# FermiQ/octree-mg

Hardware: AMD Instinct MI355X
Metric: V-cycle cell-updates/s + smoother HBM GB/s vs roofline, 3D Poisson 512^3 (higher is better)
Workload: dtype f64; 1 GPU; C3: 3D Poisson, 512^3 per GPU, box 16, periodic, GSRB FAS V-cycle (n_cycle_down=up=2); mode=weak, box_size=16, parallelism=domain-decomposition x1 (RCCL halos)

## Files before the change

octree-mg_amd/csrc/omg_api.cpp:

```cpp
#include <algorithm>

#include "omg_host.h"

using namespace omg;
using namespace omg::host;

thread_local bool omg::host::g_host_only = false;

namespace {

thread_local std::string g_last_error;

template <typename F>
int guarded(F&& f) {
  try {
    f();
    return 0;
  } catch (const std::exception& e) {
    g_last_error = e.what();
    return 1;
  }
}

void resolve_stats(omg_ctx* c) {
  if (c->pending.empty()) return;
  for (auto& p : c->pending) {
    float ms = 0;
    HIPCHK(hipEventSynchronize(p.e1));
    HIPCHK(hipEventElapsedTime(&ms, p.e0, p.e1));
    for (int pass = 0; pass < (p.lvl == NO_LVL ? 1 : 2); pass++) {
      auto& s = c->stats[pass ? std::string(p.name) + "@" + std::to_string(p.lvl) : std::string(p.name)];
      s.launches++;
      s.ms += ms;
      s.cells += p.cells;
    }
    (void)hipEventDestroy(p.e0);
    (void)hipEventDestroy(p.e1);
  }
  c->pending.clear();
}

double* stage(omg_ctx* c, size_t n) {
  if (n > c->stage_n) {
    dfree(c->d_stage);
    HIPCHK(hipMalloc(&c->d_stage, sizeof(double) * n));
    c->stage_n = n;
  }
  return c->d_stage;
}

constexpr long long kDenseMax = 1LL << 40;

DensePlan& dense_plan(omg_ctx* c, Level& L, const long long* lo, const long long* n, const long long* stride,
                      bool aligned, bool generic, bool own_only) {
  for (auto& P : L.dense)
    if (std::equal(lo, lo + 3, P.lo) && std::equal(n, n + 3, P.n) && std::equal(stride, stride + 3, P.stride) &&
        P.aligned == aligned && P.generic == generic && P.own_only == own_only) {
      P.age = ++c->dense_age;
      return P;
    }
  if ((int)L.dense.size() < kDensePlans) L.dense.emplace_back();
  DensePlan& P = *std::min_element(L.dense.begin(), L.dense.end(),
                                   [](const DensePlan& a, const DensePlan& b) { return a.age < b.age; });
  if (P.d_clips) host_sync(c, c->stream);
  std::copy(lo, lo + 3, P.lo);
  std::copy(n, n + 3, P.n);
  std::copy(stride, stride + 3, P.stride);
  P.aligned = aligned;
  P.generic = generic;
  P.own_only = own_only;
  P.age = ++c->dense_age;
  P.n_row = P.n_gen = 0;
  P.n_cells = 0;
  std::vector<DenseClip> row, gen;
  const long long nc = L.nc;
  const bool row_ok = !generic && aligned && dense_row_nc(L.nc) && stride[1] % 2 == 0 && stride[2] % 2 == 0;
  auto clip = [&](int b) {
    DenseClip r{};
    r.box = b;
    int* lohi[3][2] = {{&r.i0, &r.i1}, {&r.j0, &r.j1}, {&r.k0, &r.k1}};
    long long cells = 1;
    for (int d = 0; d < 3; d++) {
      const long long g0 = ((long long)c->ix[(size_t)(L.ids[b] - 1) * 3 + d] - 1) * nc;
      const long long a = std::max(g0, lo[d]), e = std::min(g0 + nc, lo[d] + n[d]);
      if (a >= e) return;
      *lohi[d][0] = (int)(a - g0) + 1;
      *lohi[d][1] = (int)(e - g0);
      r.off += (a - lo[d]) * stride[d];
      cells *= e - a;
    }
    P.n_cells += cells;
    (row_ok && r.i0 == 1 && r.i1 == L.nc && r.off % 2 == 0 ? row : gen).push_back(r);
  };
  if (own_only)
    for (int b : L.host_local) clip(b);
  else
    for (int b = 0; b < L.n; b++) clip(b);
  P.n_row = (int)row.size();
  P.n_gen = (int)gen.size();
  row.insert(row.end(), gen.begin(), gen.end());
  if (!c->host_only && !row.empty()) {
    if (row.size() > P.cap) {
      dfree(P.d_clips);
      if (P.h_clips) HIPCHK(hipHostFree(P.h_clips));
      P.h_clips = nullptr;
      P.cap = 0;
      HIPCHK(hipHostMalloc((void**)&P.h_clips, sizeof(DenseClip) * row.size()));
      HIPCHK(hipMalloc(&P.d_clips, sizeof(DenseClip) * row.size()));
      P.cap = row.size();
    }
    std::copy(row.begin(), row.end(), P.h_clips);
    HIPCHK(hipMemcpyAsync(P.d_clips, P.h_clips, sizeof(DenseClip) * row.size(), hipMemcpyHostToDevice, c->stream));
  }
  return P;
}

void dense_io(omg_ctx* c, int lvl, int iv, double* dev, const long long* lo, const long long* n,
              const long long* stride, void* stream, long long* n_cells, bool put) {
  const char* who = put ? "omg_put_dense" : "omg_get_dense";
  auto fail = [&](const std::string& what) { throw OmgError(std::string(who) + ": " + what); };
  Level* L = level_ptr(c, lvl);
  if (!L) fail("no such level");
  if (iv < 1 || iv > c->n_vars) fail("bad variable index");
  if (!lo || !n || !stride) fail("lo, n and stride are required");
  for (int d = 0; d < 3; d++) {
    if (n[d] < 0) fail("negative extent");
    if (n[d] > kDenseMax || lo[d] > kDenseMax || lo[d] < -kDenseMax || stride[d] > kDenseMax)
      fail("window out of range");
  }
  if (stride[0] != 1) fail("stride[0] must be 1");
  const bool empty = n[0] == 0 || n[1] == 0 || n[2] == 0;
  if (!empty) {
    if (stride[1] < n[0]) fail("stride[1] < n[0]");
    if (stride[2] / n[1] < stride[1]) fail("stride[2] < stride[1]*n[1]");
    if (stride[2] > LLONG_MAX / 8 / n[2]) fail("window out of range");
    if (!dev) fail("NULL pointer with a non-empty window");
  }
  if (put && L->replicated)
    fail("level " + std::to_string(lvl) + " is replicated on every rank: use omg_upload_level");
  const bool generic = env_flag("OMG_DENSE_GENERIC");
  const bool aligned = ((uintptr_t)dev & 15) == 0;
  if (c->host_only) {
    if (n_cells) *n_cells = empty ? 0 : dense_plan(c, *L, lo, n, stride, aligned, generic, L->replicated).n_cells;
    return;
  }
  if (!empty) {
    hipPointerAttribute_t at{};
    if (hipPointerGetAttributes(&at, dev) != hipSuccess) {
      (void)hipGetLastError();
      fail("the pointer is not device memory");
    }
    if (at.type != hipMemoryTypeDevice) fail("the pointer is not device memory");
    if (at.device != c->device) fail("the pointer belongs to another GPU than the context's");
    hipDeviceptr_t base = nullptr;
    size_t bytes = 0;
    if (hipMemGetAddressRange(&base, &bytes, (hipDeviceptr_t)dev) == hipSuccess) {
      const long long extent = (n[2] - 1) * stride[2] + (n[1] - 1) * stride[1] + n[0];
      if ((const char*)dev + (size_t)extent * sizeof(double) > (const char*)base + bytes)
        fail("the window reaches past the end of the pointer's allocation");
    } else {
      (void)hipGetLastError();
    }
  }
  if (put) {
    enter(c);
    if (iv == 1) phi_dirty(c, lvl);
  } else {
    enter(c, false);
  }
  if (n_cells) *n_cells = 0;
  if (empty || !L->n) return;
  DensePlan& P = dense_plan(c, *L, lo, n, stride, aligned, generic, L->replicated);
  if (n_cells) *n_cells = P.n_cells;
  if (!P.n_cells) return;
  if ((long long)P.n_gen * 16 > INT_MAX) fail("too many boxes for one launch");
  hipStream_t user = (hipStream_t)stream;
  const bool foreign = user != c->stream;
  if (foreign) {
    HIPCHK(hipEventRecord(c->ev_dense_in, user));
    HIPCHK(hipStreamWaitEvent(c->stream, c->ev_dense_in, 0));
  }
  {
    Prof p(c, put ? "dense_put" : "dense_get", (double)P.n_cells, lvl);
    const LevelView V = L->view();
    if (P.n_row) {
      Prof pr(c, put ? "dense_put_row" : "dense_get_row", (double)P.n_row * L->nc * L->nc * L->nc, lvl);
      launch_dense_row(V, iv, P.d_clips, P.n_row, dev, stride[1], stride[2], put, c->stream);
    }
    launch_dense_cell(V, iv, P.d_clips + P.n_row, P.n_gen, dev, stride[1], stride[2], put, c->stream);
    HIPCHK(hipGetLastError());
  }
  if (foreign) {
    HIPCHK(hipEventRecord(c->ev_dense_out, c->stream));
    HIPCHK(hipStreamWaitEvent(user, c->ev_dense_out, 0));
  }
}

}

extern "C" {

const char* omg_last_error(void) { return g_last_error.c_str(); }

int omg_get_unique_id(void* out) {
  return guarded([&] {
    ncclUniqueId id;
    NCCLCHK(ncclGetUniqueId(&id));
    std::memcpy(out, &id, sizeof(id));
  });
}

int omg_loopback_unique_id(long long tag, void* out) {
  return guarded([&] {
    loopback_unique_id(tag, out);
  });
}

int omg_host_unique_id(void* out) {
  return guarded([&] {
    host_unique_id(out);
  });
}

int omg_set_host_transport(omg_ctx* c, omg_host_exchange_fn exchange, omg_host_allgather_fn allgather, void* user) {
  return guarded([&] {
    if (!c->host_xport) throw OmgError("omg_set_host_transport: the context was not created with omg_host_unique_id");
    c->hx_exchange = exchange;
    c->hx_allgather = allgather;
    c->hx_user = user;
  });
}

int omg_device_count(int* n) {
  return guarded([&] { HIPCHK(hipGetDeviceCount(n)); });
}

int omg_ctx_create(omg_ctx** out, int device, int rank, int n_ranks, const void* unique_id) {
  return guarded([&] {
    if (n_ranks < 1 || rank < 0 || rank >= n_ranks) throw OmgError("bad rank / n_ranks");
    if (n_ranks > 1 && !unique_id && device != OMG_DEVICE_NONE)
      throw OmgError("unique_id required for n_ranks > 1");
    auto plan_switches = [](omg_ctx* c) {
      c->no_block3 = env_flag("OMG_NO_BLOCK3");
      c->no_block3_phys = env_flag("OMG_NO_BLOCK3_PHYS");
      c->no_deep = env_flag("OMG_NO_DEEP");
      if (const char* v = getenv("OMG_BLOCK3_MIN_BOXES")) c->b3_min_boxes = std::max(1, atoi(v));
      if (const char* v = getenv("OMG_BLOCK3_COLUMN")) c->b3_col = std::min(std::max(2, atoi(v) & ~1), kB3MaxZ);
      if (const char* v = getenv("OMG_BLOCK3_SMALL_COL")) c->b3_col_small = std::min(std::max(2, atoi(v) & ~1), kB3MaxZ);
    };
    if (device == OMG_DEVICE_NONE) {
      omg_ctx* c = new omg_ctx();
      c->device = device;
      c->rank = rank;
      c->n_ranks = n_ranks;
      c->host_only = true;
      plan_switches(c);
      *out = c;
      return;
    }
    if (device < 0) {
      int n_dev = 0;
      HIPCHK(hipGetDeviceCount(&n_dev));
      if (n_dev < 1) throw OmgError("no HIP device visible");
      device = rank % n_dev;
    }
    omg_ctx* c = new omg_ctx();
    c->device = device;
    c->rank = rank;
    c->n_ranks = n_ranks;
    c->no_tail = env_flag("OMG_NO_TAIL");
    c->no_fuse_up = env_flag("OMG_NO_FUSE_UP");
    c->no_skip1 = env_flag("OMG_NO_SKIP1");
    c->tail_timing = env_flag("OMG_TAIL_TIMING");
    c->no_fill_tile = env_flag("OMG_NO_FILL_TILE");
    c->no_fill_crhs = env_flag("OMG_NO_FILL_CRHS");
    c->no_tail_crhs = env_flag("OMG_NO_TAIL_CRHS");
    c->no_rbgv = env_flag("OMG_NO_RBGV");
    c->no_graph = !env_flag("OMG_GRAPH");
    c->no_fuse_down = env_flag("OMG_NO_FUSE_DOWN");
    c->no_rb_fill_fuse = env_flag("OMG_NO_RB_FUSE");
    c->no_gs_plane = env_flag("OMG_NO_GS_PLANE");
    c->no_fill_xl = env_flag("OMG_NO_FILL_XL");
    c->no_gs_dbl = env_flag("OMG_NO_GS_DBL");
    plan_switches(c);
    c->no_block3p = env_flag("OMG_NO_BLOCK3P");
    c->no_block3r = env_flag("OMG_NO_BLOCK3R");
    c->block4 = !env_flag("OMG_NO_BLOCK4");
    c->no_block4p = env_flag("OMG_NO_BLOCK4P");
    c->block4_phys = env_flag("OMG_BLOCK4_PHYS");
    c->no_defer_gc = env_flag("OMG_NO_DEFER_GC");
    c->no_rhs_pend = env_flag("OMG_NO_RHS_PEND");
    c->no_fuse_down_bc = env_flag("OMG_NO_FUSE_DOWN_BC");
    c->roctx = env_flag("OMG_ROCTX");
    c->debug = env_flag("OMG_DEBUG");
    c->check_collective = env_flag("OMG_CHECK_COLLECTIVE") || c->debug;
    if (const char* v = getenv("OMG_GRAPH_FAIL")) c->graph_fail_at = std::atoi(v);
    HIPCHK(hipSetDevice(device));
    HIPCHK(hipStreamCreateWithFlags(&c->stream, hipStreamNonBlocking));
    HIPCHK(hipMalloc(&c->d_scalar, sizeof(double) * (64 + 2 * (size_t)n_ranks)));
    HIPCHK(hipMalloc(&c->d_red, sizeof(double) * (8 + 2 * (size_t)n_ranks)));
    HIPCHK(hipMemset(c->d_red, 0, sizeof(double) * (8 + 2 * (size_t)n_ranks)));
    HIPCHK(hipMalloc(&c->d_rhs_pend, sizeof(double) * (omg::kRhsPendMax + 1)));
    HIPCHK(hipMemset(c->d_rhs_pend, 0, sizeof(double) * (omg::kRhsPendMax + 1)));
    HIPCHK(hipMalloc(&c->d_maxslots, sizeof(unsigned long long) * omg::kMaxSlots * omg::kMaxSlotStride));
    HIPCHK(hipMalloc(&c->d_tail, sizeof(TailArgs)));
    c->h_tail = new TailArgs;
    std::memset(c->h_tail, 0xff, sizeof(TailArgs));
    HIPCHK(hipMemset(c->d_maxslots, 0, sizeof(unsigned long long) * omg::kMaxSlots * omg::kMaxSlotStride));
    HIPCHK(hipStreamCreateWithFlags(&c->stream2, hipStreamNonBlocking));
    {
      int least = 0, greatest = 0;
      HIPCHK(hipDeviceGetStreamPriorityRange(&least, &greatest));
      HIPCHK(hipStreamCreateWithPriority(&c->stream_comm, hipStreamNonBlocking, greatest));
      c->comm_priority = greatest;
    }
    HIPCHK(hipEventCreateWithFlags(&c->ev_bnd, hipEventDisableTiming));
    HIPCHK(hipEventCreateWithFlags(&c->ev_comm, hipEventDisableTiming));
    HIPCHK(hipEventCreateWithFlags(&c->ev_main, hipEventDisableTiming));
    HIPCHK(hipEventCreateWithFlags(&c->ev_side, hipEventDisableTiming));
    HIPCHK(hipEventCreateWithFlags(&c->ev_phi, hipEventDisableTiming));
    HIPCHK(hipEventCreateWithFlags(&c->ev_dense_in, hipEventDisableTiming));
    HIPCHK(hipEventCreateWithFlags(&c->ev_dense_out, hipEventDisableTiming));
    HIPCHK(hipHostMalloc(&c->h_scalar, sizeof(double) * (16 + (size_t)n_ranks)));
    for (int iv = 0; iv < kMaxVars; iv++)
      for (int nb = 0; nb < 6; nb++) {
        c->bc[iv].type[nb] = OMG_BC_DIRICHLET;
        c->bc[iv].value[nb] = 0.0;
      }
    transport_attach(c, unique_id);
    *out = c;
  });
}

int omg_ctx_destroy(omg_ctx* c) {
  return guarded([&] {
    if (!c) return;
    if (c->host_only) {
      g_host_only = true;
      free_levels(c);
      g_host_only = false;
      delete c;
      return;
    }
    (void)hipSetDevice(c->device);
    (void)hipStreamSynchronize(c->stream);
    (void)hipStreamSynchronize(c->stream2);
    (void)hipStreamSynchronize(c->stream_comm);
    free_levels(c);
    dfree(c->d_scalar);
    if (c->d_tail) (void)hipFree(c->d_tail);
    if (c->d_tail_stamps) (void)hipFree(c->d_tail_stamps);
    delete c->h_tail;
    dfree(c->d_red);
    dfree(c->d_rhs_pend);
    dfree(c->d_maxslots);
    for (auto& kv : c->graphs)
      if (kv.second) (void)hipGraphExecDestroy(kv.second);
    c->graphs.clear();
    dfree(c->d_stage);
    if (c->ev_main) (void)hipEventDestroy(c->ev_main);
    if (c->ev_side) (void)hipEventDestroy(c->ev_side);
    if (c->ev_phi) (void)hipEventDestroy(c->ev_phi);
    if (c->ev_dense_in) (void)hipEventDestroy(c->ev_dense_in);
    if (c->ev_dense_out) (void)hipEventDestroy(c->ev_dense_out);
    if (c->stream2) (void)hipStreamDestroy(c->stream2);
    if (c->stream_comm) (void)hipStreamDestroy(c->stream_comm);
    if (c->ev_bnd) (void)hipEventDestroy(c->ev_bnd);
    if (c->ev_comm) (void)hipEventDestroy(c->ev_comm);
    if (c->h_scalar) (void)hipHostFree(c->h_scalar);
    if (c->h_xsend) (void)hipHostFree(c->h_xsend);
    if (c->h_xrecv) (void)hipHostFree(c->h_xrecv);
    transport_detach(c);
    (void)hipStreamDestroy(c->stream);
    delete c;
  });
}

int omg_tree_setup(omg_ctx* c, int n_boxes, const int* lvl, const int* parent, const int* children,
                   const int* neighbors, const int* ix, const int* rank, int lowest_lvl,
                   int highest_lvl, int first_normal_lvl, int box_size, const int* box_size_lvl,
                   const double* dr, const int* list_off, const int* lists, int n_vars) {
  return guarded([&] {
    if (n_vars < 4 || n_vars > kMaxVars) throw OmgError("n_vars out of range");
    struct HostOnly {
      explicit HostOnly(bool on) { g_host_only = on; }
      ~HostOnly() { g_host_only = false; }
    } host_only_scope(c->host_only);
    if (!c->host_only) (void)hipSetDevice(c->device);
    free_levels(c);
    c->n_boxes = n_boxes;
    c->lvl.assign(lvl, lvl + n_boxes);
    c->parent.assign(parent, parent + n_boxes);
    c->children.assign(children, children + 8 * (size_t)n_boxes);
    c->neighbors.assign(neighbors, neighbors + 6 * (size_t)n_boxes);
    c->ix.assign(ix, ix + 3 * (size_t)n_boxes);
    c->rank_of.assign(rank, rank + n_boxes);
    c->lowest = lowest_lvl;
    c->highest = highest_lvl;
    c->first_normal = first_normal_lvl;
    c->box_size = box_size;
    c->n_vars = n_vars;
    c->bsl.clear();
    c->drl.clear();
    c->ids.clear(); c->leaves.clear(); c->parents.clear(); c->ref_bnds.clear();
    for (int l = lowest_lvl; l <= highest_lvl; l++) {
      const int li = l - lowest_lvl;
      c->bsl[l] = box_size_lvl[li];
      c->drl[l] = {dr[3 * li], dr[3 * li + 1], dr[3 * li + 2]};
      std::map<int, std::vector<int>>* dst[4] = {&c->ids, &c->leaves, &c->parents, &c->ref_bnds};
      for (int t = 0; t < 4; t++) {
        const int a = list_off[4 * li + t], b = list_off[4 * li + t + 1];
        (*dst[t])[l] = std::vector<int>(lists + a, lists + b);
      }
    }
    if (!c->host_only) {
      host_sync(c, c->stream);
      host_sync(c, c->stream2);
    }
    c->rhs_cache_valid = false;
    c->phi_shift_pending = false;
    c->phi_mean_on_side = false;
    build_plan(c);
    if (!c->host_only) HIPCHK(hipDeviceSynchronize());
  });
}

int omg_plan_transfer(omg_ctx* c, int lvl, int which, int dir, int cap, int* peers, long long* keys,
                      int* n_items, int* item_doubles) {
  return guarded([&] {
    Level* L = level_ptr(c, lvl);
    if (!L) throw OmgError("no such level");
    if (which < 0 || which > 5) throw OmgError("omg_plan_transfer: bad transfer");
    const Transfer* T[6] = {&L->halo, &L->restr, &L->prol, &L->rbx, &L->repl, &L->deep_phi};
    const auto& lists = dir ? T[which]->recv : T[which]->send;
    int n = 0;
    for (auto& p : lists)
      for (long long k : p.keys) {
        if (n < cap) {
          peers[n] = p.peer;
          keys[n] = k;
        }
        n++;
      }
    *n_items = n;
    *item_doubles = T[which]->item_doubles;
  });
}

int omg_set_operator(omg_ctx* c, int op, double lambda) {
  return guarded([&] { set_operator(c, op, lambda); });
}

int omg_set_smoother(omg_ctx* c, int smoother, int n_cycle_down, int n_cycle_up, int max_coarse_cycles,
                     double res_abs, double res_rel) {
  return guarded([&] {
    if (smoother != OMG_SMOOTHER_GS && smoother != OMG_SMOOTHER_GSRB)
      throw OmgError("unsupported smoother type");
    if (smoother != c->smoother || std::max(n_cycle_down, 0) != c->n_cycle_down ||
        std::max(n_cycle_up, 0) != c->n_cycle_up)
      rhs_pend_retry(c);
    c->smoother = smoother;
    c->n_substeps = smoother == OMG_SMOOTHER_GSRB ? 2 : 1;
    ensure_rhs_lex(c);
    c->n_cycle_down = std::max(n_cycle_down, 0);
    c->n_cycle_up = std::max(n_cycle_up, 0);
    c->max_coarse_cycles = max_coarse_cycles;
    c->res_abs = res_abs;
    c->res_rel = res_rel;
  });
}

int omg_set_subtract_mean(omg_ctx* c, int on) {
  return guarded([&] { c->subtract_mean = on; });
}

int omg_set_bc(omg_ctx* c, int iv, int nb, int bc_type, double bc_value) {
  return guarded([&] {
    if (iv < 1 || iv > kMaxVars || nb < 1 || nb > 6) throw OmgError("omg_set_bc: bad iv/nb");
    enter(c, false);
    phi_dirty_all(c);
    c->bc[iv - 1].type[nb - 1] = bc_type;
    c->bc[iv - 1].value[nb - 1] = bc_value;
  });
}

int omg_set_bc_faces(omg_ctx* c, int iv, const long long* face_off, const int* face_type,
                     const double* data, long long n_data) {
  return guarded([&] {
    if (iv < 1 || iv > kMaxVars) throw OmgError("omg_set_bc_faces: bad iv");
    if (!c->host_only) enter(c, false);
    phi_dirty_all(c);
    const int k = iv - 1;
    for (auto& kv : c->d_face_off_lvl[k]) dfree(kv.second);
    for (auto& kv : c->d_face_type_lvl[k]) dfree(kv.second);
    c->d_face_off_lvl[k].clear();
    c->d_face_type_lvl[k].clear();
    c->h_face_off_lvl[k].clear();
    c->h_face_type_lvl[k].clear();
    dfree(c->d_face_data[k]);
    if (!face_off) return;
    std::vector<double> packed;
    for (auto& kv : c->levels) {
      Level& L = kv.second;
      if (!L.n) continue;
      std::vector<long long> off(L.n * 6, -1);
      std::vector<int> typ(L.n * 6, 0);
      const long long n2 = (long long)L.nc * L.nc;
      if (L.replicated) {
        bool any[6] = {}, miss[6] = {};
        for (int b = 0; b < L.n; b++)
          for (int nb = 0; nb < 6; nb++) {
            if (L.h_nbk[(size_t)b * 6 + nb] != NB_PHYS) continue;
            (face_off[(size_t)(L.ids[b] - 1) * 6 + nb] >= 0 ? any : miss)[nb] = true;
          }
        for (int nb = 0; nb < 6; nb++)
          if (any[nb] && miss[nb])
            throw OmgError("omg_set_bc_faces: replicated level " + std::to_string(L.lvl) +
                           " needs the boundary table of every box (omg_replicated_level)");
      }
      for (int b = 0; b < L.n; b++)
        for (int nb = 0; nb < 6; nb++) {
          const long long o = face_off[(size_t)(L.ids[b] - 1) * 6 + nb];
          if (o < 0) continue;
          if (o + n2 > n_data) throw OmgError("omg_set_bc_faces: offset out of range");
          off[b * 6 + nb] = (long long)packed.size();
          typ[b * 6 + nb] = face_type[(size_t)(L.ids[b] - 1) * 6 + nb];
          packed.insert(packed.end(), data + o, data + o + n2);
        }
      c->d_face_off_lvl[k][kv.first] = to_device(off);
      c->d_face_type_lvl[k][kv.first] = to_device(typ);
      c->h_face_off_lvl[k][kv.first] = off;
      c->h_face_type_lvl[k][kv.first] = typ;
    }
    c->d_face_data[k] = to_device(packed);
  });
}

int omg_level_size(omg_ctx* c, int lvl, int* n_boxes, int* nc) {
  return guarded([&] {
    Level* L = level_ptr(c, lvl);
    if (!L) throw OmgError("no such level");
    *n_boxes = (int)L->host_local.size();
    *nc = L->nc;
  });
}

int omg_set_coarse_replication(omg_ctx* c, long long max_cells) {
  return guarded([&] {
    if (!c->levels.empty()) throw OmgError("omg_set_coarse_replication: call before omg_tree_setup");
    if (max_cells < 0) throw OmgError("omg_set_coarse_replication: max_cells < 0");
    c->rep_cells = max_cells;
  });
}

int omg_replicated_level(omg_ctx* c, int* lvl) {
  return guarded([&] { *lvl = c->rep_lvl == INT_MIN ? c->lowest - 1 : c->rep_lvl; });
}

int omg_upload_level(omg_ctx* c, int lvl, int iv, const double* host) {
  return guarded([&] {
    enter(c);
    Level* L = level_ptr(c, lvl);
    if (!L) throw OmgError("no such level");
    if (iv < 1 || iv > c->n_vars) throw OmgError("bad variable index");
    if (iv == 1) phi_dirty(c, lvl);
    if (!L->n) return;
    const size_t s = L->nc + 2, box = s * s * s, n = box * L->n;
    double* st = stage(c, n);
    if (L->replicated) {
      std::vector<double> full(n, 0.0);
      for (size_t q = 0; q < L->host_local.size(); q++)
        std::memcpy(full.data() + box * L->host_local[q], host + box * q, sizeof(double) * box);
      HIPCHK(hipMemcpyAsync(st, full.data(), sizeof(double) * n, hipMemcpyHostToDevice, c->stream));
      launch_from_ref(L->view(), iv, st, c->stream);
      if (L->repl.n_send || L->repl.n_recv) {
        launch_box_pack(L->view(), iv, L->repl.d_send_items, L->repl.n_send, L->d_sendbuf, c->stream);
        exchange(c, L->repl, L->d_sendbuf, L->d_recvbuf, nullptr, lvl);
        launch_box_unpack(L->view(), iv, L->repl.d_recv_items, L->repl.n_recv, L->d_recvbuf, c->stream);
      }
      host_sync(c, c->stream);
      return;
    }
    HIPCHK(hipMemcpyAsync(st, host, sizeof(double) * n, hipMemcpyHostToDevice, c->stream));
    launch_from_ref(L->view(), iv, st, c->stream);
    host_sync(c, c->stream);
  });
}

int omg_download_level(omg_ctx* c, int lvl, int iv, double* host) {
  return guarded([&] {
    enter(c, false);
    Level* L = level_ptr(c, lvl);
    if (!L) throw OmgError("no such level");
    if (iv < 1 || iv > c->n_vars) throw OmgError("bad variable index");
// ... 242 lines not shown
```

octree-mg_amd/csrc/omg_cycle.cpp:

```cpp
#include <algorithm>
#include <cmath>
#include <numeric>

#include "omg_host.h"

namespace omg {
namespace host {

static GcBC bc_for(omg_ctx* c, int lvl, int iv) {
  GcBC g;
  for (int nb = 0; nb < 6; nb++) {
    g.type[nb] = c->bc[iv - 1].type[nb];
    g.value[nb] = c->bc[iv - 1].value[nb];
  }
  auto it = c->d_face_off_lvl[iv - 1].find(lvl);
  g.face_off = it == c->d_face_off_lvl[iv - 1].end() ? nullptr : it->second;
  auto jt = c->d_face_type_lvl[iv - 1].find(lvl);
  g.face_type = jt == c->d_face_type_lvl[iv - 1].end() ? nullptr : jt->second;
  g.face_data = c->d_face_data[iv - 1];
  g.phi_stored = c->phi_bc_data_stored;
  return g;
}

void rb_stale_above(omg_ctx* c, int lvl) {
  if (Level* U = level_ptr(c, lvl + 1)) {
    if (U->any_rb) U->phi_gc_ok = false;
    U->rbgv_ok = false;
  }
}
void phi_dirty(omg_ctx* c, int lvl) {
  if (Level* L = level_ptr(c, lvl)) L->phi_gc_ok = L->gc_deferred = false;
  rb_stale_above(c, lvl);
}
void phi_dirty_all(omg_ctx* c) {
  for (auto& kv : c->levels) kv.second.phi_gc_ok = kv.second.rbgv_ok = kv.second.gc_deferred = false;
}

static void rb_host_fixup(omg_ctx* c, Level* L, int iv) {
  if (!c->rbh_any) return;
  auto it = L->rbh.find(iv);
  if (it == L->rbh.end() || it->second.n == 0) return;
  if (c->capturing) throw OmgError("refinement_bnd host callback inside a captured cycle");
  RbHostFaces& R = it->second;
  const int nc = L->nc, nc2 = nc * nc;
  const size_t per = (size_t)(nc + 2) * (nc + 2) * (nc + 2);
  launch_rbh_gather(L->view(), view_of(c, L->lvl - 1), iv, L->d_rb, R.d_items, R.d_slot, R.n, L->d_rbrecv, R.d_cgc,
                    R.d_cc, c->stream);
  HIPCHK(hipMemcpyAsync(R.h_cgc, R.d_cgc, sizeof(double) * R.n * nc2, hipMemcpyDeviceToHost, c->stream));
  HIPCHK(hipMemcpyAsync(R.h_cc, R.d_cc, sizeof(double) * R.n * per, hipMemcpyDeviceToHost, c->stream));
  host_sync(c, c->stream);
  for (int q0 = 0; q0 < R.n;) {
    int q1 = q0;
    while (q1 < R.n && R.nbs[q1] == R.nbs[q0]) q1++;
    const int nb = R.nbs[q0];
    auto fn = (omg_rb_fn)c->rb_fn[iv - 1][nb - 1];
    fn(c->rb_user[iv - 1][nb - 1], L->lvl, iv, q1 - q0, R.ids.data() + q0, R.nbs.data() + q0, nc,
       R.h_cgc + (size_t)q0 * nc2, R.h_cc + (size_t)q0 * per);
    q0 = q1;
  }
  HIPCHK(hipMemcpyAsync(R.d_cc, R.h_cc, sizeof(double) * R.n * per, hipMemcpyHostToDevice, c->stream));
  launch_rbh_scatter(L->view(), iv, R.d_items, R.n, R.d_cc, c->stream);
  host_sync(c, c->stream);
}

static void finish_rb(omg_ctx* c, Level* L, int iv);
static void finish_halo(omg_ctx* c, Level* L, int iv, bool rb_hook = true) {
  if (c->n_ranks > 1) {
    if (L->halo.n_send || L->halo.n_recv) {
      exchange(c, L->halo, L->d_sendbuf, L->d_recvbuf, nullptr, L->lvl);
      launch_unpack_faces(L->view(), iv, L->halo.d_recv_items, L->halo.n_recv, L->d_recvbuf, c->stream);
    }
    finish_rb(c, L, iv);
  }
  if (rb_hook) rb_host_fixup(c, L, iv);
}

static void finish_rb(omg_ctx* c, Level* L, int iv) {
  if (c->n_ranks == 1) return;
  if (L->rbx.n_send || L->rbx.n_recv) {
    launch_rb_pack(view_of(c, L->lvl - 1), iv, L->rbx.d_send_items, L->rbx.n_send, L->nc, L->d_rbsend,
                   c->stream);
    exchange(c, L->rbx, L->d_rbsend, L->d_rbrecv, nullptr, L->lvl);
    launch_rb_unpack(L->view(), iv, L->rbx.d_recv_items, L->rbx.n_recv, L->d_rbrecv, c->stream);
  }
}

void fill_gc_lvl(omg_ctx* c, int lvl, int iv) {
  if (lvl < c->lowest) throw OmgError("fill_ghost_cells_lvl: lvl < lowest_lvl");
  if (lvl > c->highest) throw OmgError("fill_ghost_cells_lvl: lvl > highest_lvl");
  Level* L = level_ptr(c, lvl);
  if (!L) return;
  if (iv == 1) {
    L->phi_gc_ok = true;
    L->gc_deferred = false;
    rb_stale_above(c, lvl);
  }
  if (L->n) {
    Prof p(c, "fill_gc", (double)L->n * 6 * L->nc * L->nc, lvl);
    if (iv != 1 || L->has_rb || c->no_fill_tile ||
        !launch_fill_tile(L->sweep_view(), bc_for(c, lvl, iv), L->d_sendbuf, c->stream))
      launch_fill_gc(L->view(), iv, 3, view_of(c, lvl - 1), L->d_rb, bc_for(c, lvl, iv), L->d_sendbuf,
                     c->stream);
  }
  finish_halo(c, L, iv);
}

static void deep_before(omg_ctx* c, Level* L, int colour) {
  if (!L->deep) return;
  materialize_rhs(c, L);
  const LevelView V = L->view();
  if (c->check_collective && (allreduce(c, L->prox_rhs_ok ? 1.0 : 0.0, true) > 0.5) != L->prox_rhs_ok)
    throw OmgError("deep halo: the rhs refill decision differs across ranks (an rhs write was not collective)");
  if (!L->prox_rhs_ok) {
    Prof p(c, "deep_rhs", (double)L->deep_rhs.n_recv * 64, L->lvl);
    launch_deep_copy(V, 2, 0, 64, L->deep_rhs.d_send_items, L->deep_rhs.n_send, L->d_sendbuf, false, c->stream);
    exchange(c, L->deep_rhs, L->d_sendbuf, L->d_recvbuf, nullptr, L->lvl);
    launch_deep_copy(V, 2, 0, 64, L->deep_rhs.d_recv_items, L->deep_rhs.n_recv, L->d_recvbuf, true, c->stream);
    L->prox_rhs_ok = true;
  }
  Prof p(c, "deep_phi", (double)L->deep_phi.n_recv * 32, L->lvl);
  launch_deep_copy(V, 1, colour, 32, L->deep_phi.d_send_items, L->deep_phi.n_send, L->d_sendbuf, false, c->stream);
  exchange(c, L->deep_phi, L->d_sendbuf, L->d_recvbuf, nullptr, L->lvl);
  launch_deep_copy(V, 1, colour, 32, L->deep_phi.d_recv_items, L->deep_phi.n_recv, L->d_recvbuf, true, c->stream);
}
static void deep_after(omg_ctx* c, Level* L, bool defer = false) {
  if (!L->deep) return;
  hipStream_t st = c->stream;
  if (defer && L->n_bnd && L->n_int) {
    HIPCHK(hipEventRecord(c->ev_bnd, c->stream));
    HIPCHK(hipStreamWaitEvent(c->stream_comm, c->ev_bnd, 0));
    st = c->stream_comm;
    L->faces_pending = true;
  }
  Prof p(c, "deep_faces", (double)L->halo.n_recv * L->nc * L->nc, L->lvl, st);
  launch_face_pack(L->view(), 1, L->halo.d_send_items, L->halo.n_send, L->d_sendbuf, st);
  exchange(c, L->halo, L->d_sendbuf, L->d_recvbuf, st, L->lvl);
  launch_unpack_faces(L->view(), 1, L->halo.d_recv_items, L->halo.n_recv, L->d_recvbuf, st);
  if (L->faces_pending) HIPCHK(hipEventRecord(c->ev_comm, c->stream_comm));
}
static void deep_res(omg_ctx* c, Level* L) {
  if (!L->deep) return;
  const LevelView V = L->view();
  Prof p(c, "deep_res", (double)L->deep_rhs.n_recv * 64, L->lvl);
  launch_deep_copy(V, 4, 0, 64, L->deep_rhs.d_send_items, L->deep_rhs.n_send, L->d_sendbuf, false, c->stream);
  exchange(c, L->deep_rhs, L->d_sendbuf, L->d_recvbuf, nullptr, L->lvl);
  launch_deep_copy(V, 4, 0, 64, L->deep_rhs.d_recv_items, L->deep_rhs.n_recv, L->d_recvbuf, true, c->stream);
  launch_face_pack(V, 4, L->halo.d_send_items, L->halo.n_send, L->d_sendbuf, c->stream);
  exchange(c, L->halo, L->d_sendbuf, L->d_recvbuf, nullptr, L->lvl);
  launch_unpack_faces(V, 4, L->halo.d_recv_items, L->halo.n_recv, L->d_recvbuf, c->stream);
}

static void faces_join(omg_ctx* c, Level* L) {
  if (!L || !L->faces_pending) return;
  HIPCHK(hipStreamWaitEvent(c->stream, c->ev_comm, 0));
  L->faces_pending = false;
}

bool smooth_boxes(omg_ctx* c, int lvl, int n_cycle, int first_substep, int skip_last,
                  bool want_res, bool four, bool defer_faces) {
  Level* L = level_ptr(c, lvl);
  const int n_sub = n_cycle * c->n_substeps - skip_last;
  bool res_done = false;
  if (!L) return false;
  if (n_sub >= 1) rb_stale_above(c, lvl);
  const bool absorb = L->shift_pending && c->smoother == OMG_SMOOTHER_GSRB && n_sub >= 1 &&
                      (L->phi_gc_ok || L->gc_deferred) &&
                      !L->has_rb && gs_tiled(L->nc, c->op, L->has_rb) && !(L->d_b3 && L->b3_phys);
  if (L->shift_pending && !absorb) materialize_level(c, L);
  if (c->smoother != OMG_SMOOTHER_GSRB) {
    materialize_rhs(c, L);
    const bool ring = n_sub >= 1 && L->d_rhs_lex && gs_lex_ring_ok(L->nc, c->op);
    if (ring && !L->rhs_lex_ok) {
      Prof p(c, "rhs_lex", (double)L->n * L->nc * L->nc * L->nc, lvl);
      launch_rhs_lex(L->view(), L->d_rhs_lex, c->stream);
      L->rhs_lex_ok = true;
    }
    const bool xlf = ring && L->d_xlay && !L->has_rb && !c->no_fill_tile && !c->no_fill_xl;
    if (xlf && L->d_galt && n_sub % 2 == 0 && L->n && !c->no_gs_dbl) {
      const GcBC bc = bc_for(c, lvl, 1);
      double* prim = L->d_phi + 2 * (long long)L->view().hv;
      for (int n = 1; n <= n_sub; n++) {
        const bool odd = n & 1;
        GhostSets gs;
        gs.in = odd ? prim : L->d_galt;
        gs.in_stride = odd ? L->stride : 6 * (long long)stored_face(L->nc);
        gs.out = odd ? L->d_galt : prim;
        gs.out_stride = odd ? 6 * (long long)stored_face(L->nc) : L->stride;
        gs.phys_load = n > 1;
        Prof p(c, "smoother_gs", (double)L->n * L->nc * L->nc * L->nc, lvl);
        launch_gs_lex(L->view(), c->op, c->lambda, c->stream, L->d_rhs_lex, nullptr, &gs, &bc);
      }
      if (L->n_physbox) {
        Prof p(c, "fill_gc", (double)L->n_physbox * 6 * L->nc * L->nc, lvl);
        launch_phys_gc(L->view(), bc, L->d_physbox, L->n_physbox, c->stream);
      }
      L->phi_gc_ok = true;
      return false;
    }
    for (int n = 1; n <= n_sub; n++) {
      if (L->n) {
        Prof p(c, "smoother_gs", (double)L->n * L->nc * L->nc * L->nc, lvl);
        launch_gs_lex(L->view(), c->op, c->lambda, c->stream, ring ? L->d_rhs_lex : nullptr,
                      xlf ? L->d_xlay : nullptr);
      }
      if (xlf) {
        L->phi_gc_ok = true;
        if (L->n) {
          Prof p(c, "fill_gc", (double)L->n * 6 * L->nc * L->nc, lvl);
          launch_fill_tile_xl(L->sweep_view(), bc_for(c, lvl, 1), L->d_sendbuf, L->d_xlay, c->stream);
        }
        finish_halo(c, L, 1);
      } else {
        fill_gc_lvl(c, lvl, 1);
      }
    }
    return false;
  }
  for (int n = first_substep; n <= n_sub; n++) {
    const int e = n & 1;
    const bool odd = L->nc & 1;
    if (n == 1 && absorb) phi_mean_ready(c);
    const double* shift = (n == 1 && absorb) ? red_mean(c, 0) : nullptr;
    if (n == 1) L->shift_pending = false;
    B3Phys P3;
    const B3Phys* ph = nullptr;
    const bool b3 = b3_usable(c, lvl, P3, ph);
    if (four && (n_sub - n + 1) % 4 == 0 && b3 && (!ph || c->block4_phys)) {
      double* other = L->d_phi == L->d_data ? L->d_phi_buf : L->d_data;
      deep_before(c, L, 1 - e);
      if (ph) materialize_rhs(c, L);
      {
        Prof p(c, "smoother_gsrb4", 2.0 * L->n * L->nc * L->nc * L->nc, lvl);
        launch_gsrb4(L->view(), other, L->d_b3, L->n_b3, c->op, c->lambda, e, shift, c->stream, nullptr, nullptr,
                     ph, true, rhs_shifts(c, L));
      }
      L->d_phi = other;
      if (L->gc_deferred) L->phi_gc_ok = true, L->gc_deferred = false;
      deep_after(c, L, defer_faces && n + 3 == n_sub);
      n += 3;
      continue;
    }
    if (n + 2 <= n_sub && b3 && !(want_res && (n_sub - n + 1) % 3 != 0)) {
      double* other = L->d_phi == L->d_data ? L->d_phi_buf : L->d_data;
      const bool push1 = L->deep || !(skip_last == 1 && n + 2 == n_sub && e == 1);
      const bool res = want_res && n + 2 == n_sub && push1;
      materialize_rhs(c, L);
      deep_before(c, L, 1 - e);
      {
        Prof p(c, res ? "smoother_gsrb3r" : "smoother_gsrb3", 1.5 * L->n * L->nc * L->nc * L->nc, lvl);
        launch_gsrb3(L->view(), other, L->d_b3, L->n_b3, c->op, c->lambda, e, shift, c->stream, push1, nullptr,
                     nullptr, 1, res, ph);
      }
      res_done = res;
      L->d_phi = other;
      if (L->gc_deferred) L->phi_gc_ok = true, L->gc_deferred = false;
      deep_after(c, L);
      if (res) deep_res(c, L);
      n += 2;
      continue;
    }
    if (L->gc_deferred) fill_gc_lvl(c, lvl, 1);
    materialize_rhs(c, L);
    if (L->n_bnd && L->n_int && !odd && gs_tiled(L->nc, c->op, L->has_rb)) {
      const int gvm = L->d_rbgv ? (L->rbgv_ok ? 2 : 1) : 0;
      if (gvm) L->rbgv_ok = true;
      {
        Prof p(c, "smoother_gsrb", 0.5 * L->n_bnd * L->nc * L->nc * L->nc, lvl);
        launch_gs_substep(L->sweep_view(), c->op, c->lambda, e, 1 << e, view_of(c, lvl - 1), L->d_rb, L->has_rb,
                          bc_for(c, lvl, 1), L->d_sendbuf, shift, c->stream, L->d_bnd, L->n_bnd, L->d_rbgv, gvm);
      }
      HIPCHK(hipEventRecord(c->ev_bnd, c->stream));
      {
        Prof p(c, "smoother_gsrb", 0.5 * L->n_int * L->nc * L->nc * L->nc, lvl);
        launch_gs_substep(L->sweep_view(), c->op, c->lambda, e, 1 << e, view_of(c, lvl - 1), L->d_rb, L->has_rb,
                          bc_for(c, lvl, 1), L->d_sendbuf, shift, c->stream, L->d_int, L->n_int, L->d_rbgv, gvm);
      }
      HIPCHK(hipStreamWaitEvent(c->stream_comm, c->ev_bnd, 0));
      exchange(c, L->halo, L->d_sendbuf, L->d_recvbuf, c->stream_comm, lvl);
      launch_unpack_faces(L->view(), 1, L->halo.d_recv_items, L->halo.n_recv, L->d_recvbuf, c->stream_comm);
      HIPCHK(hipEventRecord(c->ev_comm, c->stream_comm));
      HIPCHK(hipStreamWaitEvent(c->stream, c->ev_comm, 0));
      finish_rb(c, L, 1);
      if (!L->phi_gc_ok) fill_gc_lvl(c, lvl, 1);
      else rb_host_fixup(c, L, 1);
      continue;
    }
    if (L->n) {
      Prof p(c, "smoother_gsrb", 0.5 * L->n * L->nc * L->nc * L->nc, lvl);
      const int gvm = L->d_rbgv ? (L->rbgv_ok ? 2 : 1) : 0;
      if (gvm) L->rbgv_ok = true;
      launch_gs_substep(L->sweep_view(), c->op, c->lambda, e, odd ? 0 : 1 << e, view_of(c, lvl - 1), L->d_rb,
                        L->has_rb, bc_for(c, lvl, 1), L->d_sendbuf, shift, c->stream, nullptr, 0, L->d_rbgv, gvm);
    }
    const bool full_fill = odd || !L->phi_gc_ok;
    finish_halo(c, L, 1, !full_fill);
    if (full_fill) fill_gc_lvl(c, lvl, 1);
  }
  return res_done;
}

static bool tiled_level(omg_ctx* c, const Level* L) {
  (void)c;
  return L && tiled_nc(L->nc);
}

void residual_lvl(omg_ctx* c, int lvl, unsigned long long* maxbits) {
  Level* L = level_ptr(c, lvl);
  if (!L || L->n == 0) return;
  if (!tiled_level(c, L)) materialize_rhs(c, L);
  Prof p(c, "residual", (double)L->n * L->nc * L->nc * L->nc, lvl);
  if (tiled_level(c, L))
    launch_resid_restrict(L->sweep_view(), empty_view(), c->op, c->lambda, maxbits, 0, nullptr, nullptr, c->stream,
                          nullptr, 0, rhs_shifts(c, L));
  else
    launch_residual(L->view(), c->op, c->lambda, maxbits, c->stream);
}

static double max_residual_levels(omg_ctx* c, int lo, int hi) {
  unsigned long long* d = (unsigned long long*)c->d_scalar;
  for (int l = lo; l <= hi; l++) {
    residual_lvl(c, l, c->d_maxslots);
    launch_max_fold(c->d_maxslots, d, l > lo, c->stream);
  }
  HIPCHK(hipMemcpyAsync(c->h_scalar, d, 8, hipMemcpyDeviceToHost, c->stream));
  if (c->capturing) {
    if (c->max_deferred) throw OmgError("internal: two max-residual readbacks in one captured cycle");
    c->max_deferred = true;
    return 0.0;
  }
  host_sync(c, c->stream);
  return c->h_scalar[0];
}

double max_residual_lvl(omg_ctx* c, int lvl) { return max_residual_levels(c, lvl, lvl); }

static void restrict_remote(omg_ctx* c, int iv, int lvl) {
  Level* F = level_ptr(c, lvl);
  Level* C = level_ptr(c, lvl - 1);
  if (c->n_ranks > 1 && F && C && (F->restr.n_send || F->restr.n_recv)) {
    launch_restrict_pack(F->view(), iv, F->restr.d_send_items, F->restr.n_send, F->d_sendbuf, c->stream);
    exchange(c, F->restr, F->d_sendbuf, C->d_recvbuf, nullptr, lvl);
    launch_restrict_unpack(C->view(), iv, F->restr.d_recv_items, F->restr.n_recv, F->nc / 2, C->d_recvbuf,
                           c->stream);
  }
}

void restrict_lvl(omg_ctx* c, int iv, int lvl) {
  if (lvl <= c->lowest) throw OmgError("cannot restrict lvl <= lowest_lvl");
  if (iv == 1) phi_dirty(c, lvl - 1);
  Level* F = level_ptr(c, lvl);
  restrict_remote(c, iv, lvl);
  if (F && F->n_pairs) {
    Prof p(c, "restrict", (double)F->n_pairs * F->nc * F->nc * F->nc, lvl);
    launch_restrict(F->view(), view_of(c, lvl - 1), iv, F->d_pairs, F->n_pairs, F->d_parent_local, F->d_dix,
                    c->stream);
  }
}

void prolong(omg_ctx* c, int lvl, int iv, int iv_to, int add) {
  if (lvl == c->highest) throw OmgError("cannot prolong highest level");
  if (lvl < c->lowest) throw OmgError("cannot prolong below lowest level");
  if (iv_to == 1) phi_dirty(c, lvl + 1);
  Level* F = level_ptr(c, lvl + 1);
  Level* C = level_ptr(c, lvl);
  const LevelView FV = view_of(c, lvl + 1), CV = view_of(c, lvl);
  if (c->n_ranks > 1 && F && C && (F->prol.n_send || F->prol.n_recv)) {
    launch_prolong_pack(CV, FV, iv, F->prol.d_send_items, F->prol.n_send, C->d_sendbuf, c->stream);
    exchange(c, F->prol, C->d_sendbuf, F->d_recvbuf, nullptr, lvl + 1);
    launch_prolong_unpack(FV, iv_to, add, F->prol.d_recv_items, F->prol.n_recv, F->d_recvbuf,
                          c->stream);
  }
  if (F && F->n_pairs) {
    Prof p(c, "prolong", (double)F->n_pairs * F->nc * F->nc * F->nc, lvl + 1);
    launch_prolong(CV, FV, iv, iv_to, add, F->d_pairs, F->n_pairs, F->d_parent_local, F->d_dix,
                   c->stream);
  }
}

static bool smooth_resid_ok(omg_ctx* c, int lvl) {
  const Level* F = level_ptr(c, lvl);
  const Level* C = level_ptr(c, lvl - 1);
  if (F) {
    const auto rbh = F->rbh.find(1);
    if (rbh != F->rbh.end() && rbh->second.n) return false;
  }
  return !c->no_fuse_down && F && C && F->n && c->smoother == OMG_SMOOTHER_GSRB && c->n_substeps == 2 &&
         c->n_cycle_down >= 1 &&
         (c->op == OP_LPL || c->op == OP_HELM) && (F->nc == 16 || F->nc == 8) &&
         !(c->no_fuse_down_bc && (F->has_rb || F->has_phys)) && (!F->has_remote || F->n_int) &&
         !F->any_rbx;
}

void update_coarse(omg_ctx* c, int lvl, bool fused, bool tail_crhs) {
  Level* F = level_ptr(c, lvl);
  if (Level* Cl = level_ptr(c, lvl - 1)) {
    Cl->rhs_lex_ok = Cl->prox_rhs_ok = false;
    if (Cl->all_parents) Cl->shift_pending = false;
    else materialize_level(c, Cl);
    materialize_rhs(c, Cl);
  }
  if (F && (fused || !tiled_level(c, F))) materialize_rhs(c, F);
  if (F && F->n && tiled_level(c, F)) {
    const bool rbgv = F->rbgv_ok;
    phi_dirty(c, lvl - 1);
    if (fused && F->has_remote) {
      const bool faces = F->any_phys || F->any_rb;
      {
        Prof p(c, "smoother_gsrb", 0.5 * F->n_bnd * F->nc * F->nc * F->nc, lvl);
        launch_gs_substep(F->view(), c->op, c->lambda, 0, faces ? 1 | 4 : 1, view_of(c, lvl - 1), F->d_rb,
                          F->has_rb, bc_for(c, lvl, 1), F->d_sendbuf, nullptr, c->stream, F->d_bnd, F->n_bnd,
                          rbgv ? F->d_rbgv : nullptr, rbgv ? 2 : 0);
      }
      HIPCHK(hipEventRecord(c->ev_bnd, c->stream));
      {
        Prof p(c, "smooth_resid", (double)F->n_int * F->nc * F->nc * F->nc, lvl);
        if (!launch_smooth_resid(F->sweep_view(), view_of(c, lvl - 1), c->op, c->lambda, 1, F->d_parent_local,
                                 F->d_dix, c->stream, F->d_int, F->n_int, bc_for(c, lvl, 1), F->has_rb, F->has_phys,
                                 rbgv ? F->d_rbgv : nullptr))
          throw OmgError("smooth_resid: not available for this level");
      }
      HIPCHK(hipStreamWaitEvent(c->stream_comm, c->ev_bnd, 0));
      exchange(c, F->halo, F->d_sendbuf, F->d_recvbuf, c->stream_comm, lvl);
      launch_unpack_faces(F->view(), 1, F->halo.d_recv_items, F->halo.n_recv, F->d_recvbuf, c->stream_comm, 1);
      HIPCHK(hipEventRecord(c->ev_comm, c->stream_comm));
      HIPCHK(hipStreamWaitEvent(c->stream, c->ev_comm, 0));
      if (faces && F->n_bndface) {
        Prof p(c, "face_gc", (double)F->n_bndface * 6 * F->nc * F->nc, lvl);
        launch_face_gc(F->view(), view_of(c, lvl - 1), bc_for(c, lvl, 1), F->d_bndface, F->n_bndface, c->stream);
      }
      {
        Prof p(c, "resid_restrict", (double)F->n_bnd * F->nc * F->nc * F->nc, lvl);
        launch_resid_restrict(F->sweep_view(), view_of(c, lvl - 1), c->op, c->lambda, nullptr, 1, F->d_parent_local,
                              F->d_dix, c->stream, F->d_bnd, F->n_bnd, rhs_shifts(c, F));
      }
    } else if (fused) {
      Prof p(c, "smooth_resid", (double)F->n * F->nc * F->nc * F->nc, lvl);
      if (!launch_smooth_resid(F->sweep_view(), view_of(c, lvl - 1), c->op, c->lambda, 1, F->d_parent_local,
                               F->d_dix, c->stream, nullptr, 0, bc_for(c, lvl, 1), F->has_rb, F->has_phys,
                               rbgv ? F->d_rbgv : nullptr))
        throw OmgError("smooth_resid: not available for this level");
    } else if (F->faces_pending) {
      {
        Prof p(c, "resid_restrict", (double)F->n_int * F->nc * F->nc * F->nc, lvl);
        launch_resid_restrict(F->sweep_view(), view_of(c, lvl - 1), c->op, c->lambda, nullptr, 1, F->d_parent_local,
                              F->d_dix, c->stream, F->d_int, F->n_int, rhs_shifts(c, F));
      }
      faces_join(c, F);
      {
        Prof p(c, "resid_restrict", (double)F->n_bnd * F->nc * F->nc * F->nc, lvl);
        launch_resid_restrict(F->sweep_view(), view_of(c, lvl - 1), c->op, c->lambda, nullptr, 1, F->d_parent_local,
                              F->d_dix, c->stream, F->d_bnd, F->n_bnd, rhs_shifts(c, F));
      }
    } else {
      Prof p(c, "resid_restrict", (double)F->n * F->nc * F->nc * F->nc, lvl);
      launch_resid_restrict(F->sweep_view(), view_of(c, lvl - 1), c->op, c->lambda, nullptr, 1, F->d_parent_local,
                            F->d_dix, c->stream, nullptr, 0, rhs_shifts(c, F));
    }
    restrict_remote(c, 1, lvl);
    restrict_remote(c, 4, lvl);
    if (fused && (F->any_phys || F->any_rb)) F->phi_gc_ok = false;
  } else {
    residual_lvl(c, lvl, nullptr);
    restrict_lvl(c, 1, lvl);
    restrict_lvl(c, 4, lvl);
  }
  if (tail_crhs) return;
  Level* C = level_ptr(c, lvl - 1);
  if (C && C->n && !C->parents.empty() && !C->has_rb && !C->has_remote && !c->no_fill_tile && !c->no_fill_crhs &&
      (C->nc == 16 || C->nc == 8 || C->nc == 4)) {
    C->phi_gc_ok = true;
    rb_stale_above(c, lvl - 1);
    {
      Prof p(c, "fill_crhs", (double)C->n * C->nc * C->nc * C->nc, lvl - 1);
      launch_fill_crhs(C->sweep_view(), c->op, c->lambda, bc_for(c, lvl - 1, 1), C->d_parmask, c->stream);
    }
    finish_halo(c, C, 1);
    return;
  }
  fill_gc_lvl(c, lvl - 1, 1);
  if (C && !C->parents.empty()) {
    Prof p(c, "coarse_rhs", (double)C->parents.size() * C->nc * C->nc * C->nc, lvl - 1);
    if (!launch_coarse_rhs_tile(C->sweep_view(), c->op, c->lambda, C->d_parents, (int)C->parents.size(), c->stream))
      launch_coarse_rhs(C->view(), c->op, c->lambda, C->d_parents, (int)C->parents.size(), c->stream);
  }
}

void correct_children(omg_ctx* c, int lvl) {
  Level* C = level_ptr(c, lvl);
  if (C && !C->parents.empty()) {
    Prof p(c, "sub_parents", (double)C->parents.size() * C->nc * C->nc * C->nc, lvl);
    launch_sub_parents(C->view(), C->d_parents, (int)C->parents.size(), c->stream);
  }
  prolong(c, lvl, 4, 1, 1);
}

static bool prolong_smooth(omg_ctx* c, int lvl) {
  Level* F = level_ptr(c, lvl + 1);
  Level* C = level_ptr(c, lvl);
  const bool rb_ok = F && !c->no_rb_fill_fuse && !F->any_rbx && (F->nc == 16 || F->nc == 8) &&
                     !(F->rbh.count(1) && F->rbh.at(1).n);
  if (c->no_fuse_up || !F || !C || !F->prolong_smooth_ok || c->smoother != OMG_SMOOTHER_GSRB ||
      (c->op != OP_LPL && c->op != OP_HELM) ||
      c->n_cycle_up < 1 || (F->has_rb && !rb_ok) || (F->has_remote && !F->n_int) || !gs_tiled(F->nc, c->op, F->has_rb) ||
      !((size_t)F->n == 8 * C->parents.size() || C->nc * 2 == F->nc) ||
      (c->n_ranks > 1 && (F->prol.n_send || F->prol.n_recv)))
    return false;
  if (F->shift_pending) materialize_level(c, F);
  materialize_rhs(c, F);
  rb_stale_above(c, lvl + 1);
  const bool split = F->has_remote;
  {
    const int n = split ? F->n_int : F->n;
    Prof p(c, "prolong_smooth", (double)n * F->nc * F->nc * F->nc, lvl + 1);
    launch_prolong_smooth(C->view(), F->sweep_view(), c->op, c->lambda, F->d_parent_local, F->d_dix,
                          bc_for(c, lvl + 1, 1), C->nc * 2 == F->nc, split ? F->d_int : nullptr, n,
                          split ? F->d_push0 : nullptr, c->stream, F->has_rb, F->has_rb ? F->d_rbgv : nullptr);
    if (F->has_rb && F->d_rbgv) F->rbgv_ok = true;
  }
  if (split) {
    {
      Prof p(c, "prolong_fill", (double)F->n_bnd * F->nc * F->nc * F->nc, lvl + 1);
      launch_prolong_fill(C->view(), F->sweep_view(), 4, F->d_parent_local, F->d_dix, bc_for(c, lvl + 1, 1),
                          F->d_sendbuf, true, !c->no_skip1, c->stream, F->d_bnd, F->n_bnd, false,
                          F->h_rb.empty() ? nullptr : F->d_rb);
    }
    finish_halo(c, F, 1);
    {
      Prof p(c, "smoother_gsrb", 0.5 * F->n_bnd * F->nc * F->nc * F->nc, lvl + 1);
      launch_gs_substep(F->view(), c->op, c->lambda, 1, 1 << 1, view_of(c, lvl), F->d_rb, F->has_rb,
                        bc_for(c, lvl + 1, 1), F->d_sendbuf, nullptr, c->stream, F->d_bnd, F->n_bnd,
                        F->has_rb ? F->d_rbgv : nullptr, F->has_rb && F->d_rbgv ? 1 : 0);
    }
    finish_halo(c, F, 1);
  }
  F->phi_gc_ok = true;
  return true;
}

static bool block3c_ok(omg_ctx* c, const Level* F) {
  return F && F->d_b3c && !c->no_block3 && !c->no_block3p && c->smoother == OMG_SMOOTHER_GSRB &&
         gsrb3_op_ok(c->op) && c->n_cycle_up * c->n_substeps >= 3;
}
static int correct_block3(omg_ctx* c, int l, bool res_ready, bool defer_gc = false) {
  Level* F = level_ptr(c, l);
  Level* C = level_ptr(c, l - 1);
  if (!block3c_ok(c, F) || !C || !C->phi_gc_ok || C->shift_pending) return 0;
  if (F->deep && !res_ready) return 0;
  if (F->shift_pending) materialize_level(c, F);
  rb_stale_above(c, l);
  double* other = F->d_phi == F->d_data ? F->d_phi_buf : F->d_data;
  const LevelView cv = C->view();
  int done = 3;
  deep_before(c, F, 0);
  bool deferred = false;
  if (res_ready && c->block4 && !c->no_block4p && c->n_cycle_up * c->n_substeps >= 4) {
    deferred = defer_gc && c->n_ranks == 1 && c->n_cycle_up * c->n_substeps == 4 && !F->deep && !F->b3_phys &&
               !c->no_defer_gc;
    Prof p(c, "smoother_gsrb4p", 2.0 * F->n * F->nc * F->nc * F->nc, l);
    launch_gsrb4(F->view(), other, F->d_b3, F->n_b3, c->op, c->lambda, 1, nullptr, c->stream, &cv, F->d_b3c,
                 nullptr, !deferred, rhs_shifts(c, F));
    done = 4;
  } else {
    materialize_rhs(c, F);
    Prof p(c, "smoother_gsrb3p", 1.5 * F->n * F->nc * F->nc * F->nc, l);
    launch_gsrb3(F->view(), other, F->d_b3, F->n_b3, c->op, c->lambda, 1, nullptr, c->stream, true, &cv, F->d_b3c,
                 res_ready ? 2 : 1);
  }
  F->d_phi = other;
  deep_after(c, F);
  F->phi_gc_ok = !deferred;
  F->gc_deferred = deferred;
  return done;
}

static bool correct_fill_fused(omg_ctx* c, int lvl) {
  Level* F = level_ptr(c, lvl + 1);
  Level* C = level_ptr(c, lvl);
  return F && C && F->n && F->n_pairs == F->n && tiled_nc(F->nc) && !(F->has_rb && c->no_rb_fill_fuse) &&
         !(c->n_ranks > 1 && (F->prol.n_send || F->prol.n_recv));
}

static void correct_and_fill(omg_ctx* c, int lvl, bool then_gsrb = false, bool save_old = false) {
  Level* F = level_ptr(c, lvl + 1);
  Level* C = level_ptr(c, lvl);
  if (save_old && (then_gsrb || !correct_fill_fused(c, lvl)))
    throw OmgError("internal: old = phi fused into an unfused correction");
  rb_stale_above(c, lvl + 1);
  if (correct_fill_fused(c, lvl)) {
    const bool sub = (size_t)F->n == 8 * C->parents.size() || C->nc * 2 == F->nc;
    if (!sub && !C->parents.empty()) {
      Prof p(c, "sub_parents", (double)C->parents.size() * C->nc * C->nc * C->nc, lvl);
      launch_sub_parents(C->view(), C->d_parents, (int)C->parents.size(), c->stream);
    }
    {
      Prof p(c, "prolong_fill", (double)F->n * F->nc * F->nc * F->nc, lvl + 1);
      launch_prolong_fill(C->view(), F->sweep_view(), 4, F->d_parent_local, F->d_dix, bc_for(c, lvl + 1, 1),
                          F->d_sendbuf, sub, then_gsrb && !c->no_skip1, c->stream, nullptr, 0, save_old,
                          F->h_rb.empty() ? nullptr : F->d_rb);
    }
    finish_halo(c, F, 1);
    F->phi_gc_ok = true;
    return;
  }
  correct_children(c, lvl);
  fill_gc_lvl(c, lvl + 1, 1);
}

static int tail_top(omg_ctx* c, int max_lvl) {
  if (c->op != OP_LPL && c->op != OP_HELM) return INT_MIN;
  if (max_lvl - c->lowest + 1 > kTailMaxLevels) max_lvl = c->lowest + kTailMaxLevels - 1;
  int top = INT_MIN;
  for (int l = c->lowest; l <= max_lvl; l++) {
    Level* L = level_ptr(c, l);
    if (!L || L->n < 1 || L->n > kTailMaxBoxes || L->n != (int)c->ids[l].size() || L->has_rb ||
        !tiled_nc(L->nc))
      break;
    if (l > c->lowest) {
      Level* C = level_ptr(c, l - 1);
      if (L->n_pairs != L->n || !((size_t)L->n == 8 * C->parents.size() || C->nc * 2 == L->nc)) break;
    }
    top = l;
  }
  return top;
}

static void tail_lds_plan(omg_ctx* c, int top, int* lds_levels, int* lds_top) {
  const int n_lvls = top - c->lowest + 1;
  auto lds_box_ok = [&](int l, int max_nc) {
    Level* L = level_ptr(c, l);
    if (!L || L->n != 1 || L->nc > max_nc) return false;
    for (int nb = 0; nb < 6; nb++) {
      const int k = L->h_nbk[nb];
      if (!(k == NB_PHYS || (k == NB_LOCAL && L->h_nba[nb] == 0))) return false;
    }
    return true;
  };
  int n = 0;
  while (n < std::min(n_lvls, kTailLdsMaxLevels) && lds_box_ok(c->lowest + n, 8)) n++;
  *lds_levels = n;
  *lds_top = n > 0 && n == n_lvls - 1 && level_ptr(c, top)->nc == 16 && lds_box_ok(top, 16);
}

static bool tail_crhs_ok(omg_ctx* c, int top) {
  const Level* T = level_ptr(c, top);
  return !c->no_tail_crhs && T && T->n == 1 && !T->parents.empty() && !T->has_rb && !T->has_remote &&
         level_ptr(c, top + 1) != nullptr;
}

static void run_tail(omg_ctx* c, int top, bool top_crhs) {
  TailArgs A;
  std::memset(&A, 0, sizeof(A));
  A.n_lvls = top - c->lowest + 1;
  for (int l = c->lowest; l <= top; l++) {
    Level* L = level_ptr(c, l);
    if (L->shift_pending) {
      if (L->all_parents && l < top) L->shift_pending = false;
      else materialize_level(c, L);
    }
    materialize_rhs(c, L);
    L->rhs_lex_ok = L->prox_rhs_ok = false;
    TailLevel& T = A.lv[l - c->lowest];
    T.L = L->view();
    T.bc = bc_for(c, l, 1);
    T.parents = L->d_parents;
    T.n_par = (int)L->parents.size();
    T.parent_local = L->d_parent_local;
    T.dixp = L->d_dix;
    auto fo = c->h_face_off_lvl[0].find(l);
    auto ft = c->h_face_type_lvl[0].find(l);
    for (int nb = 0; nb < 6; nb++) {
      const bool tab = fo != c->h_face_off_lvl[0].end() && fo->second.size() >= 6;
      const long long o = tab ? fo->second[nb] : -1;
      T.foff[nb] = o > INT_MAX ? -2 : (int)o;
      T.ftype[nb] = (signed char)(tab && ft != c->h_face_type_lvl[0].end() && ft->second.size() >= 6 ? ft->second[nb] : 0);
    }
  }
  A.lambda = c->lambda;
  A.n_down = c->n_cycle_down;
  A.n_up = c->n_cycle_up;
  A.max_coarse = c->max_coarse_cycles;
  A.res_abs = c->res_abs;
  A.res_rel = c->res_rel;
  A.maxbits = (unsigned long long*)c->d_scalar;
  A.coarse_its = (int*)(c->d_scalar + 1);
  A.gs_lex = c->smoother != OMG_SMOOTHER_GSRB;
  A.top_crhs = top_crhs;
  tail_lds_plan(c, top, &A.lds_levels, &A.lds_top);
  const bool tail_timing = c->tail_timing;
  if (tail_timing) {
    if (!c->d_tail_stamps) HIPCHK(hipMalloc(&c->d_tail_stamps, 8 * 64));
    A.stamps = c->d_tail_stamps;
    HIPCHK(hipMemsetAsync(c->d_tail_stamps, 0, 8 * 64, c->stream));
  }
  if (std::memcmp(&A, c->h_tail, sizeof(TailArgs)) != 0) {
    *c->h_tail = A;
    launch_store_tail(A, c->d_tail, c->stream);
  }
  {
    Prof p(c, "coarse_tail", 0.0, top);
    launch_coarse_tail(c->d_tail, A.gs_lex, c->op, c->stream);
  }
  if (tail_timing) {
    long long h[64];
    HIPCHK(hipMemcpyAsync(h, c->d_tail_stamps, sizeof(h), hipMemcpyDeviceToHost, c->stream));
    host_sync(c, c->stream);
    std::fprintf(stderr, "tail us:");
    for (int i = 1; i < 64 && h[i]; i++) std::fprintf(stderr, " %.1f", (h[i] - h[i - 1]) * 0.01);
    std::fprintf(stderr, "\n");
  }
  for (int l = c->lowest; l <= top; l++) level_ptr(c, l)->phi_gc_ok = true;
  rb_stale_above(c, top);
}

void check_finite_res(double r, const char* where) {
  if (!std::isfinite(r))
    throw OmgError(std::string(where) + ": non-finite residual (" + (std::isnan(r) ? "NaN" : "Inf") +
                   "): phi or rhs holds NaN/Inf");
}

double fas_vcycle(omg_ctx* c, int highest_lvl, bool want_max_res, bool standalone) {
  const bool has_highest = highest_lvl >= c->lowest;
  const int min_lvl = c->lowest, max_lvl = has_highest ? highest_lvl : c->highest;
  const bool full = standalone && !has_highest;
  if (c->phi_shift_pending) {
    if (!full) {
      materialize_phi(c);
    } else {
      for (auto& kv : c->levels) {
        Level& L = kv.second;
        if (L.shift_pending && L.lvl != max_lvl && !L.all_parents) materialize_level(c, &L);
      }
    }
  }
  if (!full) materialize_rhs_all(c);
  struct FullCycle {
    omg_ctx* c;
    ~FullCycle() { c->in_full_cycle = false; }
  } full_cycle{c};
  c->in_full_cycle = full;
  if (c->subtract_mean && !has_highest) subtract_mean(c, 2, 0, full ? kInCycle : kPlain);
  if (standalone) {
    Level* L = level_ptr(c, max_lvl);
    bool need = !(L && L->phi_gc_ok && (!L->any_rb || c->n_ranks == 1 || !c->subtract_mean));
    if (L && L->gc_deferred && c->smoother == OMG_SMOOTHER_GSRB && tail_top(c, max_lvl) < max_lvl &&
        c->n_cycle_down * c->n_substeps >= 1)
      need = false;
    if (c->n_ranks > 1 && c->check_collective && (allreduce(c, need ? 1.0 : 0.0, true) > 0.5) != need)
      throw OmgError("mg_fas_vcycle: the stand-alone fill decision differs across ranks "
                     "(an upload of phi was not made on every rank)");
    if (need) {
      if (L) materialize_level(c, L);
      fill_gc_lvl(c, max_lvl, 1);
    }
  }
  const int top = tail_top(c, max_lvl);
  const bool tail = top >= min_lvl && !c->no_tail;
  const bool tail_crhs = tail && max_lvl > top && tail_crhs_ok(c, top);
  for (int l = max_lvl; l >= min_lvl + 1; l--) {
    if (tail && l <= top) break;
    B3Phys P3;
    const B3Phys* ph = nullptr;
    const bool four = c->block4 && c->smoother == OMG_SMOOTHER_GSRB && b3_usable(c, l, P3, ph) &&
                      (!ph || c->block4_phys) && (c->n_cycle_down * c->n_substeps) % 4 == 0;
    const bool fused = !four && smooth_resid_ok(c, l);
    smooth_boxes(c, l, c->n_cycle_down, 1, fused ? 1 : 0, false, four, four);
    if (Level* Fd = level_ptr(c, l); Fd && Fd->gc_deferred) fill_gc_lvl(c, l, 1);
    update_coarse(c, l, fused, tail_crhs && l == top + 1);
    faces_join(c, level_ptr(c, l));
  }
  if (tail) {
    run_tail(c, top, tail_crhs);
  } else {
    const auto& ids = c->ids[min_lvl];
    for (int id : ids)
      if (min_lvl > c->rep_lvl && c->rank_of[id - 1] != c->rank_of[ids[0] - 1])
        throw OmgError("Multiple CPUs for coarse grid (not implemented yet)");
    const Level* Lmin = level_ptr(c, min_lvl);
    const bool own_coarse = Lmin && Lmin->n > 0;
    double init_res = own_coarse ? max_residual_lvl(c, min_lvl) : 0.0;
    for (int i = 1; own_coarse && i <= c->max_coarse_cycles; i++) {
      smooth_boxes(c, min_lvl, c->n_cycle_up + c->n_cycle_down);
      double res = max_residual_lvl(c, min_lvl);
      if (res < c->res_rel * init_res || res < c->res_abs) break;
    }
  }
  bool res_ready = false;
  for (int l = (tail ? top : min_lvl) + 1; l <= max_lvl; l++) {
    const bool want_res = l < max_lvl && block3c_ok(c, level_ptr(c, l + 1)) && !c->no_block3r;
    bool done = false;
    int pro = 0;
    if (!want_res && (pro = correct_block3(c, l, res_ready, full && l == max_lvl && !want_max_res)) > 0) {
      done = smooth_boxes(c, l, c->n_cycle_up, pro + 1);
    } else {
      if (Level* Fd = level_ptr(c, l); Fd && Fd->gc_deferred) fill_gc_lvl(c, l, 1);
      if (prolong_smooth(c, l - 1)) {
        done = smooth_boxes(c, l, c->n_cycle_up, 2, 0, want_res);
      } else {
        correct_and_fill(c, l - 1, c->smoother == OMG_SMOOTHER_GSRB && c->n_cycle_up >= 1);
        done = smooth_boxes(c, l, c->n_cycle_up, 1, 0, want_res);
      }
    }
    res_ready = done;
  }
  double max_res = 0.0;
  if (want_max_res) {
    double m = 0.0;
    if (min_lvl <= max_lvl) m = max_residual_levels(c, min_lvl, max_lvl);
    max_res = allreduce(c, m, true);
  }
  materialize_phi(c);
  if (c->subtract_mean) subtract_mean(c, 1, 1, full ? kInCycle : kPlain);
  return max_res;
}

double fas_fmg(omg_ctx* c, bool have_guess, bool want_max_res) {
  materialize_rhs_all(c);
  if (have_guess) {
    materialize_phi(c);
  } else {
    for (auto& kv : c->levels) kv.second.shift_pending = false;
    c->phi_shift_pending = false;
  }
  if (!have_guess) phi_dirty_all(c);
  if (!have_guess)
    for (int l = c->highest; l >= c->lowest; l--) {
      Level* L = level_ptr(c, l);
      if (L && L->n) launch_copy_var(L->view(), 0, 1, c->stream);
    }
  fill_gc_lvl(c, c->highest, 1);
  for (int l = c->highest; l >= c->lowest + 1; l--) update_coarse(c, l);
  if (c->subtract_mean) subtract_mean(c, 2, 0);
  double max_res = 0.0;
  for (int l = c->lowest; l <= c->highest; l++) {
    Level* L = level_ptr(c, l);
    const bool old_is_phi = l < c->highest && L && L->all_parents && !c->subtract_mean;
    const bool save_old = L && L->n && !old_is_phi && l > c->lowest && correct_fill_fused(c, l - 1);
    if (save_old) {
      launch_copy_ghosts(L->view(), c->stream);
    } else if (L && L->n && !old_is_phi) {
      launch_copy_var(L->view(), 1, 3, c->stream);
    }
    if (l > c->lowest) correct_and_fill(c, l - 1, false, save_old);
    if (l == c->highest)
      max_res = fas_vcycle(c, l, want_max_res, false);
    else
      fas_vcycle(c, l, false, false);
  }
  return max_res;
}

static bool graph_ok(omg_ctx* c) {
  return !c->no_graph && !c->capturing && c->n_ranks == 1 && !c->subtract_mean && !c->profiling && !c->rbh_any &&
         !c->tail_timing && !c->no_tail && c->n_boxes > 0 && tail_top(c, c->highest) >= c->lowest;
}

static void graph_rollback(omg_ctx* c, int key, const std::map<int, double*>& phi_at_start) {
  c->capturing = false;
  for (auto& kv : phi_at_start) c->levels[kv.first].d_phi = kv.second;
  c->max_deferred = false;
  std::memset(c->h_tail, 0xff, sizeof(TailArgs));
  auto it = c->graphs.find(key);
  if (it != c->graphs.end()) {
    if (it->second) (void)hipGraphExecDestroy(it->second);
    c->graphs.erase(it);
  }
  phi_dirty_all(c);
  drop_rhs_lex(c);
  (void)hipGetLastError();
}

double run_cycle(omg_ctx* c, int key, const std::function<double()>& body) {
  if (!graph_ok(c)) return body();
  std::map<int, double*> phi_at_start;
  for (auto& kv : c->levels) phi_at_start[kv.first] = kv.second.d_phi;
  c->capturing = true;
  c->max_deferred = false;
  HIPCHK(hipStreamBeginCapture(c->stream, hipStreamCaptureModeThreadLocal));
  hipGraph_t g = nullptr;
  try {
    if (c->graph_fail_at == 1) {
      c->graph_fail_at = 0;
      throw OmgError("injected failure during capture (OMG_GRAPH_FAIL=1)");
    }
    body();
  } catch (...) {
    (void)hipStreamEndCapture(c->stream, &g);
    if (g) (void)hipGraphDestroy(g);
    graph_rollback(c, key, phi_at_start);
    throw;
  }
  c->capturing = false;
  try {
    HIPCHK(hipStreamEndCapture(c->stream, &g));
    size_t n_nodes = 0;
    HIPCHK(hipGraphGetNodes(g, nullptr, &n_nodes));
    if (c->graph_fail_at == 2) {
      c->graph_fail_at = 0;
      throw OmgError("injected failure before the launch (OMG_GRAPH_FAIL=2)");
    }
    if (n_nodes) {
      hipGraphExec_t& ex = c->graphs[key];
      if (ex) {
        hipGraphNode_t err_node = nullptr;
        hipGraphExecUpdateResult res;
        if (hipGraphExecUpdate(ex, g, &err_node, &res) != hipSuccess || res != hipGraphExecUpdateSuccess) {
          (void)hipGetLastError();
          HIPCHK(hipGraphExecDestroy(ex));
          ex = nullptr;
        }
      }
      if (!ex) HIPCHK(hipGraphInstantiate(&ex, g, nullptr, nullptr, 0));
      HIPCHK(hipGraphLaunch(ex, c->stream));
    }
  } catch (...) {
    if (g) (void)hipGraphDestroy(g);
    graph_rollback(c, key, phi_at_start);
    throw;
  }
  HIPCHK(hipGraphDestroy(g));
  if (!c->max_deferred) return 0.0;
  c->max_deferred = false;
  host_sync(c, c->stream);
  return c->h_scalar[0];
}

void set_operator(omg_ctx* c, int op, double lambda) {
  if (op < OMG_LAPLACIAN || op > OMG_AHELMHOLTZ) throw OmgError("mg_set_methods: unknown operator");
  if (lambda < 0) throw OmgError("helmholtz_set_lambda: lambda < 0 not allowed");
  if (op == OMG_AHELMHOLTZ && c->n_vars < 7 && c->n_boxes > 0)
    throw OmgError("ahelmholtz_set_methods: needs 3 extra variables");
  if ((op == OMG_VLAPLACIAN || op == OMG_VHELMHOLTZ) && c->n_vars < 5 && c->n_boxes > 0)
    throw OmgError("vlaplacian/vhelmholtz_set_methods: mg%n_extra_vars == 0");
  if (op == OMG_VLAPLACIAN) lambda = 0.0;
  const bool changed = c->op != op;
  if (changed) rhs_pend_retry(c);
  c->op = op;
  c->lambda = lambda;
  if (changed && !c->capturing) ensure_rhs_lex(c);
}

void apply_op(omg_ctx* c, int i_out) {
  enter(c);
  if (i_out == 1) phi_dirty_all(c);
  for (int l = c->lowest; l <= c->highest; l++) {
    Level* L = level_ptr(c, l);
    if (L && L->n) launch_box_op(L->view(), c->op, c->lambda, i_out, c->stream);
  }
}

void set_rhs(omg_ctx* c, double f1, double f2) {
  enter(c);
  for (int l = 1; l <= c->highest; l++) {
    Level* L = level_ptr(c, l);
    if (!L || L->leaves.empty()) continue;
    launch_set_rhs(L->view(), L->d_leaves, (int)L->leaves.size(), f1, f2, c->stream);
  }
}

constexpr int kDiffusionMaxIts = 10;
void diffusion_solve(omg_ctx* c, int op, double dt, double coeff, int order, double max_res, int* n_vcycles,
                     double* res_out) {
  if (op != OMG_HELMHOLTZ && op != OMG_VHELMHOLTZ && op != OMG_AHELMHOLTZ)
    throw OmgError("diffusion_solve: operator must be helmholtz, vhelmholtz or ahelmholtz");
  if (order != 1 && order != 2) throw OmgError("diffusion_solve: order should be 1 or 2");
  const double dtc = op == OMG_HELMHOLTZ ? dt * coeff : dt;
  set_operator(c, op, 0.0);
  if (op != OMG_AHELMHOLTZ) c->subtract_mean = 0;
  if (order == 1) {
    set_operator(c, op, 1 / dtc);
    set_rhs(c, -1 / dtc, 0.0);
  } else {
    apply_op(c, 2);
    set_operator(c, op, 2 / dtc);
    set_rhs(c, -2 / dtc, -1.0);
  }
  double res = run_cycle(c, 2 + 2 + 4, [&] { return fas_fmg(c, true, true); });
  int n = 1;
  for (; n <= kDiffusionMaxIts; n++) {
    if (!std::isfinite(res)) {
      if (n_vcycles) *n_vcycles = n - 1;
      if (res_out) *res_out = res;
      check_finite_res(res, "diffusion_solve");
    }
    if (res <= max_res) break;
    res = run_cycle(c, 1 + 2 + 4 + 8 * (c->lowest - 1 + 64),
                    [&] { return fas_vcycle(c, c->lowest - 1, true, true); });
  }
  if (n_vcycles) *n_vcycles = n - 1;
  if (res_out) *res_out = res;
  if (n == kDiffusionMaxIts + 1) throw OmgError("diffusion_solve: no convergence");
}

void phi_bc_store(omg_ctx* c) {
  phi_dirty_all(c);
  for (auto& kv : c->levels) {
    Level& L = kv.second;
    if (!L.n) continue;
    GcBC g = bc_for(c, kv.first, 1);
    g.phi_stored = 0;
    launch_phi_bc_store(L.view(), g, L.d_nba, c->stream);
    HIPCHK(hipMemcpyAsync(L.h_nba.data(), L.d_nba, sizeof(int) * L.h_nba.size(), hipMemcpyDeviceToHost,
                          c->stream));
    host_sync(c, c->stream);
    for (int b = 0; b < L.n; b++)
      for (int nb = 1; nb <= 6; nb++)
        if (L.h_nbk[(size_t)b * 6 + nb - 1] == NB_PHYS)
          c->neighbors[(size_t)(L.ids[b] - 1) * 6 + nb - 1] = L.h_nba[(size_t)b * 6 + nb - 1];
    pack_topo(L);
  }
  c->phi_bc_data_stored = 1;
}

}
}
```

octree-mg_amd/csrc/omg_host.h:

```cpp
#pragma once

#include <hip/hip_runtime.h>
#include <hipfft/hipfft.h>
#include <rccl/rccl.h>
#include <rocprofiler-sdk-roctx/roctx.h>

#include <climits>
#include <condition_variable>
#include <cstdio>
#include <cstdlib>
#include <cstring>
#include <functional>
#include <map>
#include <memory>
#include <mutex>
#include <stdexcept>
#include <string>
#include <tuple>
#include <vector>

#include "../../include/omg.h"
#include "omg_free.h"
#include "omg_kernels.h"

struct omg_loop {
  struct Msg {
    const double* src;
    size_t n;
    hipEvent_t ev;
  };
  using Key = std::tuple<int, int, long long>;
  int n_ranks = 0;
  std::mutex mu;
  std::condition_variable cv;
  std::map<Key, Msg> box;
  std::map<Key, hipEvent_t> acks;
  std::map<long long, std::vector<double>> vals;
  std::map<long long, int> n_in, n_out;
};

struct omg_free_state {
  bool initialized = false;
  int fft_lvl = INT_MIN;
  omg::FreeGrid G{};
  double r_min[3] = {0, 0, 0};
  double* d_R = nullptr;
  double2* d_Z = nullptr;
  double* d_karray = nullptr;
  double* d_planes = nullptr;
  hipfftHandle fwd = 0, inv = 0;
  bool have_plans = false;
  int n_my = 0;
  int* d_my = nullptr;
  int* d_my_ix = nullptr;
  omg::Transfer gather;
  double* d_send = nullptr;
  double* d_recv = nullptr;
  int* d_recv_ix = nullptr;
  omg::FreePlaneGeom P{};
};

namespace omg {
namespace host {

struct OmgError : std::runtime_error {
  using std::runtime_error::runtime_error;
};

#define HIPCHK(x)                                                                            \
  do {                                                                                       \
    hipError_t e_ = (x);                                                                     \
    if (e_ != hipSuccess)                                                                    \
      throw OmgError(std::string(#x) + ": " + hipGetErrorString(e_) + " (" + __FILE__ + ":" + \
                     std::to_string(__LINE__) + ")");                                        \
  } while (0)

#define NCCLCHK(x)                                                                         \
  do {                                                                                     \
    ncclResult_t r_ = (x);                                                                 \
    if (r_ != ncclSuccess) throw OmgError(std::string(#x) + ": " + ncclGetErrorString(r_)); \
  } while (0)

inline void host_sync(omg_ctx* c, hipStream_t st) {
  c->n_host_syncs++;
  HIPCHK(hipStreamSynchronize(st));
}

extern thread_local bool g_host_only;

template <typename T>
void dmalloc(T** p, size_t bytes, bool zero = false) {
  *p = nullptr;
  if (g_host_only || bytes == 0) return;
  HIPCHK(hipMalloc((void**)p, bytes));
  if (zero) HIPCHK(hipMemset(*p, 0, bytes));
}

template <typename T>
T* to_device(const std::vector<T>& v) {
  if (v.empty() || g_host_only) return nullptr;
  T* d = nullptr;
  HIPCHK(hipMalloc(&d, sizeof(T) * v.size()));
  HIPCHK(hipMemcpy(d, v.data(), sizeof(T) * v.size(), hipMemcpyHostToDevice));
  return d;
}

template <typename T>
void dfree(T*& p) {
  if (p) (void)hipFree((void*)p);
  p = nullptr;
}

const int kNeighbRev[6] = {2, 1, 4, 3, 6, 5};

inline bool env_flag(const char* name) {
  const char* v = getenv(name);
  return v && *v && std::strcmp(v, "0") != 0;
}

inline double snan_value() {
  const unsigned long long bits = 0x7FF4000000000000ULL;
  double d;
  std::memcpy(&d, &bits, 8);
  return d;
}

inline int pack_dix(const int d[3]) { return d[0] | (d[1] << 10) | (d[2] << 20); }

struct Tree {
  omg_ctx* c;
  int lvl(int id) const { return c->lvl[id - 1]; }
  int parent(int id) const { return c->parent[id - 1]; }
  int child(int id, int s) const { return c->children[(id - 1) * 8 + s - 1]; }
  int nbr(int id, int nb) const { return c->neighbors[(id - 1) * 6 + nb - 1]; }
  int rank(int id) const { return c->rank_of[id - 1]; }
  void child_offset(int id, int d[3]) const {
    if (lvl(id) <= c->first_normal) {
      d[0] = d[1] = d[2] = 0;
    } else {
      for (int q = 0; q < 3; q++) d[q] = ((c->ix[(id - 1) * 3 + q] - 1) & 1) * (c->box_size >> 1);
    }
  }
};

inline Level* level_ptr(omg_ctx* c, int l) {
  auto it = c->levels.find(l);
  return it == c->levels.end() ? nullptr : &it->second;
}

inline LevelView empty_view() {
  LevelView v;
  std::memset(&v, 0, sizeof(v));
  return v;
}

inline LevelView view_of(omg_ctx* c, int l) {
  Level* L = level_ptr(c, l);
  return L ? L->view() : empty_view();
}

struct Rec {
  int peer;
  long long key;
  int a, b, c = 0;
};
std::vector<PeerList> group(std::vector<Rec>& recs, int ints_per_item);

constexpr int NO_LVL = INT_MIN;

struct Prof {
  omg_ctx* c;
  const char* name;
  double cells;
  int lvl;
  hipStream_t st;
  hipEvent_t e0 = nullptr, e1 = nullptr;
  bool range = false;
  Prof(omg_ctx* c_, const char* n, double cl, int l = NO_LVL, hipStream_t s = nullptr)
      : c(c_), name(n), cells(cl), lvl(l), st(s ? s : c_->stream) {
    if (c->roctx) {
      char buf[64];
      if (lvl == NO_LVL) std::snprintf(buf, sizeof(buf), "%s", name);
      else std::snprintf(buf, sizeof(buf), "%s@%d", name, lvl);
      roctxRangePushA(buf);
      range = true;
    }
    if (!c->profiling) return;
    HIPCHK(hipEventCreate(&e0));
    HIPCHK(hipEventCreate(&e1));
    HIPCHK(hipEventRecord(e0, st));
  }
  ~Prof() {
    if (range) roctxRangePop();
    if (!e0) return;
    (void)hipEventRecord(e1, st);
    c->pending.push_back({name, e0, e1, cells, lvl});
  }
};

void loopback_unique_id(long long tag, void* out);
void host_unique_id(void* out);
void transport_attach(omg_ctx* c, const void* unique_id);
void transport_detach(omg_ctx* c);
std::vector<double> loop_allgather(omg_ctx* c, double v);
std::vector<double> host_allgather(omg_ctx* c, double v);
void exchange(omg_ctx* c, const Transfer& T, const double* sendbuf, double* recvbuf, hipStream_t st = nullptr,
              int lvl = NO_LVL);
double allreduce(omg_ctx* c, double v, bool is_max);

void pack_topo(Level& L);
void finalize_transfer(Transfer& T);
void rbh_build(omg_ctx* c);
void ensure_rhs_lex(omg_ctx* c);
void free_levels(omg_ctx* c);
bool b3_usable(omg_ctx* c, int lvl, B3Phys& P, const B3Phys*& ph);
void build_plan(omg_ctx* c);

void rb_stale_above(omg_ctx* c, int lvl);
void phi_dirty(omg_ctx* c, int lvl);
void phi_dirty_all(omg_ctx* c);
void fill_gc_lvl(omg_ctx* c, int lvl, int iv);
bool smooth_boxes(omg_ctx* c, int lvl, int n_cycle, int first_substep = 1, int skip_last = 0,
                  bool want_res = false, bool four = false, bool defer_faces = false);
void residual_lvl(omg_ctx* c, int lvl, unsigned long long* maxbits);
double max_residual_lvl(omg_ctx* c, int lvl);
void restrict_lvl(omg_ctx* c, int iv, int lvl);
void prolong(omg_ctx* c, int lvl, int iv, int iv_to, int add);
void update_coarse(omg_ctx* c, int lvl, bool fused = false, bool tail_crhs = false);
void correct_children(omg_ctx* c, int lvl);
void check_finite_res(double r, const char* where);
double fas_vcycle(omg_ctx* c, int highest_lvl, bool want_max_res, bool standalone);
double fas_fmg(omg_ctx* c, bool have_guess, bool want_max_res);
double run_cycle(omg_ctx* c, int key, const std::function<double()>& body);
void set_operator(omg_ctx* c, int op, double lambda);
void apply_op(omg_ctx* c, int i_out);
void set_rhs(omg_ctx* c, double f1, double f2);
void diffusion_solve(omg_ctx* c, int op, double dt, double coeff, int order, double max_res, int* n_vcycles,
                     double* res_out);
void phi_bc_store(omg_ctx* c);

enum { kChPhi = 0, kChRhs = 1 };
double* red_mean(omg_ctx* c, int ch);
double get_sum(omg_ctx* c, int iv);
void phi_mean_ready(omg_ctx* c);
void materialize_level(omg_ctx* c, Level* L);
void materialize_phi(omg_ctx* c);
RhsShifts rhs_shifts(omg_ctx* c, const Level* L);
void materialize_rhs(omg_ctx* c, Level* L);
void materialize_rhs_all(omg_ctx* c);
void rhs_pend_retry(omg_ctx* c);
void drop_rhs_lex(omg_ctx* c);
void enter(omg_ctx* c, bool writes = true);
enum { kPlain = 0, kInCycle = 1 };
void subtract_mean(omg_ctx* c, int iv, int ghosts, int mode = kPlain);

void free_state_destroy(omg_ctx* c);
double poisson_free_3d(omg_ctx* c, bool new_rhs, double max_fft_frac, bool fmgcycle, bool want_max_res,
                       const double* r_min, const double* box_r_min);

}
}
```

octree-mg_amd/csrc/omg_internal.h:

```cpp
#pragma once

#include <cstdlib>
#include <hip/hip_runtime.h>

#include <climits>
#include <cstdint>
#include <map>
#include <memory>
#include <string>
#include <vector>

#include "../../include/omg.h"

namespace omg {

enum NbKind : int8_t { NB_LOCAL = 0, NB_PHYS = 1, NB_RB = 2, NB_REMOTE = 3, NB_RBREM = 4 };

enum Op : int { OP_LPL = 1, OP_VLPL = 2, OP_HELM = 3, OP_VHELM = 4, OP_AHELM = 5 };

constexpr int kMaxVars = 16;

constexpr int kB3MinBoxes = 4096;

#ifdef OMG_RHS_PEND_MAX
constexpr int kRhsPendMax = OMG_RHS_PEND_MAX;
#else
constexpr int kRhsPendMax = 4;
#endif

struct RhsShifts {
  const double* s = nullptr;
  int n = 0;
};

struct BCVar {
  int type[6];
  double value[6];
  long long* d_face_off = nullptr;
  int* d_face_type = nullptr;
};

struct LevelView {
  double* data;
  double* phi;
  long long stride;
  long long vstride;
  int n;
  int nc;
  int h, hf;
  int hv;
  int fs;
  double idr2[3];
  double dr[3];
  const int8_t* nbk;
  const int* nba;
  const int* sendpos;
  const int* topo;
  int rev;
};

inline int stored_face(int nc) { return 2 * ((nc + 1) / 2) * nc; }

inline int stored_cells(int nc) {
  const int h = (nc + 1) / 2;
  return 2 * h * nc * nc + 6 * 2 * h * nc;
}

struct RBRec {
  int coarse_idx;
  int dix[3];
};

struct PeerList {
  int peer;
  std::vector<long long> keys;
  std::vector<int> items;
  int offset = 0;
};

struct Transfer {
  std::vector<PeerList> send, recv;
  int* d_send_items = nullptr;
  int* d_recv_items = nullptr;
  int n_send = 0, n_recv = 0;
  int item_doubles = 0;
  int send_ints = 1, recv_ints = 1;
};

struct RbHostFaces {
  std::vector<int> items, slot, ids, nbs;
  int n = 0;
  int* d_items = nullptr;
  int* d_slot = nullptr;
  double* d_cgc = nullptr;
  double* d_cc = nullptr;
  double* h_cgc = nullptr;
  double* h_cc = nullptr;
};

struct DenseClip {
  int box;
  int i0, i1, j0, j1, k0, k1;
  int pad_;
  long long off;
};

struct DensePlan {
  long long lo[3] = {0, 0, 0}, n[3] = {0, 0, 0}, stride[3] = {0, 0, 0};
  bool aligned = false, generic = false, own_only = false;
  DenseClip* h_clips = nullptr;
  DenseClip* d_clips = nullptr;
  size_t cap = 0;
  int n_row = 0, n_gen = 0;
  long long n_cells = 0;
  long long age = 0;
};
constexpr int kDensePlans = 4;

struct Level {
  int lvl = 0, nc = 0, n = 0;
  long long stride = 0;
  double dr[3] = {0, 0, 0};
  std::vector<int> ids;
  bool replicated = false;
  std::vector<int> host_local;
  Transfer repl;
  double* d_data = nullptr;
  double* d_phi = nullptr;
  bool phi_gc_ok = false;
  bool gc_deferred = false;
  bool has_rb = false, has_remote = false, has_phys = false;
  bool any_rb = false, any_phys = false;
  bool any_rbx = false;
  bool all_parents = false;
  bool prolong_smooth_ok = false;
  bool shift_pending = false;
  int rhs_pend = 0;
  bool rhs_pend_off = false;
  int8_t* d_nbk = nullptr;
  int* d_nba = nullptr;
  int* d_sendpos = nullptr;
  std::vector<int> h_sendpos;
  int* d_topo = nullptr;
  std::vector<int8_t> h_nbk;
  std::vector<int> h_nba;
  RBRec* d_rb = nullptr;
  std::vector<RBRec> h_rb;
  std::vector<int> parents, leaves;
  int* d_parents = nullptr;
  int* d_leaves = nullptr;
  uint8_t* d_parmask = nullptr;
  double* d_rbgv = nullptr;
  bool rbgv_ok = false;
  std::vector<int> parent_local;
  std::vector<int> dix_packed;
  int* d_parent_local = nullptr;
  int* d_dix = nullptr;
  int* d_pairs = nullptr;
  int n_pairs = 0;
  Transfer halo;
  Transfer restr;
  Transfer prol;
  Transfer rbx;
  double* d_scratch_rhs = nullptr;
  double* d_rhs_lex = nullptr;
  bool rhs_lex_ok = false;
  double* d_xlay = nullptr;
  double* d_galt = nullptr;
  double* d_phi_buf = nullptr;
  int* d_b3 = nullptr;
  int n_b3 = 0;
  std::vector<int> h_b3;
  bool b3_phys = false;
  int* d_b3c = nullptr;
  bool deep = false;
  int n_prox = 0;
  std::vector<int> prox_ids;
  Transfer deep_phi, deep_rhs;
  bool prox_rhs_ok = false;
  bool faces_pending = false;
  int* d_physbox = nullptr;
  int n_physbox = 0;
  int* d_bnd = nullptr;
  int* d_int = nullptr;
  int n_bnd = 0, n_int = 0;
  int* d_bndface = nullptr;
  int n_bndface = 0;
  uint8_t* d_push0 = nullptr;
  double* d_rbsend = nullptr;
  double* d_rbrecv = nullptr;
  double* d_sendbuf = nullptr;
  double* d_recvbuf = nullptr;
  size_t sendbuf_doubles = 0, recvbuf_doubles = 0;
  double* d_scratch = nullptr;
  std::map<int, RbHostFaces> rbh;
  std::vector<DensePlan> dense;

  LevelView view() const {
    LevelView v;
    v.data = d_data;
    v.phi = d_phi;
    v.stride = stride;
    v.vstride = stride * (n + n_prox);
    v.n = n;
    v.nc = nc;
    v.h = v.hf = (nc + 1) / 2;
    v.hv = v.h * nc * nc;
    v.fs = 2 * v.hf * nc;
    for (int d = 0; d < 3; d++) {
      v.idr2[d] = 1 / (dr[d] * dr[d]);
      v.dr[d] = dr[d];
    }
    v.nbk = d_nbk;
    v.nba = d_nba;
    v.sendpos = d_sendpos;
    v.topo = d_topo;
    v.rev = 0;
    return v;
  }
  mutable int dir = 0;
  LevelView sweep_view() const {
    static const int on = getenv("OMG_NO_REV") ? 0 : 1;
    LevelView v = view();
    v.rev = dir & on;
    dir ^= 1;
    return v;
  }
};

struct PendingEv {
  const char* name;
  hipEvent_t e0, e1;
  double cells;
  int lvl;
};

struct KStat {
  long long launches = 0;
  double ms = 0, cells = 0;
};

}

struct omg_loop;
struct omg_free_state;

namespace omg {
struct TailArgs;
constexpr int kMaxSlots = 256, kMaxSlotStride = 16;
}

struct omg_ctx {
  int device = 0, rank = 0, n_ranks = 1;
  bool host_only = false;
  hipStream_t stream = nullptr;
  void* nccl = nullptr;
  std::shared_ptr<omg_loop> loop;
  std::map<int, long long> loop_seq_send, loop_seq_recv;
  long long loop_ar_seq = 0;
  int n_boxes = 0, lowest = 0, highest = 0, first_normal = 0, box_size = 0, n_vars = 4;
  std::vector<int> lvl, parent, children, neighbors, ix, rank_of;
  std::map<int, int> bsl;
  std::map<int, std::vector<double>> drl;
  std::map<int, std::vector<int>> ids, leaves, parents, ref_bnds;
  std::vector<int> local_index;
  long long rep_cells = 0;
  int rep_lvl = INT_MIN;
  std::map<int, omg::Level> levels;
  int op = omg::OP_LPL, smoother = 1, n_substeps = 1;
  int n_cycle_down = 2, n_cycle_up = 2, max_coarse_cycles = 1000;
  double lambda = 0, res_abs = 1e-8, res_rel = 1e-8;
  int subtract_mean = 0, phi_bc_data_stored = 0;
  omg::BCVar bc[omg::kMaxVars];
  std::vector<long long> h_face_off[omg::kMaxVars];
  std::vector<int> h_face_type[omg::kMaxVars];
  double* d_face_data[omg::kMaxVars] = {};
  std::map<int, long long*> d_face_off_lvl[omg::kMaxVars];
  std::map<int, int*> d_face_type_lvl[omg::kMaxVars];
  std::map<int, std::vector<long long>> h_face_off_lvl[omg::kMaxVars];
  std::map<int, std::vector<int>> h_face_type_lvl[omg::kMaxVars];
  double* d_red = nullptr;
  double* d_rhs_pend = nullptr;
  int rhs_n = 0;
  bool in_full_cycle = false;
  bool no_rhs_pend = false;
  hipStream_t stream2 = nullptr;
  hipStream_t stream_comm = nullptr;
  int comm_priority = 0;
  hipEvent_t ev_bnd = nullptr, ev_comm = nullptr;
  hipEvent_t ev_main = nullptr, ev_side = nullptr, ev_phi = nullptr;
  hipEvent_t ev_dense_in = nullptr, ev_dense_out = nullptr;
  long long dense_age = 0;
  bool phi_mean_on_side = false;
  bool no_tail = false;
  bool no_fuse_up = false;
  bool no_skip1 = false;
  bool no_fuse_down = false;
  bool no_fill_tile = false;
  bool no_fill_crhs = false;
  bool no_tail_crhs = false;
  bool no_rbgv = false;
  bool no_rb_fill_fuse = false;
  bool no_gs_plane = false;
  bool no_fill_xl = false;
  bool no_fuse_down_bc = false;
  bool no_gs_dbl = false;
  bool no_block3 = false;
  bool no_block3_phys = false;
  bool no_deep = false;
  bool no_block3p = false;
  bool block4 = true;
  bool no_block4p = false;
  bool block4_phys = false;
  bool no_defer_gc = false;
  bool no_block3r = false;
  int b3_min_boxes = omg::kB3MinBoxes;
  int b3_col_small = 2;
  int b3_col = 0;
  bool rhs_cache_valid = false;
  bool phi_shift_pending = false;
  double* d_scalar = nullptr;
  unsigned long long* d_maxslots = nullptr;
  omg::TailArgs* d_tail = nullptr;
  omg::TailArgs* h_tail = nullptr;
  bool host_xport = false;
  omg_host_exchange_fn hx_exchange = nullptr;
  omg_host_allgather_fn hx_allgather = nullptr;
  void* hx_user = nullptr;
  double* h_xsend = nullptr;
  double* h_xrecv = nullptr;
  size_t h_xsend_n = 0, h_xrecv_n = 0;
  bool tail_timing = false;
  long long* d_tail_stamps = nullptr;
  double* h_scalar = nullptr;
  double* d_stage = nullptr;
  size_t stage_n = 0;
  omg_free_state* free_state = nullptr;
  bool no_graph = true;
  bool capturing = false;
  bool max_deferred = false;
  std::map<int, hipGraphExec_t> graphs;
  int graph_fail_at = 0;
  bool profiling = false;
  bool roctx = false;
  bool debug = false;
  bool check_collective = false;
  void* rb_fn[omg::kMaxVars][6] = {};
  void* rb_user[omg::kMaxVars][6] = {};
  bool rbh_any = false;
  long long n_host_syncs = 0;
  std::map<std::string, omg::KStat> stats;
  std::vector<omg::PendingEv> pending;
};
```

octree-mg_amd/csrc/omg_kernels.h:

```cpp
#pragma once

#include "omg_internal.h"

namespace omg {

struct GcBC {
  int type[6];
  double value[6];
  const long long* face_off;
  const int* face_type;
  const double* face_data;
  int phi_stored;
};

void launch_gs_substep(const LevelView& L, int op, double lambda, int e, int colours, const LevelView& C,
                       const RBRec* rb, bool has_rb, const GcBC& bc, double* sendbuf, const double* shift,
                       hipStream_t st, const int* boxes = nullptr, int n_boxes = 0, double* rbgv = nullptr,
                       int rbgv_mode = 0);
#define OMG_FOR_OP(op, M, NC, BS)         \
  switch (op) {                           \
    case OP_HELM: M(NC, BS, OP_HELM) break;   \
    case OP_VLPL: M(NC, BS, OP_VLPL) break;   \
    case OP_VHELM: M(NC, BS, OP_VHELM) break; \
    case OP_AHELM: M(NC, BS, OP_AHELM) break; \
    default: M(NC, BS, OP_LPL) break;         \
  }

inline bool gs_tiled(int nc, int op, bool has_rb) {
  (void)op;
  (void)has_rb;
  return nc == 16 || nc == 8 || nc == 4 || nc == 2;
}
constexpr int kB3TX = 2;
constexpr int kB3S = 3 * (kB3TX + 2);
constexpr int kB3MaxZ = 16;
constexpr int kB3Rec = (1 + kB3S * (kB3MaxZ + 2) + 15) / 16 * 16;
bool gsrb3_op_ok(int op);
constexpr int kB3LenMask = 255;
struct B3Phys {
  double k[6], c1[6], c2[6];
};
void launch_gsrb4(const LevelView& L, double* dst, const int* cols, int n_cols, int op, double lambda, int e,
                  const double* shift, hipStream_t st, const LevelView* coarse = nullptr,
                  const int* ccols = nullptr, const B3Phys* phys = nullptr, bool push = true,
                  RhsShifts rs = RhsShifts());
constexpr int kB3CSlots = 9 * (kB3MaxZ / 2 + 2);
constexpr int kB3CRec = (1 + kB3CSlots + 15) / 16 * 16;
void launch_gsrb3(const LevelView& L, double* dst, const int* cols, int n_cols, int op, double lambda, int e,
                  const double* shift, hipStream_t st, bool push1 = true, const LevelView* coarse = nullptr,
                  const int* ccols = nullptr, int coarse_mode = 1, bool res = false,
                  const B3Phys* phys = nullptr);
void launch_gs_sub(const LevelView& L, int op, double lambda, int e, int colours, const LevelView& C,
                   const RBRec* rb, const GcBC& bc, double* sendbuf, hipStream_t st);
struct GhostSets {
  const double* in;
  long long in_stride;
  double* out;
  long long out_stride;
  int phys_load;
};
void launch_gs_lex(const LevelView& L, int op, double lambda, hipStream_t st, const double* rl = nullptr,
                   double* xl = nullptr, const GhostSets* gs = nullptr, const GcBC* bc = nullptr);
void launch_rbh_gather(const LevelView& L, const LevelView& C, int iv, const RBRec* rb, const int* items,
                       const int* rslot, int n, const double* rbrecv, double* cgc, double* cc, hipStream_t st);
void launch_rbh_scatter(const LevelView& L, int iv, const int* items, int n, const double* cc, hipStream_t st);
void launch_phys_gc(const LevelView& L, const GcBC& bc, const int* boxes, int n_boxes, hipStream_t st);
void launch_face_gc(const LevelView& L, const LevelView& C, const GcBC& bc, const int* boxes, int n_boxes,
                    hipStream_t st);
bool gs_lex_ring_ok(int nc, int op);
void launch_rhs_lex(const LevelView& L, double* rl, hipStream_t st);
void launch_box_op(const LevelView& L, int op, double lambda, int i_out, hipStream_t st);
void launch_residual(const LevelView& L, int op, double lambda, unsigned long long* maxbits,
                     hipStream_t st);
void launch_max_fold(unsigned long long* slots, unsigned long long* out, bool accumulate, hipStream_t st);
void launch_fill_gc(const LevelView& L, int iv, int colours, const LevelView& C, const RBRec* rb,
                    const GcBC& bc, double* sendbuf, hipStream_t st);
void launch_unpack_faces(const LevelView& L, int iv, const int* items, int n, const double* recv,
                         hipStream_t st, int colours = 3);
void launch_deep_copy(const LevelView& L, int iv, int c, int per, const int* items, int n, double* buf, bool unpack,
                      hipStream_t st);
void launch_face_pack(const LevelView& L, int iv, const int* items, int n, double* buf, hipStream_t st);
void launch_rb_pack(const LevelView& C, int iv, const int* items, int n, int nc, double* buf, hipStream_t st);
void launch_rb_unpack(const LevelView& L, int iv, const int* items, int n, const double* recv, hipStream_t st);
void launch_restrict(const LevelView& F, const LevelView& C, int iv, const int* pairs, int n_pairs,
                     const int* parent_local, const int* dixp, hipStream_t st);
void launch_restrict_pack(const LevelView& F, int iv, const int* items, int n, double* buf,
                          hipStream_t st);
void launch_box_pack(const LevelView& L, int iv, const int* items, int n, double* buf, hipStream_t st);
void launch_box_unpack(const LevelView& L, int iv, const int* items, int n, const double* buf, hipStream_t st);
void launch_restrict_unpack(const LevelView& C, int iv, const int* items, int n, int hnc,
                            const double* buf, hipStream_t st);
void launch_coarse_rhs(const LevelView& C, int op, double lambda, const int* parents, int n_par,
                       hipStream_t st);
void launch_sub_parents(const LevelView& C, const int* parents, int n_par, hipStream_t st);
void launch_prolong(const LevelView& C, const LevelView& F, int iv, int iv_to, int add, const int* pairs,
                    int n_pairs, const int* parent_local, const int* dixp, hipStream_t st);
void launch_prolong_pack(const LevelView& C, const LevelView& F, int iv, const int* items, int n,
                         double* buf, hipStream_t st);
void launch_prolong_unpack(const LevelView& F, int iv_to, int add, const int* items, int n,
                           const double* buf, hipStream_t st);
void launch_subtract(const LevelView& L, int iv, const double* mean, int ghosts, hipStream_t st);
void launch_set_rhs(const LevelView& L, const int* leaves, int n_leaves, double f1, double f2, hipStream_t st);
void launch_copy_var(const LevelView& L, int src, int dst, hipStream_t st);
void launch_from_ref(const LevelView& L, int iv, const double* ref, hipStream_t st);
void launch_to_ref(const LevelView& L, int iv, double* ref, double unstored, hipStream_t st);
void launch_poison_ghosts(const LevelView& L, int n_vars, double poison, hipStream_t st);
bool dense_row_nc(int nc);
void launch_dense_row(const LevelView& L, int iv, const DenseClip* clips, int n, double* dense, long long s1,
                      long long s2, bool put, hipStream_t st);
void launch_dense_cell(const LevelView& L, int iv, const DenseClip* clips, int n, double* dense, long long s1,
                       long long s2, bool put, hipStream_t st);
void launch_phi_bc_store(const LevelView& L, const GcBC& bc, int* nba, hipStream_t st);

constexpr int kTailMaxLevels = 12;
constexpr int kTailMaxBoxes = 1;
struct TailLevel {
  LevelView L;
  GcBC bc;
  const int* parents;
  int n_par;
  const int* parent_local;
  const int* dixp;
  int foff[6];
  signed char ftype[6];
};
struct TailArgs {
  int n_lvls;
  TailLevel lv[kTailMaxLevels];
  double lambda;
  int n_down, n_up, max_coarse;
  double res_abs, res_rel;
  unsigned long long* maxbits;
  int* coarse_its;
  int gs_lex;
  long long* stamps;
  int lds_levels, lds_top;
  int top_crhs, pad_;
};
constexpr int kTailLdsMaxLevels = 3;

void launch_coarse_tail(const TailArgs* dA, int gs_lex, int op, hipStream_t st);
void launch_store_tail(const TailArgs& A, TailArgs* d, hipStream_t st);

bool tiled_nc(int nc);
bool launch_fill_tile(const LevelView& L, const GcBC& bc, double* sendbuf, hipStream_t st);
void launch_fill_tile_xl(const LevelView& L, const GcBC& bc, double* sendbuf, const double* xl, hipStream_t st);
bool launch_smooth_resid(const LevelView& F, const LevelView& C, int op, double lambda, int restrict_on,
                         const int* parent_local, const int* dixp, hipStream_t st, const int* list,
                         int n_list, const GcBC& bc, bool has_rb, bool has_phys, const double* rbgv = nullptr);
void launch_resid_restrict(const LevelView& F, const LevelView& C, int op, double lambda,
                           unsigned long long* maxbits, int restrict_on, const int* parent_local,
                           const int* dixp, hipStream_t st, const int* list = nullptr, int n_list = 0,
                           RhsShifts rs = RhsShifts());
void launch_prolong_fill(const LevelView& C, const LevelView& F, int iv, const int* parent_local,
                         const int* dixp, const GcBC& bc, double* sendbuf, bool sub, bool skip1,
                         hipStream_t st, const int* list = nullptr, int n_list = 0, bool save_old = false,
                         const RBRec* rb = nullptr);
void launch_copy_ghosts(const LevelView& L, hipStream_t st);
void launch_prolong_smooth(const LevelView& C, const LevelView& F, int op, double lambda, const int* parent_local,
                           const int* dixp, const GcBC& bc, int one_child, const int* list, int n_list,
                           const uint8_t* push0, hipStream_t st, bool rb = false, double* rbgv = nullptr);
void launch_fill_crhs(const LevelView& C, int op, double lambda, const GcBC& bc, const uint8_t* parmask,
                      hipStream_t st);
bool launch_coarse_rhs_tile(const LevelView& C, int op, double lambda, const int* parents, int n_par,
                            hipStream_t st);
void launch_box_sums(const LevelView& L, int iv, const int* leaves, int n, double* out, hipStream_t st,
                     RhsShifts rs = RhsShifts());
bool subtract_sums_nc(int nc);
void launch_subtract_sums(const LevelView& L, int iv, const int* leaves, int n, RhsShifts rs, double* out,
                          hipStream_t st);
void launch_mean(const double* all, int n, double volume, double* mean, hipStream_t st);
void launch_seq_sum(const double* box_sums, int n, double w, double* acc, bool init, hipStream_t st);

}
```

octree-mg_amd/csrc/omg_mean.cpp:

```cpp
#include <algorithm>

#include "omg_host.h"

namespace omg {
namespace host {

static double* red_acc(omg_ctx* c, int ch) { return c->d_red + ch; }
double* red_mean(omg_ctx* c, int ch) { return c->d_red + 2 + ch; }
static double* red_all(omg_ctx* c, int ch) { return c->d_red + 8 + (size_t)ch * c->n_ranks; }

static double* leaf_scratch(Level* L, int ch) { return ch == kChRhs ? L->d_scratch_rhs : L->d_scratch; }

static void side_done(omg_ctx* c) {
  HIPCHK(hipStreamWaitEvent(c->stream, c->ev_side, 0));
  HIPCHK(hipStreamWaitEvent(c->stream, c->ev_phi, 0));
}

static void leaf_box_sums(omg_ctx* c, int iv, int ch, hipStream_t st) {
  for (int l = 1; l <= c->highest; l++) {
    Level* L = level_ptr(c, l);
    if (!L || L->leaves.empty()) continue;
    Prof p(c, "box_sums", (double)L->leaves.size() * L->nc * L->nc * L->nc, l, st);
    launch_box_sums(L->sweep_view(), iv, L->d_leaves, (int)L->leaves.size(), leaf_scratch(L, ch), st,
                    iv == 2 ? rhs_shifts(c, L) : RhsShifts());
  }
}

static void leaf_chain(omg_ctx* c, int ch, hipStream_t st) {
  double* acc = red_acc(c, ch);
  bool first = true;
  for (int l = 1; l <= c->highest; l++) {
    Level* L = level_ptr(c, l);
    if (!L || L->leaves.empty()) continue;
    Prof p(c, "seq_sum", (double)L->leaves.size(), l, st);
    launch_seq_sum(leaf_scratch(L, ch), (int)L->leaves.size(), L->dr[0] * L->dr[1] * L->dr[2], acc, first, st);
    first = false;
  }
  if (first) HIPCHK(hipMemsetAsync(acc, 0, 8, st));
}

static void leaf_sum_device(omg_ctx* c, int iv, int ch) {
  side_done(c);
  leaf_box_sums(c, iv, ch, c->stream);
  leaf_chain(c, ch, c->stream);
}

static double subtract_volume(omg_ctx* c) {
  const int nc = c->box_size;
  const auto& d1 = c->drl[1];
  return (double)(nc * nc * nc) * (d1[0] * d1[1] * d1[2]) * (double)c->ids[1].size();
}

static void mean_device(omg_ctx* c, int ch, double* mean) {
  const int n = c->n_ranks;
  if (n > 64) throw OmgError("subtract_mean: more than 64 ranks");
  double* all = red_all(c, ch);
  if (n == 1) {
    all = red_acc(c, ch);
  } else if (c->loop || c->host_xport) {
    HIPCHK(hipMemcpyAsync(c->h_scalar + 4, red_acc(c, ch), 8, hipMemcpyDeviceToHost, c->stream));
    host_sync(c, c->stream);
    std::vector<double> v = c->loop ? loop_allgather(c, c->h_scalar[4]) : host_allgather(c, c->h_scalar[4]);
    for (int r = 0; r < n; r++) c->h_scalar[8 + r] = v[r];
    HIPCHK(hipMemcpyAsync(all, c->h_scalar + 8, 8 * n, hipMemcpyHostToDevice, c->stream));
  } else {
    NCCLCHK(ncclAllGather(red_acc(c, ch), all, 1, ncclDouble, (ncclComm_t)c->nccl, c->stream));
  }
  launch_mean(all, n, subtract_volume(c), mean, c->stream);
}

double get_sum(omg_ctx* c, int iv) {
  leaf_sum_device(c, iv, kChPhi);
  HIPCHK(hipMemcpyAsync(c->h_scalar + 2, red_acc(c, kChPhi), 8, hipMemcpyDeviceToHost, c->stream));
  host_sync(c, c->stream);
  return allreduce(c, c->h_scalar[2], false);
}

void phi_mean_ready(omg_ctx* c) {
  if (!c->phi_mean_on_side) return;
  c->phi_mean_on_side = false;
  HIPCHK(hipStreamWaitEvent(c->stream, c->ev_phi, 0));
  if (c->n_ranks > 1) mean_device(c, kChPhi, red_mean(c, kChPhi));
}

void materialize_level(omg_ctx* c, Level* L) {
  if (!L->shift_pending) return;
  phi_mean_ready(c);
  L->shift_pending = false;
  rb_stale_above(c, L->lvl);
  if (L->n) {
    Prof p(c, "subtract", (double)L->n * L->nc * L->nc * L->nc, L->lvl);
    launch_subtract(L->view(), 1, red_mean(c, kChPhi), 1, c->stream);
  }
}
void materialize_phi(omg_ctx* c) {
  if (!c->phi_shift_pending) return;
  for (auto& kv : c->levels) materialize_level(c, &kv.second);
  c->phi_shift_pending = false;
}

RhsShifts rhs_shifts(omg_ctx* c, const Level* L) {
  RhsShifts r;
  r.s = c->d_rhs_pend + (c->rhs_n - L->rhs_pend);
  r.n = L->rhs_pend;
  return r;
}
void materialize_rhs(omg_ctx* c, Level* L) {
  if (!L->rhs_pend) return;
  if (c->in_full_cycle) L->rhs_pend_off = true;
  {
    Prof p(c, "subtract_rhs", (double)L->n * L->nc * L->nc * L->nc, L->lvl);
    launch_subtract_sums(L->sweep_view(), 2, L->d_leaves, L->n, rhs_shifts(c, L), nullptr, c->stream);
  }
  L->rhs_pend = 0;
  L->rhs_lex_ok = L->prox_rhs_ok = false;
}
void materialize_rhs_all(omg_ctx* c) {
  for (auto& kv : c->levels) materialize_rhs(c, &kv.second);
}
void rhs_pend_retry(omg_ctx* c) {
  for (auto& kv : c->levels) kv.second.rhs_pend_off = false;
}
static bool rhs_pend_ok(omg_ctx* c, const Level* L) {
  return c->n_ranks == 1 && c->smoother == OMG_SMOOTHER_GSRB && !c->no_rhs_pend && L->d_b3 && !L->b3_phys &&
         !L->rhs_pend_off;
}

void drop_rhs_lex(omg_ctx* c) {
  for (auto& kv : c->levels) kv.second.rhs_lex_ok = kv.second.prox_rhs_ok = false;
}
static void drop_rhs_cache(omg_ctx* c) {
  c->rhs_cache_valid = false;
  drop_rhs_lex(c);
}
void enter(omg_ctx* c, bool writes) {
  materialize_rhs_all(c);
  materialize_phi(c);
  for (auto& kv : c->levels)
    if (kv.second.gc_deferred) fill_gc_lvl(c, kv.first, 1);
  if (writes) drop_rhs_cache(c);
}

void subtract_mean(omg_ctx* c, int iv, int ghosts, int mode) {
  if (iv == 1) {
    materialize_phi(c);
    for (auto& kv : c->levels)
      if (!ghosts || kv.second.any_phys || kv.second.any_rb) kv.second.phi_gc_ok = false;
  }
  if (iv == 2 && (ghosts || mode != kInCycle)) materialize_rhs_all(c);
  if (iv == 2 && !ghosts) {
    if (c->rhs_cache_valid) {
      HIPCHK(hipStreamWaitEvent(c->stream, c->ev_side, 0));
    } else {
      leaf_sum_device(c, 2, kChRhs);
    }
    c->rhs_cache_valid = false;
    std::vector<int> prox_kept;
    for (auto& kv : c->levels)
      if (kv.second.prox_rhs_ok) prox_kept.push_back(kv.first);
    drop_rhs_lex(c);
    bool any_pend = false;
    for (auto& kv : c->levels) any_pend = any_pend || kv.second.rhs_pend > 0;
    if (!any_pend) c->rhs_n = 0;
    const bool list_full = c->rhs_n >= kRhsPendMax;
    double* mean = c->d_rhs_pend + c->rhs_n;
    mean_device(c, kChRhs, mean);
    bool all_fused = true;
    for (int l = c->lowest; l <= c->highest; l++) {
      Level* L = level_ptr(c, l);
      if (!L || !L->n) continue;
      if (mode == kInCycle && L->all_parents) continue;
      if (L->n_prox && std::count(prox_kept.begin(), prox_kept.end(), l)) {
        LevelView P = L->view();
        P.data += (long long)L->n * L->stride;
        P.phi += (long long)L->n * L->stride;
        P.n = L->n_prox;
        launch_subtract(P, 2, mean, 0, c->stream);
        L->prox_rhs_ok = true;
      }
      const double cells = (double)L->n * L->nc * L->nc * L->nc;
      if (l >= 1 && (int)L->leaves.size() == L->n && subtract_sums_nc(L->nc)) {
        RhsShifts rs = rhs_shifts(c, L);
        rs.n++;
        if (mode == kInCycle && !list_full && rhs_pend_ok(c, L)) {
          Prof p(c, "box_sums", cells, l);
          launch_box_sums(L->sweep_view(), 2, L->d_leaves, L->n, L->d_scratch_rhs, c->stream, rs);
          L->rhs_pend++;
        } else {
          Prof p(c, "subtract_rhs", cells, l);
          launch_subtract_sums(L->sweep_view(), 2, L->d_leaves, L->n, rs, L->d_scratch_rhs, c->stream);
          L->rhs_pend = 0;
        }
      } else {
        materialize_rhs(c, L);
        Prof p(c, "subtract_rhs", cells, l);
        launch_subtract(L->view(), 2, mean, 0, c->stream);
        if (l >= 1 && !L->leaves.empty()) all_fused = false;
      }
    }
    c->rhs_n = list_full ? 0 : c->rhs_n + 1;
    if (all_fused) {
      HIPCHK(hipEventRecord(c->ev_main, c->stream));
      HIPCHK(hipStreamWaitEvent(c->stream2, c->ev_main, 0));
      leaf_chain(c, kChRhs, c->stream2);
      HIPCHK(hipEventRecord(c->ev_side, c->stream2));
      c->rhs_cache_valid = true;
    }
    return;
  }
  if (iv == 2) drop_rhs_cache(c);
  const int ch = iv == 2 ? kChRhs : kChPhi;
  if (iv == 1 && ghosts && mode == kInCycle) {
    side_done(c);
    leaf_box_sums(c, 1, kChPhi, c->stream);
    HIPCHK(hipEventRecord(c->ev_main, c->stream));
    HIPCHK(hipStreamWaitEvent(c->stream2, c->ev_main, 0));
    leaf_chain(c, kChPhi, c->stream2);
    if (c->n_ranks == 1) launch_mean(red_acc(c, kChPhi), 1, subtract_volume(c), red_mean(c, kChPhi), c->stream2);
    HIPCHK(hipEventRecord(c->ev_phi, c->stream2));
    c->phi_mean_on_side = true;
    for (auto& kv : c->levels) kv.second.shift_pending = kv.second.n > 0;
    c->phi_shift_pending = true;
    return;
  }
  leaf_sum_device(c, iv, ch);
  mean_device(c, ch, red_mean(c, ch));
  for (int l = c->lowest; l <= c->highest; l++) {
    Level* L = level_ptr(c, l);
    if (L && iv == 1) L->rbgv_ok = false;
    if (L && L->n) {
      Prof p(c, "subtract", (double)L->n * L->nc * L->nc * L->nc, l);
      launch_subtract(L->view(), iv, red_mean(c, ch), ghosts, c->stream);
    }
  }
}

}
}
```

octree-mg_amd/csrc/omg_tiles.hip:

```cpp
#include <stdexcept>
#include <string>

#include "omg_face.h"
#include "omg_gsrb.h"
#include "omg_kernels.h"

namespace omg {

constexpr int kPsBS16 = 512, kPsWaves = 8;
constexpr int kSumsLPW = 32, kSumsR = 4;
constexpr bool kSumsNT = true, kSubNTLd = false, kSubNTSt = false;

template <int NC, int OP, int BS>
__device__ __forceinline__ void resid_restrict_core(const LevelView& F, const LevelView& Cv, double lambda,
                                                    unsigned long long* maxbits, int restrict_on,
                                                    const int* parent_local, const int* dixp, int b, double* sb,
                                                    const v2d* fr);

template <int NC, int OP, int BS>
__device__ __forceinline__ void resid_restrict_box(const LevelView& F, const LevelView& Cv, double lambda,
                                                   unsigned long long* maxbits, int restrict_on,
                                                   const int* parent_local, const int* dixp, int b, double* sb,
                                                   const double* __restrict__ rsh = nullptr, int n_rsh = 0) {
  using TL = Tl<NC>;
  constexpr int NST = TL::NST, HV = TL::HV, NR = (HV + BS - 1) / BS;
  const int tid = threadIdx.x;
  const long long boff = (long long)b * F.stride;
  const double* __restrict__ u = F.phi + boff;
  const double* __restrict__ f = F.data + F.vstride + boff;
  for (int q = tid; q < NST / 2; q += BS) reinterpret_cast<v2d*>(sb)[q] = ld_nt(u + 2 * q);
  v2d fr[NR];
#pragma unroll
  for (int r = 0; r < NR; r++) {
    const int q2 = tid + BS * r;
    if (q2 < HV) fr[r] = ld_nt(f + 2 * q2);
  }
  if (n_rsh) {
    const RhsSub rsub(rsh, n_rsh);
#pragma unroll
    for (int r = 0; r < NR; r++)
      if (tid + BS * r < HV) {
        double a = fr[r].x, b2 = fr[r].y;
        rsub(a, b2);
        fr[r].x = a;
        fr[r].y = b2;
      }
  }
  __syncthreads();
  resid_restrict_core<NC, OP, BS>(F, Cv, lambda, maxbits, restrict_on, parent_local, dixp, b, sb, fr);
}

template <int NC, int OP, int BS>
__device__ __forceinline__ void resid_restrict_core(const LevelView& F, const LevelView& Cv, double lambda,
                                                    unsigned long long* maxbits, int restrict_on,
                                                    const int* parent_local, const int* dixp, int b, double* sb,
                                                    const v2d* fr) {
  using TL = Tl<NC>;
  constexpr int HV = TL::HV, FH = TL::FH, FS = TL::FS, NR = (HV + BS - 1) / BS, HN = NC / 2;
  const int tid = threadIdx.x;
  double* __restrict__ res = F.data + 3 * F.vstride + (long long)b * F.stride;

  const OpCoef<OP> K(F, lambda);
  double mx = 0.0;
  double2 rv[NR];
#pragma unroll
  for (int r = 0; r < NR; r++) {
    const int q2 = tid + BS * r;
    if (q2 >= HV) continue;
    const int e = q2 >= HV / 2, o = 1 - e;
    Nbr7 s0, s1;
    if constexpr (HN % 2 == 0) {
      pair_stencil<NC>(sb + o * HV, sb + 2 * HV + o * FH, FS, e, 2 * q2 - e * HV, s0, s1);
    } else {
      int i, j, k;
      TL::decode(2 * q2, i, j, k);
      s0.xm = sb[TL::ocell(i - 1, j, k)]; s0.xp = sb[TL::ocell(i + 1, j, k)];
      s0.ym = sb[TL::ocell(i, j - 1, k)]; s0.yp = sb[TL::ocell(i, j + 1, k)];
      s0.zm = sb[TL::ocell(i, j, k - 1)]; s0.zp = sb[TL::ocell(i, j, k + 1)];
      TL::decode(2 * q2 + 1, i, j, k);
      s1.xm = sb[TL::ocell(i - 1, j, k)]; s1.xp = sb[TL::ocell(i + 1, j, k)];
      s1.ym = sb[TL::ocell(i, j - 1, k)]; s1.yp = sb[TL::ocell(i, j + 1, k)];
      s1.zm = sb[TL::ocell(i, j, k - 1)]; s1.zp = sb[TL::ocell(i, j, k + 1)];
    }
    const double2 cc = reinterpret_cast<const double2*>(sb)[q2];
    s0.c = cc.x;
    s1.c = cc.y;
    double l0, l1;
    op_pair<NC, OP>(K, F, b, e, 2 * q2 - e * HV, s0, s1, l0, l1);
    const double r0 = fr[r].x - l0, r1 = fr[r].y - l1;
    mx = amax(mx, amax(fabs(r0), fabs(r1)));
    rv[r] = make_double2(r0, r1);
    st_nt(res + 2 * q2, r0, r1);
  }
  if (maxbits) launch_max<BS>(maxbits, mx);
  if (!restrict_on || parent_local[b] < 0) return;

  const int pb = parent_local[b], dp = dixp[b];
  const int dx = dp & 1023, dy = (dp >> 10) & 1023, dz = dp >> 20;
  const long long poff = (long long)pb * Cv.stride;
  for (int pass = 0; pass < 2; pass++) {
    double* __restrict__ dst = pass == 0 ? Cv.phi + poff : Cv.data + 3 * Cv.vstride + poff;
    for (int q = tid; q < HN * HN * HN; q += BS) {
      const int i = q % HN + 1, j = (q / HN) % HN + 1, k = q / (HN * HN) + 1;
      double acc = 0.0;
#pragma unroll
      for (int kk = 0; kk < 2; kk++)
#pragma unroll
        for (int jj = 0; jj < 2; jj++)
#pragma unroll
          for (int ii = 0; ii < 2; ii++) acc += sb[TL::oint(2 * i - 1 + ii, 2 * j - 1 + jj, 2 * k - 1 + kk)];
      dst[off_int(Cv, dx + i, dy + j, dz + k)] = 0.125 * acc;
    }
    if (pass == 0) {
      __syncthreads();
#pragma unroll
      for (int r = 0; r < NR; r++) {
        const int q2 = tid + BS * r;
        if (q2 < HV) reinterpret_cast<double2*>(sb)[q2] = rv[r];
      }
      __syncthreads();
    }
  }
}

template <int NC, int OP, int BS>
__global__ void __launch_bounds__(BS) k_resid_restrict(LevelView F, LevelView Cv, double lambda,
                                                       unsigned long long* maxbits, int restrict_on,
                                                       const int* parent_local, const int* dixp,
                                                       const int* list, const double* __restrict__ rsh,
                                                       int n_rsh) {
  __shared__ double sb[Tl<NC>::NST];
  const int q = xcd_box(blockIdx.x, gridDim.x, F.rev);
  resid_restrict_box<NC, OP, BS>(F, Cv, lambda, maxbits, restrict_on, parent_local, dixp, list ? list[q] : q, sb,
                                 rsh, n_rsh);
}

template <int NC>
__device__ __forceinline__ int sr_int(int d, int v, int a, int c) {
  return d == 0 ? Tl<NC>::oint(v, a, c) : (d == 1 ? Tl<NC>::oint(a, v, c) : Tl<NC>::oint(a, c, v));
}
template <int NC>
__device__ __forceinline__ int sr_edge(int d, int t, bool lo, int nl, int a, int c) {
  const int t1 = d == 0 ? 1 : 0, t2 = d == 2 ? 1 : 2, ax = t == 0 ? t1 : t2;
  const int fn = 2 * ax + (lo ? 1 : 2);
  const int i = d == 0 ? nl : a, j = d == 1 ? nl : (d == 0 ? a : c), k = d == 2 ? nl : c;
  return ax == 0 ? Tl<NC>::ogh(fn, j, k) : (ax == 1 ? Tl<NC>::ogh(fn, i, k) : Tl<NC>::ogh(fn, i, j));
}

__device__ __forceinline__ v2d sr_ld(const double* p) { return *reinterpret_cast<const v2d*>(p); }

template <int NC, int OP, int BS, int BCK = 0>
__global__ void __launch_bounds__(BS) k_smooth_resid(LevelView F, LevelView Cv, double lambda, int restrict_on,
                                                     const int* parent_local, const int* dixp,
                                                     const int* list, GcBC bc, const double* __restrict__ rbgv) {
  using TL = Tl<NC>;
  constexpr int H = NC / 2, HV = TL::HV, FH = TL::FH, FS = TL::FS, NR = (HV + BS - 1) / BS;
  constexpr int NG = (6 * FH + BS - 1) / BS;
  __shared__ double sb[TL::NST];
  const int tid = threadIdx.x, bq = xcd_box(blockIdx.x, gridDim.x, F.rev), b = list ? list[bq] : bq;
  const FaceTopo T = load_topo(F, b);
  const long long boff = (long long)b * F.stride;
  double* __restrict__ u = F.phi + boff;
  const double* __restrict__ f = F.data + F.vstride + boff;
  v2d fr[NR];
  auto bulk_loads = [&]() {
    for (int q = tid; q < HV / 2; q += BS)
      reinterpret_cast<v2d*>(sb + HV)[q] = sr_ld(u + HV + 2 * q);
    for (int q = tid; q < 3 * FH; q += BS) {
      const int nb = q / (FH / 2), r = q % (FH / 2);
      reinterpret_cast<v2d*>(sb + 2 * HV + nb * FS + FH)[r] = sr_ld(u + 2 * HV + nb * FS + FH + 2 * r);
    }
#pragma unroll
    for (int r = 0; r < NR; r++) {
      const int q2 = tid + BS * r;
      if (q2 < HV) fr[r] = sr_ld(f + 2 * q2);
    }
  };
  double gdeep[NG] = {}, grhs[NG] = {}, gedge[NG][2] = {};
#pragma unroll
  for (int g = 0; g < NG; g++) {
    const int p = tid + BS * g;
    if (p >= 6 * FH) continue;
    const int nb = p / FH + 1, hi = p % FH, ah = hi % H, c = hi / H + 1;
    if (BCK && T.kind(nb - 1) != NB_LOCAL) continue;
    const bool low = nb & 1;
    const int gl = low ? 0 : NC + 1, a = 2 * ah + 1 + ((gl + 1 + c) & 1);
    const int d = (nb - 1) >> 1, nl = low ? NC : 1;
    const long long noff = (long long)T.arg(nb - 1) * F.stride;
    const double* un = F.phi + noff;
    gdeep[g] = un[sr_int<NC>(d, low ? NC - 1 : 2, a, c)];
    grhs[g] = F.data[F.vstride + noff + sr_int<NC>(d, nl, a, c)];
    gedge[g][0] = gedge[g][1] = 0.0;
    const bool ea = a == 1 || a == NC, ec = c == 1 || c == NC;
    if (ea) gedge[g][0] = un[sr_edge<NC>(d, 0, a == 1, nl, a, c)];
    if (ec) {
      const double e = un[sr_edge<NC>(d, 1, c == 1, nl, a, c)];
      if (ea) gedge[g][1] = e; else gedge[g][0] = e;
    }
  }
  constexpr int NF = 6 * NC * NC, NPF = (NF + BS - 1) / BS;
  RbCoarse rt[BCK == 2 ? NPF : 1];
  if constexpr (BCK == 2) {
    if (T.nonlocal()) {
#pragma unroll
      for (int r = 0; r < NPF; r++) {
        const int p = tid + BS * r;
        if (p >= NF) continue;
        const int f = p / (NC * NC), cell = p % (NC * NC);
        if (T.kind(f) != NB_RB) continue;
        if (rbgv)
          rt[r].tc = rbgv[((long long)b * 6 + f) * (NC * NC) + cell];
        else
          rt[r] = rb_coarse_load(F, RbSide{Cv, nullptr}, rb_unpack(F, T.arg(f)), f + 1, cell % NC + 1, cell / NC + 1);
      }
    }
  }
  bulk_loads();
  __syncthreads();

  const OpCoef<OP> K(F, lambda);
#pragma unroll
  for (int r = 0; r < NR; r++) {
    const int q2 = tid + BS * r;
    if (q2 >= HV / 2) continue;
    Nbr7 s0, s1;
    pair_stencil<NC>(sb + HV, sb + 2 * HV + FH, FS, 0, 2 * q2, s0, s1);
    const double v0 = gs_value<OP>(K, s0, fr[r].x), v1 = gs_value<OP>(K, s1, fr[r].y);
    reinterpret_cast<double2*>(sb)[q2] = make_double2(v0, v1);
    st_nt(u + 2 * q2, v0, v1);
  }
  if (BCK && T.nonlocal()) __syncthreads();
#pragma unroll
  for (int g = 0; g < NG; g++) {
    const int p = tid + BS * g;
    if (p >= 6 * FH) continue;
    const int nb = p / FH + 1, hi = p % FH, ah = hi % H, c = hi / H + 1;
    const bool low = nb & 1;
    const int gl = low ? 0 : NC + 1, a = 2 * ah + 1 + ((gl + 1 + c) & 1);
    const int d = (nb - 1) >> 1;
    if (BCK && T.kind(nb - 1) != NB_LOCAL) continue;
    const double across = sb[sr_int<NC>(d, low ? 1 : NC, a, c)];
    const bool ea = a == 1 || a == NC;
    const double dm = low ? gdeep[g] : across, dp = low ? across : gdeep[g];
    const double am = a == 1 ? gedge[g][0] : sb[TL::ogh(nb, a - 1, c)];
    const double ap = a == NC ? gedge[g][0] : sb[TL::ogh(nb, a + 1, c)];
    const double ce = ea ? gedge[g][1] : gedge[g][0];
    const double cm = c == 1 ? ce : sb[TL::ogh(nb, a, c - 1)];
    const double cp = c == NC ? ce : sb[TL::ogh(nb, a, c + 1)];
    Nbr7 s;
    s.xm = d == 0 ? dm : am;
    s.xp = d == 0 ? dp : ap;
    s.ym = d == 1 ? dm : (d == 0 ? am : cm);
    s.yp = d == 1 ? dp : (d == 0 ? ap : cp);
    s.zm = d == 2 ? dm : cm;
    s.zp = d == 2 ? dp : cp;
    sb[2 * HV + (nb - 1) * FS + hi] = gs_value<OP>(K, s, grhs[g]);
  }
  if (BCK && T.nonlocal()) {
#pragma unroll
    for (int r = 0; r < NPF; r++) {
      const int p = tid + BS * r;
      if (p >= NF) continue;
      const int f = p / (NC * NC), cell = p % (NC * NC), nb = f + 1, kind = T.kind(f);
      if (kind == NB_LOCAL) continue;
      const int a = cell % NC + 1, c = cell / NC + 1, d = f >> 1;
      const bool low = nb & 1;
      const double x1 = sb[sr_int<NC>(d, low ? 1 : NC, a, c)], x2 = sb[sr_int<NC>(d, low ? 2 : NC - 1, a, c)];
      const int gi = TL::ogh(nb, a, c);
      double gv = 0.0;
      if (kind == NB_PHYS)
        gv = phys_ghost(F, bc, b, (long long)b * 6 + f, nb, T.phys_code(f), a, c, gi, x1, x2);
      else if constexpr (BCK == 2)
        if (kind == NB_RB) gv = rb_ghost_gv(rbgv ? rt[r].tc : rb_gv(rt[r], a, c), x1, x2);
      sb[gi] = gv;
      if (gi < 2 * HV + f * FS + FH) u[gi] = gv;
    }
  }
  __syncthreads();
  face_push_local<NC>(F, T, 1, [&](int i, int j, int k) { return sb[TL::oint(i, j, k)]; });
  resid_restrict_core<NC, OP, BS>(F, Cv, lambda, nullptr, restrict_on, parent_local, dixp, b, sb, fr);
}

template <int NC>
constexpr int prolong_cb() { return ((NC / 2 + 2) * (NC / 2 + 2) * (NC / 2 + 2) + 1) & ~1; }

template <int NC, int BS, bool SUB, bool EDGES = false>
__device__ __forceinline__ void load_parent_octant(const LevelView& Cv, int iv, int pb, int dx, int dy, int dz,
                                                   double* cb) {
  auto ld = [](const double* p) { return *p; };
  constexpr int CB = NC / 2 + 2, N = CB * CB * CB, NQ = (N + BS - 1) / BS;
  const int tid = threadIdx.x;
  const int n1 = Cv.nc + 1;
  double rv[NQ];
  int off[NQ];
  unsigned store = 0;
#pragma unroll
  for (int r = 0; r < NQ; r++) {
    const int q = tid + BS * r;
    off[r] = -1;
    if (q >= N) continue;
    const int p = q % CB, s = (q / CB) % CB, t = q / (CB * CB);
    const int nbnd = (p == 0 || p == CB - 1) + (s == 0 || s == CB - 1) + (t == 0 || t == CB - 1);
    const int x = dx + p, y = dy + s, z = dz + t;
    const int nghost = (x == 0 || x == n1) + (y == 0 || y == n1) + (z == 0 || z == n1);
    if (EDGES ? (nbnd == 3 || nghost >= 2) : nbnd >= 2) continue;
    const int o = off_cell(Cv, x, y, z);
    off[r] = o;
    if (SUB) {
      rv[r] = ld(boxp(Cv, 1, pb) + o) - ld(boxp(Cv, 3, pb) + o);
      if (nbnd == 0 || (nbnd == 1 && nghost)) store |= 1u << r;
    } else {
      rv[r] = ld(boxp(Cv, iv, pb) + o);
    }
  }
#pragma unroll
  for (int r = 0; r < NQ; r++) {
    if (off[r] < 0) continue;
    cb[tid + BS * r] = rv[r];
    if (SUB && (store >> r & 1)) boxp(Cv, 4, pb)[off[r]] = rv[r];
  }
}

template <int NC, int BS, bool SUB, bool RB = false>
__device__ __forceinline__ void prolong_fill_box(const LevelView& Cv, const LevelView& F, int iv,
                                                 const int* parent_local, const int* dixp, const GcBC& bc,
                                                 double* sendbuf, int b, double* lds, bool skip1,
                                                 bool save_old = false, const RBRec* rb = nullptr) {
  using TL = Tl<NC>;
  constexpr int HV = TL::HV, NR = (HV + BS - 1) / BS, HN = NC / 2, CB = HN + 2;
  double* cb = lds;
  double* sb = lds + prolong_cb<NC>();
  const int tid = threadIdx.x;
  const FaceTopo T = load_topo(F, b);
  const int pb = parent_local[b], dp = dixp[b];
  const int dx = dp & 1023, dy = (dp >> 10) & 1023, dz = dp >> 20;
  const bool only0 = skip1 && !T.nonlocal();
  const int npair = only0 ? HV / 2 : HV;
  double* __restrict__ u = F.phi + (long long)b * F.stride;
  v2d old[NR];
#pragma unroll
  for (int r = 0; r < NR; r++) {
    const int q2 = tid + BS * r;
    if (q2 < npair) old[r] = ld_nt(u + 2 * q2);
  }
  load_parent_octant<NC, BS, SUB>(Cv, iv, pb, dx, dy, dz, cb);
  __syncthreads();
#pragma unroll
  for (int r = 0; r < NR; r++) {
    const int q2 = tid + BS * r;
    if (q2 >= npair) continue;
    double nv[2];
#pragma unroll
    for (int s = 0; s < 2; s++) {
      const int q = 2 * q2 + s;
      int i, j, k;
      TL::decode(q, i, j, k);
      const int ic = (i + 1) >> 1, jc = (j + 1) >> 1, kc = (k + 1) >> 1;
      const int c0 = ic + CB * (jc + CB * kc);
      const double f0 = 0.25 * cb[c0];
      const double fx = 0.25 * cb[(i & 1) ? c0 - 1 : c0 + 1];
      const double fy = 0.25 * cb[(j & 1) ? c0 - CB : c0 + CB];
      const double fz = 0.25 * cb[(k & 1) ? c0 - CB * CB : c0 + CB * CB];
      const double o = s ? old[r].y : old[r].x;
      nv[s] = o + (f0 + fx + fy + fz);
      sb[q] = nv[s];
    }
    st_nt(u + 2 * q2, nv[0], nv[1]);
    if (save_old) st_nt(F.data + 2 * F.vstride + (long long)b * F.stride + 2 * q2, old[r].x, old[r].y);
  }
  __syncthreads();
  if constexpr (RB) {
    const RbSide rbs{Cv, rb};
    tile_face_fill<NC>(F, b, T, sb, only0 ? 1 : 3, bc, sendbuf,
                       [&](int arg, int nb, int a, int c, double v1, double v2) {
                         return rb_ghost(F, rbs, arg, nb, a, c, v1, v2);
                       });
  } else {
    tile_face_fill<NC>(F, b, T, sb, only0 ? 1 : 3, bc, sendbuf);
  }
}

template <int NC, int BS, bool SUB, bool RB = false>
__global__ void __launch_bounds__(BS) k_prolong_fill(LevelView Cv, LevelView F, int iv,
                                                     const int* parent_local, const int* dixp, GcBC bc,
                                                     double* sendbuf, int skip1, const int* list, int save_old,
                                                     const RBRec* rb) {
  __shared__ double lds[prolong_cb<NC>() + Tl<NC>::HV * 2];
  const int t = xcd_box(blockIdx.x, gridDim.x, F.rev);
  prolong_fill_box<NC, BS, SUB, RB>(Cv, F, iv, parent_local, dixp, bc, sendbuf, list ? list[t] : t, lds,
                                    skip1 != 0, save_old != 0, rb);
}

template <int NC>
__device__ __forceinline__ double prolong_at(const LevelView& Cv, int pc, const int dix[3], int fi, int fj,
                                             int fk) {
  const int ic = ((fi + 1) >> 1) + dix[0], jc = ((fj + 1) >> 1) + dix[1], kc = ((fk + 1) >> 1) + dix[2];
  const double* ph = boxp(Cv, 1, pc);
  const double* ol = boxp(Cv, 3, pc);
  auto r = [&](int x, int y, int z) {
    const int o = off_cell(Cv, x, y, z);
    return ph[o] - ol[o];
  };
  const double f0 = 0.25 * r(ic, jc, kc);
  const double fx = 0.25 * r((fi & 1) ? ic - 1 : ic + 1, jc, kc);
  const double fy = 0.25 * r(ic, (fj & 1) ? jc - 1 : jc + 1, kc);
  const double fz = 0.25 * r(ic, jc, (fk & 1) ? kc - 1 : kc + 1);
  return f0 + fx + fy + fz;
}

template <int NC>
constexpr int prolong_smooth_lds() {
  return 2 * Tl<NC>::HV + (prolong_cb<NC>() > 6 * Tl<NC>::FH ? prolong_cb<NC>() : 6 * Tl<NC>::FH);
}

template <int NC, int OP, int BS, bool RB = false>
__device__ __forceinline__ void prolong_smooth_box(const LevelView& Cv, const LevelView& F, double lambda,
                                                   const int* parent_local, const int* dixp, const GcBC& bc,
                                                   int one_child, const uint8_t* push0, int b, double* lds,
                                                   double* rbgv = nullptr) {
  using TL = Tl<NC>;
  constexpr int HV = TL::HV, FH = TL::FH, NR = (HV + BS - 1) / BS, HN = NC / 2, CB = HN + 2;
  double* sb = lds;
  double* sg = lds + 2 * HV;
  double* cb = sg;
  const int tid = threadIdx.x;
  const FaceTopo T = load_topo(F, b);
  const int pb = parent_local[b], dp = dixp[b];
  const int dix[3] = {dp & 1023, (dp >> 10) & 1023, dp >> 20};
  bool phys = false;
#pragma unroll
  for (int nb = 0; nb < 6; nb++) phys |= T.kind(nb) == NB_PHYS || (RB && T.kind(nb) == NB_RB);
  const int npair = phys ? HV : HV / 2;
  constexpr int NR0 = (HV / 2 + BS - 1) / BS;
  double* __restrict__ u = F.phi + (long long)b * F.stride;
  v2d old[NR0];
#pragma unroll
  for (int r = 0; r < NR0; r++) {
// ... 139 lines not shown
        gv[g] = rb_ghost(F, RbSide{Cv, nullptr}, T.arg(nb - 1), nb, a, c, v1, v2);
    }
    sg[(nb - 1) * FH + rr] = gv[g];
  }
  __syncthreads();
  const RbSide rbs{Cv, nullptr, rbgv, rbgv ? 1 : 0};
  gsrb_box<NC, OP, BS, 2, true, RB>(F, lambda, 1, 2, bc, nullptr, nullptr, b, lds, nullptr, RB ? &rbs : nullptr);
}

template <int NC, int OP, int BS, bool RB = false>
__global__ void __launch_bounds__(BS, RB ? 4 : kPsWaves) k_prolong_smooth(LevelView Cv, LevelView F, double lambda,
                                                       const int* parent_local, const int* dixp, GcBC bc,
                                                       int one_child, const int* list, const uint8_t* push0,
                                                       double* rbgv) {
  __shared__ double lds[prolong_smooth_lds<NC>()];
  const int t = xcd_box(blockIdx.x, gridDim.x, F.rev);
  prolong_smooth_box<NC, OP, BS, RB>(Cv, F, lambda, parent_local, dixp, bc, one_child, push0, list ? list[t] : t,
                                     lds, rbgv);
}

void launch_prolong_smooth(const LevelView& C, const LevelView& F, int op, double lambda, const int* parent_local,
                           const int* dixp, const GcBC& bc, int one_child, const int* list, int n_list,
                           const uint8_t* push0, hipStream_t st, bool rb, double* rbgv) {
  const int n = list ? n_list : F.n;
  if (n == 0) return;
  const dim3 g(n);
  if (rb) {
    if (F.nc != 16 && F.nc != 8) throw std::runtime_error("launch_prolong_smooth: refinement boundaries need 16^3 / 8^3");
#define OMG_PSR(NC, BS)                                                                                         \
  if (op == OP_HELM)                                                                                            \
    k_prolong_smooth<NC, OP_HELM, BS, true><<<g, BS, 0, st>>>(C, F, lambda, parent_local, dixp, bc, one_child, \
                                                              list, push0, rbgv);                               \
  else                                                                                                          \
    k_prolong_smooth<NC, OP_LPL, BS, true><<<g, BS, 0, st>>>(C, F, lambda, parent_local, dixp, bc, one_child,  \
                                                             list, push0, rbgv);
    if (F.nc == 16) OMG_PSR(16, kPsBS16) else OMG_PSR(8, 256)
#undef OMG_PSR
    return;
  }
#define OMG_PS(NC, BS)                                                                                \
  if (op == OP_HELM)                                                                                  \
    k_prolong_smooth<NC, OP_HELM, BS><<<g, BS, 0, st>>>(C, F, lambda, parent_local, dixp, bc, one_child, \
                                                        list, push0, nullptr);                        \
  else                                                                                                \
    k_prolong_smooth<NC, OP_LPL, BS><<<g, BS, 0, st>>>(C, F, lambda, parent_local, dixp, bc, one_child,  \
                                                       list, push0, nullptr);
  switch (F.nc) {
    case 16: OMG_PS(16, kPsBS16) break;
    case 8: OMG_PS(8, 256) break;
    case 4: OMG_PS(4, 256) break;
    default: OMG_PS(2, 256) break;
  }
#undef OMG_PS
}

template <bool NT>
__device__ __forceinline__ double2 sums_ld(const double* p) {
  if (NT) {
    const v2d t = ld_nt(p);
    return make_double2(t.x, t.y);
  }
  return *reinterpret_cast<const double2*>(p);
}
template <bool NT>
__device__ __forceinline__ void sums_st(double* p, double2 v) {
  if (NT)
    st_nt(p, v.x, v.y);
  else
    *reinterpret_cast<double2*>(p) = v;
}

template <int NC, bool SUB, bool SH = SUB, int LPW = kSumsLPW>
__global__ void __launch_bounds__(64) k_box_sums3(LevelView L, int iv, const int* __restrict__ leaves,
                                                  int n_leaves, double* __restrict__ out,
                                                  const double* __restrict__ shifts, int n_sh) {
  constexpr int H = NC / 2, R = kSumsR < NC ? kSumsR : NC, SEG = R * H;
  constexpr bool NTL = SUB ? kSubNTLd : kSumsNT;
  constexpr int CH2 = SEG;
  constexpr int PER = LPW * CH2 / 64;
  constexpr int P = 2 * SEG + 1;
  constexpr int NCH = NC * NC / R;
  __shared__ double lds[LPW * P];
  const int lane = threadIdx.x, b0 = (L.rev ? gridDim.x - 1 - blockIdx.x : blockIdx.x) * LPW;
  const long long hv = L.hv;
  double* src[PER];
  int dst[PER];
  bool own[PER];
#pragma unroll
  for (int r = 0; r < PER; r++) {
    const int t = lane + 64 * r, bb = t / CH2, w = t % CH2, seg = w / (SEG / 2), off = w % (SEG / 2);
    const int q = min(b0 + bb, n_leaves - 1);
    own[r] = b0 + bb < n_leaves;
    src[r] = boxp(L, iv, leaves[q]) + seg * hv + 2 * off;
    dst[r] = bb * P + seg * SEG + 2 * off;
  }
  static_assert(SH || !SUB, "k_box_sums3: the storing form subtracts");
  const RhsSub rsub(shifts, SH ? n_sh : 0);
  double2 va[PER], vb[PER];
  auto chunk_off = [](int c) { return H * (((c % (NC / R)) * R) + NC * (c / (NC / R))); };
#pragma unroll
  for (int r = 0; r < PER; r++) va[r] = sums_ld<NTL>(src[r]);
#pragma unroll
  for (int r = 0; r < PER; r++) vb[r] = sums_ld<NTL>(src[r] + chunk_off(1));
  double acc = 0.0;
  const double* my = lds + lane * P;
  auto process = [&](double2* v, int c) {
    __syncthreads();
    const int rc = chunk_off(c);
#pragma unroll
    for (int r = 0; r < PER; r++) {
      if (SH) rsub(v[r].x, v[r].y);
      if (SUB && own[r]) sums_st<kSubNTSt>(src[r] + rc, v[r]);
      lds[dst[r]] = v[r].x;
      lds[dst[r] + 1] = v[r].y;
    }
    __syncthreads();
    if (c + 2 < NCH) {
      const int r2 = chunk_off(c + 2);
#pragma unroll
      for (int r = 0; r < PER; r++) v[r] = sums_ld<NTL>(src[r] + r2);
    }
    const int k = c / (NC / R) + 1, j0 = (c % (NC / R)) * R + 1;
    if (lane < LPW) {
#pragma unroll
      for (int rr = 0; rr < R; rr++) {
        const int ca = (1 + j0 + rr + k) & 1;
        const double* A = my + ca * SEG + rr * H;
        const double* B = my + (1 - ca) * SEG + rr * H;
#pragma unroll
        for (int q = 0; q < H; q++) {
          acc += A[q];
          acc += B[q];
        }
      }
    }
  };
  static_assert(NCH % 2 == 0, "chunks come in pairs");
  for (int c = 0; c < NCH; c += 2) {
    process(va, c);
    process(vb, c + 1);
  }
  if (out && lane < LPW && b0 + lane < n_leaves) out[b0 + lane] = acc;
}

__global__ void __launch_bounds__(64) k_box_sums_any(LevelView L, int iv, const int* leaves, int n_leaves,
                                                     double* out) {
  const int q = blockIdx.x * 64 + threadIdx.x;
  if (q >= n_leaves) return;
  const double* u = boxp(L, iv, leaves[q]);
  double acc = 0.0;
  for (int k = 1; k <= L.nc; k++)
    for (int j = 1; j <= L.nc; j++)
      for (int i = 1; i <= L.nc; i++) acc += u[off_int(L, i, j, k)];
  out[q] = acc;
}

__global__ void __launch_bounds__(64) k_seq_sum3(const double* __restrict__ box_sums, int n, double w,
                                                 double* __restrict__ acc, int init) {
  constexpr int CH = 1024, PL = CH / 128, G = 16;
  __shared__ double st[CH];
  const int lane = threadIdx.x;
  double a = init ? 0.0 : *acc;
  double2 pre[PL];
  auto fetch = [&](int base) {
#pragma unroll
    for (int r = 0; r < PL; r++) {
      const int q = base + 2 * (lane + 64 * r);
      pre[r].x = q < n ? box_sums[q] : 0.0;
      pre[r].y = q + 1 < n ? box_sums[q + 1] : 0.0;
    }
  };
  fetch(0);
  for (int base = 0; base < n; base += CH) {
    __syncthreads();
#pragma unroll
    for (int r = 0; r < PL; r++) reinterpret_cast<double2*>(st)[lane + 64 * r] = pre[r];
    __syncthreads();
    if (base + CH < n) fetch(base + CH);
    const int m = min(CH, n - base);
    if (m == CH) {
      double cur[G], nxt[G];
#pragma unroll
      for (int t = 0; t < G; t++) cur[t] = st[t];
      for (int g = 0; g < CH / G; g++) {
        const int gn = g + 1 < CH / G ? g + 1 : g;
#pragma unroll
        for (int t = 0; t < G; t++) nxt[t] = st[G * gn + t];
        double p[G];
#pragma unroll
        for (int t = 0; t < G; t++) p[t] = w * cur[t];
#pragma unroll
        for (int t = 0; t < G; t++) a = a + p[t];
#pragma unroll
        for (int t = 0; t < G; t++) cur[t] = nxt[t];
      }
    } else {
      for (int q = 0; q < m; q++) a = a + w * st[q];
    }
  }
  if (lane == 0) *acc = a;
}

template <int NC, int BS>
__global__ void __launch_bounds__(BS) k_fill_tile(LevelView L, GcBC bc, double* sendbuf) {
  constexpr int HV = Tl<NC>::HV;
  __shared__ double sb[2 * HV];
  const int b = xcd_box(blockIdx.x, gridDim.x, L.rev);
  const FaceTopo T = load_topo(L, b);
  const double* u = L.phi + (long long)b * L.stride;
  for (int q = threadIdx.x; q < HV; q += BS) reinterpret_cast<v2d*>(sb)[q] = reinterpret_cast<const v2d*>(u)[q];
  __syncthreads();
  tile_face_fill<NC>(L, b, T, sb, 3, bc, sendbuf);
}

template <int NC, int BS>
__global__ void __launch_bounds__(BS) k_fill_tile_xl(LevelView L, GcBC bc, double* sendbuf,
                                                     const double* __restrict__ xl) {
  using TL = Tl<NC>;
  constexpr int HV = TL::HV, H = NC / 2, FH = H * NC;
  __shared__ double sb[2 * HV];
  const int b = xcd_box(blockIdx.x, gridDim.x, L.rev);
  const FaceTopo T = load_topo(L, b);
  const double* u = L.phi + (long long)b * L.stride;
  bool phys = false;
#pragma unroll
  for (int nb = 0; nb < 6; nb++) phys |= T.kind(nb) == NB_PHYS;
  if (phys) {
    for (int q = threadIdx.x; q < HV; q += BS) reinterpret_cast<v2d*>(sb)[q] = reinterpret_cast<const v2d*>(u)[q];
  } else {
    const int t = threadIdx.x;
    for (int q = t; q < 2 * FH; q += BS) {
      const int e = q / FH, w = q % FH, pl = w / (FH / 2), r2 = w % (FH / 2);
      const int off = e * HV + (pl ? FH * (NC - 1) : 0) + 2 * r2;
      *reinterpret_cast<v2d*>(sb + off) = *reinterpret_cast<const v2d*>(u + off);
    }
    for (int q = t; q < 4 * NC * (H / 2); q += BS) {
      const int r2 = q % (H / 2), row = q / (H / 2), k = row % NC, jj = (row / NC) & 1, e = row / (2 * NC);
      const int off = e * HV + H * ((jj ? NC - 1 : 0) + NC * k) + 2 * r2;
      *reinterpret_cast<v2d*>(sb + off) = *reinterpret_cast<const v2d*>(u + off);
    }
    const double* xb = xl + (long long)b * 512;
    for (int q = t; q < 2 * NC * NC; q += BS) {
      const int f = q / (NC * NC), c = q % (NC * NC), j = c % NC + 1, k = c / NC + 1;
      sb[TL::oint(f ? NC : 1, j, k)] = xb[q];
    }
  }
  __syncthreads();
  tile_face_fill<NC>(L, b, T, sb, 3, bc, sendbuf);
}

void launch_fill_tile_xl(const LevelView& L, const GcBC& bc, double* sendbuf, const double* xl, hipStream_t st) {
  if (L.n == 0) return;
  if (L.nc != 16) throw std::runtime_error("launch_fill_tile_xl: 16^3 boxes only");
  k_fill_tile_xl<16, 512><<<L.n, 512, 0, st>>>(L, bc, sendbuf, xl);
}

bool launch_fill_tile(const LevelView& L, const GcBC& bc, double* sendbuf, hipStream_t st) {
  if (L.n == 0) return true;
  const dim3 g(L.n);
  switch (L.nc) {
    case 16: k_fill_tile<16, 512><<<g, 512, 0, st>>>(L, bc, sendbuf); return true;
    case 8: k_fill_tile<8, 256><<<g, 256, 0, st>>>(L, bc, sendbuf); return true;
    case 4: k_fill_tile<4, 64><<<g, 64, 0, st>>>(L, bc, sendbuf); return true;
    default: return false;
  }
}

bool launch_smooth_resid(const LevelView& F, const LevelView& C, int op, double lambda, int restrict_on,
                         const int* parent_local, const int* dixp, hipStream_t st, const int* list,
                         int n_list, const GcBC& bc, bool has_rb, bool has_phys, const double* rbgv) {
  if (op != OP_LPL && op != OP_HELM) return false;
  if (!has_rb) rbgv = nullptr;
  const int n = list ? n_list : F.n;
  if (n == 0) return true;
  const dim3 g(n);
#define OMG_SR_RB(NC, BS, RB)                                                                                    \
  if (op == OP_LPL)                                                                                              \
    k_smooth_resid<NC, OP_LPL, BS, RB><<<g, BS, 0, st>>>(F, C, lambda, restrict_on, parent_local, dixp, list, bc,   \
                                                         rbgv);                                                   \
  else                                                                                                           \
    k_smooth_resid<NC, OP_HELM, BS, RB><<<g, BS, 0, st>>>(F, C, lambda, restrict_on, parent_local, dixp, list, bc,  \
                                                          rbgv);
#define OMG_SR(NC, BS)           \
  if (has_rb) {                  \
    OMG_SR_RB(NC, BS, 2)         \
  } else if (has_phys) {         \
    OMG_SR_RB(NC, BS, 1)         \
  } else {                       \
    OMG_SR_RB(NC, BS, 0)         \
  }
  switch (F.nc) {
    case 16: OMG_SR(16, 512) return true;
    case 8: OMG_SR(8, 256) return true;
    default: return false;
  }
#undef OMG_SR
#undef OMG_SR_RB
}

bool tiled_nc(int nc) { return nc == 16 || nc == 8 || nc == 4 || nc == 2; }

void launch_resid_restrict(const LevelView& F, const LevelView& C, int op, double lambda,
                           unsigned long long* maxbits, int restrict_on, const int* parent_local,
                           const int* dixp, hipStream_t st, const int* list, int n_list, RhsShifts rs) {
  const int n = list ? n_list : F.n;
  if (n == 0) return;
  if (rs.n < 0 || rs.n > kRhsPendMax || (rs.n && !rs.s))
    throw std::runtime_error("launch_resid_restrict: at most kRhsPendMax pending rhs shifts");
  const dim3 g(n);
#define OMG_RR_OP(NC, BS, OPV)                                                                                  \
  k_resid_restrict<NC, OPV, BS><<<g, dim3(BS), 0, st>>>(F, C, lambda, maxbits, restrict_on, parent_local, dixp, \
                                                        list, rs.s, rs.n);
#define OMG_RR(NC, BS) OMG_FOR_OP(op, OMG_RR_OP, NC, BS)
  switch (F.nc) {
    case 16: OMG_RR(16, 512) break;
    case 8: OMG_RR(8, 256) break;
    case 4: OMG_RR(4, 256) break;
    default: OMG_RR(2, 256) break;
  }
#undef OMG_RR
#undef OMG_RR_OP
}

void launch_prolong_fill(const LevelView& C, const LevelView& F, int iv, const int* parent_local,
                         const int* dixp, const GcBC& bc, double* sendbuf, bool sub, bool skip1,
                         hipStream_t st, const int* list, int n_list, bool save_old, const RBRec* rb) {
  const int n = list ? n_list : F.n;
  if (n == 0) return;
  const dim3 g(n);
  const int so = save_old && !skip1;
#define OMG_PF(NC, BS)                                                                                              \
  if (rb && sub)                                                                                                    \
    k_prolong_fill<NC, BS, true, true><<<g, BS, 0, st>>>(C, F, iv, parent_local, dixp, bc, sendbuf, skip1, list, so, rb); \
  else if (rb)                                                                                                      \
    k_prolong_fill<NC, BS, false, true><<<g, BS, 0, st>>>(C, F, iv, parent_local, dixp, bc, sendbuf, skip1, list, so, rb); \
  else if (sub)                                                                                                     \
    k_prolong_fill<NC, BS, true><<<g, BS, 0, st>>>(C, F, iv, parent_local, dixp, bc, sendbuf, skip1, list, so, rb); \
  else                                                                                                              \
    k_prolong_fill<NC, BS, false><<<g, BS, 0, st>>>(C, F, iv, parent_local, dixp, bc, sendbuf, skip1, list, so, rb);
  switch (F.nc) {
    case 16: OMG_PF(16, 512) break;
    case 8: OMG_PF(8, 256) break;
    case 4: OMG_PF(4, 256) break;
    default: OMG_PF(2, 256) break;
  }
#undef OMG_PF
}

template <int NC, int OP, int BS, bool NT = false>
__device__ __forceinline__ void coarse_rhs_box(const LevelView& Cv, double lambda, int b, double* sb) {
  using TL = Tl<NC>;
  constexpr int HV = TL::HV, FH = TL::FH, FS = TL::FS, NR = (HV + BS - 1) / BS, H = NC / 2;
  constexpr int NST = TL::NST;
  const int tid = threadIdx.x;
  const long long boff = (long long)b * Cv.stride;
  const double* __restrict__ u = Cv.phi + boff;
  double* __restrict__ rhs = Cv.data + Cv.vstride + boff;
  double* __restrict__ old = Cv.data + 2 * Cv.vstride + boff;
  const double* __restrict__ res = Cv.data + 3 * Cv.vstride + boff;
  for (int q = tid; q < NST / 2; q += BS) {
    const v2d x = NT ? ld_nt(u + 2 * q) : reinterpret_cast<const v2d*>(u)[q];
    reinterpret_cast<v2d*>(sb)[q] = x;
    if (NT)
      st_nt(old + 2 * q, x.x, x.y);
    else
      reinterpret_cast<v2d*>(old)[q] = x;
  }
  v2d rr[NR];
#pragma unroll
  for (int r = 0; r < NR; r++) {
    const int q2 = tid + BS * r;
    if (q2 < HV) rr[r] = NT ? ld_nt(res + 2 * q2) : reinterpret_cast<const v2d*>(res)[q2];
  }
  __syncthreads();
  const OpCoef<OP> K(Cv, lambda);
#pragma unroll
  for (int r = 0; r < NR; r++) {
    const int q2 = tid + BS * r;
    if (q2 >= HV) continue;
    const int e = q2 >= HV / 2, o = 1 - e;
    Nbr7 s0, s1;
    if constexpr (H % 2 == 0) {
      pair_stencil<NC>(sb + o * HV, sb + 2 * HV + o * FH, FS, e, 2 * q2 - e * HV, s0, s1);
    } else {
      int i, j, k;
      TL::decode(2 * q2, i, j, k);
      s0.xm = sb[TL::ocell(i - 1, j, k)]; s0.xp = sb[TL::ocell(i + 1, j, k)];
      s0.ym = sb[TL::ocell(i, j - 1, k)]; s0.yp = sb[TL::ocell(i, j + 1, k)];
      s0.zm = sb[TL::ocell(i, j, k - 1)]; s0.zp = sb[TL::ocell(i, j, k + 1)];
      TL::decode(2 * q2 + 1, i, j, k);
      s1.xm = sb[TL::ocell(i - 1, j, k)]; s1.xp = sb[TL::ocell(i + 1, j, k)];
      s1.ym = sb[TL::ocell(i, j - 1, k)]; s1.yp = sb[TL::ocell(i, j + 1, k)];
      s1.zm = sb[TL::ocell(i, j, k - 1)]; s1.zp = sb[TL::ocell(i, j, k + 1)];
    }
    const double2 cc = reinterpret_cast<const double2*>(sb)[q2];
    s0.c = cc.x;
    s1.c = cc.y;
    double l0, l1;
    op_pair<NC, OP>(K, Cv, b, e, 2 * q2 - e * HV, s0, s1, l0, l1);
    v2d out;
    out.x = l0 + rr[r].x;
    out.y = l1 + rr[r].y;
    if (NT)
      st_nt(rhs + 2 * q2, out.x, out.y);
    else
      reinterpret_cast<v2d*>(rhs)[q2] = out;
  }
}

template <int NC, int OP, int BS>
__global__ void __launch_bounds__(BS) k_fill_crhs(LevelView C, double lambda, GcBC bc,
                                                  const uint8_t* __restrict__ parmask) {
  using TL = Tl<NC>;
  constexpr int HV = TL::HV, NST = TL::NST, FH = TL::FH, NR = (HV + BS - 1) / BS, H = NC / 2;
  __shared__ double sb[NST];
  const int tid = threadIdx.x, b = xcd_box(blockIdx.x, gridDim.x, C.rev);
  const FaceTopo T = load_topo(C, b);
  const long long boff = (long long)b * C.stride;
  const double* __restrict__ u = C.phi + boff;
  const bool par = parmask[b] != 0;
  for (int q = tid; q < HV; q += BS) reinterpret_cast<v2d*>(sb)[q] = reinterpret_cast<const v2d*>(u)[q];
  v2d rr[NR];
  if (par) {
    for (int p = tid; p < 6 * NC * NC; p += BS) {
      const int f = p / (NC * NC), cell = p % (NC * NC);
      if (T.kind(f) != NB_LOCAL) continue;
      const int nb = f + 1, a = cell % NC + 1, c = cell / NC + 1, d = f >> 1;
      const bool low = nb & 1;
      sb[TL::ogh(nb, a, c)] = C.phi[(long long)T.arg(f) * C.stride + sr_int<NC>(d, low ? NC : 1, a, c)];
    }
    const double* __restrict__ res = C.data + 3 * C.vstride + boff;
#pragma unroll
    for (int r = 0; r < NR; r++) {
      const int q2 = tid + BS * r;
      if (q2 < HV) rr[r] = ld_nt(res + 2 * q2);
    }
  }
  __syncthreads();
  tile_face_fill<NC>(C, b, T, sb, 3, bc, nullptr);
  if (!par) return;
  if (T.nonlocal()) {
    for (int p = tid; p < 6 * NC * NC; p += BS) {
      const int f = p / (NC * NC), cell = p % (NC * NC);
      if (T.kind(f) != NB_PHYS) continue;
      const int nb = f + 1, a = cell % NC + 1, c = cell / NC + 1, d = f >> 1;
      const bool low = nb & 1;
      const int gi = TL::ogh(nb, a, c);
      sb[gi] = phys_ghost(C, bc, b, (long long)b * 6 + f, nb, T.phys_code(f), a, c, gi,
                          sb[sr_int<NC>(d, low ? 1 : NC, a, c)], sb[sr_int<NC>(d, low ? 2 : NC - 1, a, c)]);
    }
  }
  __syncthreads();
  double* __restrict__ old = C.data + 2 * C.vstride + boff;
  double* __restrict__ rhs = C.data + C.vstride + boff;
  for (int q = tid; q < NST / 2; q += BS) {
    const v2d x = reinterpret_cast<const v2d*>(sb)[q];
    st_nt(old + 2 * q, x.x, x.y);
  }
  const OpCoef<OP> K(C, lambda);
  constexpr int FS = TL::FS;
#pragma unroll
  for (int r = 0; r < NR; r++) {
    const int q2 = tid + BS * r;
    if (q2 >= HV) continue;
    const int e = q2 >= HV / 2, o = 1 - e;
    Nbr7 s0, s1;
    if constexpr (H % 2 == 0) {
      pair_stencil<NC>(sb + o * HV, sb + 2 * HV + o * FH, FS, e, 2 * q2 - e * HV, s0, s1);
    } else {
      int i, j, k;
      TL::decode(2 * q2, i, j, k);
      s0.xm = sb[TL::ocell(i - 1, j, k)]; s0.xp = sb[TL::ocell(i + 1, j, k)];
      s0.ym = sb[TL::ocell(i, j - 1, k)]; s0.yp = sb[TL::ocell(i, j + 1, k)];
      s0.zm = sb[TL::ocell(i, j, k - 1)]; s0.zp = sb[TL::ocell(i, j, k + 1)];
      TL::decode(2 * q2 + 1, i, j, k);
      s1.xm = sb[TL::ocell(i - 1, j, k)]; s1.xp = sb[TL::ocell(i + 1, j, k)];
      s1.ym = sb[TL::ocell(i, j - 1, k)]; s1.yp = sb[TL::ocell(i, j + 1, k)];
      s1.zm = sb[TL::ocell(i, j, k - 1)]; s1.zp = sb[TL::ocell(i, j, k + 1)];
    }
    const double2 cc = reinterpret_cast<const double2*>(sb)[q2];
    s0.c = cc.x;
    s1.c = cc.y;
    double l0, l1;
    op_pair<NC, OP>(K, C, b, e, 2 * q2 - e * HV, s0, s1, l0, l1);
    st_nt(rhs + 2 * q2, l0 + rr[r].x, l1 + rr[r].y);
  }
}

void launch_fill_crhs(const LevelView& C, int op, double lambda, const GcBC& bc, const uint8_t* parmask,
                      hipStream_t st) {
  if (C.n == 0) return;
  const dim3 g(C.n);
#define OMG_FC_OP(NC, BS, OPV) k_fill_crhs<NC, OPV, BS><<<g, BS, 0, st>>>(C, lambda, bc, parmask);
#define OMG_FC(NC, BS) OMG_FOR_OP(op, OMG_FC_OP, NC, BS)
  switch (C.nc) {
    case 16: OMG_FC(16, 512) break;
    case 8: OMG_FC(8, 256) break;
    case 4: OMG_FC(4, 64) break;
    default: throw std::runtime_error("launch_fill_crhs: box sizes 16, 8, 4");
  }
#undef OMG_FC
#undef OMG_FC_OP
}

template <int NC, int OP, int BS>
__global__ void __launch_bounds__(BS) k_coarse_rhs_tile(LevelView Cv, double lambda, const int* parents) {
  __shared__ double sb[Tl<NC>::NST];
  coarse_rhs_box<NC, OP, BS, true>(Cv, lambda, parents[xcd_box(blockIdx.x, gridDim.x, Cv.rev)], sb);
}

bool launch_coarse_rhs_tile(const LevelView& C, int op, double lambda, const int* parents, int n_par,
                            hipStream_t st) {
  if (!tiled_nc(C.nc)) return false;
  if (n_par == 0) return true;
  const dim3 g(n_par);
#define OMG_CR_OP(NC, BS, OPV) k_coarse_rhs_tile<NC, OPV, BS><<<g, BS, 0, st>>>(C, lambda, parents);
#define OMG_CR(NC, BS) OMG_FOR_OP(op, OMG_CR_OP, NC, BS)
  switch (C.nc) {
    case 16: OMG_CR(16, 512) break;
    case 8: OMG_CR(8, 256) break;
    case 4: OMG_CR(4, 256) break;
    default: OMG_CR(2, 256) break;
  }
#undef OMG_CR
#undef OMG_CR_OP
  return true;
}

static void check_shifts(const RhsShifts& rs, const char* who) {
  if (rs.n < 0 || rs.n > kRhsPendMax + 1 || (rs.n && !rs.s))
    throw std::runtime_error(std::string(who) + ": at most kRhsPendMax + 1 shifts");
}

void launch_box_sums(const LevelView& L, int iv, const int* leaves, int n, double* out, hipStream_t st,
                     RhsShifts rs) {
  if (n == 0) return;
  check_shifts(rs, "launch_box_sums");
  if (rs.n && !subtract_sums_nc(L.nc)) throw std::runtime_error("launch_box_sums: shifts need a 16 / 8 / 4 box");
  const dim3 g((n + kSumsLPW - 1) / kSumsLPW);
  switch (L.nc) {
#define OMG_BS(NC)                                                                         \
  if (rs.n) k_box_sums3<NC, false, true><<<g, 64, 0, st>>>(L, iv, leaves, n, out, rs.s, rs.n); \
  else k_box_sums3<NC, false, false><<<g, 64, 0, st>>>(L, iv, leaves, n, out, nullptr, 0);
    case 16: OMG_BS(16) break;
    case 8: OMG_BS(8) break;
    case 4: OMG_BS(4) break;
#undef OMG_BS
    default: k_box_sums_any<<<(n + 63) / 64, 64, 0, st>>>(L, iv, leaves, n, out); break;
  }
}

bool subtract_sums_nc(int nc) { return nc == 16 || nc == 8 || nc == 4; }

void launch_subtract_sums(const LevelView& L, int iv, const int* leaves, int n, RhsShifts rs, double* out,
                          hipStream_t st) {
  if (n == 0) return;
  check_shifts(rs, "launch_subtract_sums");
  const dim3 g((n + kSumsLPW - 1) / kSumsLPW);
  switch (L.nc) {
    case 16: k_box_sums3<16, true><<<g, 64, 0, st>>>(L, iv, leaves, n, out, rs.s, rs.n); break;
    case 8: k_box_sums3<8, true><<<g, 64, 0, st>>>(L, iv, leaves, n, out, rs.s, rs.n); break;
    case 4: k_box_sums3<4, true><<<g, 64, 0, st>>>(L, iv, leaves, n, out, rs.s, rs.n); break;
    default: throw std::runtime_error("launch_subtract_sums: box size must be 16, 8 or 4");
  }
}

__global__ void k_mean(const double* all, int n, double volume, double* mean) {
  __shared__ double t[64];
  if (threadIdx.x || blockIdx.x) return;
  for (int r = 0; r < n; r++) t[r] = all[r];
  for (int w = 1; w < n; w *= 2)
    for (int r = 0; r + w < n; r += 2 * w) t[r] = t[r] + t[r + w];
  *mean = t[0] / volume;
}

void launch_mean(const double* all, int n, double volume, double* mean, hipStream_t st) {
  k_mean<<<1, 64, 0, st>>>(all, n, volume, mean);
}

void launch_seq_sum(const double* box_sums, int n, double w, double* acc, bool init, hipStream_t st) {
  if (n == 0) return;
  k_seq_sum3<<<1, 64, 0, st>>>(box_sums, n, w, acc, init);
}

constexpr int kTailBS = 512;
template <bool LEX>
constexpr int tail_lds() {
  return LEX && gs_lex_lds<16>() > Tl<16>::NST ? gs_lex_lds<16>() : Tl<16>::NST;
}

__device__ void tail_fill(const TailArgs& A, int li);

template <int OP, bool LEX>
__device__ void tail_smooth(const TailArgs& A, int li, int n_cycle, double* lds) {
  const TailLevel& T = A.lv[li];
  if constexpr (LEX) {
    for (int n = 1; n <= n_cycle; n++) {
      for (int b = 0; b < T.L.n; b++) {
        switch (T.L.nc) {
          case 16: gs_lex_box<OP, 16>(T.L, A.lambda, b, lds); break;
          case 8: gs_lex_box<OP, 8>(T.L, A.lambda, b, lds); break;
          case 4: gs_lex_box<OP, 4>(T.L, A.lambda, b, lds); break;
          default: gs_lex_box<OP, 2>(T.L, A.lambda, b, lds); break;
        }
      }
      tail_fill(A, li);
    }
    return;
  }
  for (int n = 1; n <= 2 * n_cycle; n++) {
    const int e = n & 1;
    for (int b = 0; b < T.L.n; b++) {
      switch (T.L.nc) {
        case 16: gsrb_box<16, OP, kTailBS, 0>(T.L, A.lambda, e, 1 << e, T.bc, nullptr, nullptr, b, lds); break;
        case 8: gsrb_box<8, OP, kTailBS, 0>(T.L, A.lambda, e, 1 << e, T.bc, nullptr, nullptr, b, lds); break;
// ... 839 lines not shown
```

Before: 38.32 billion cell-updates/s.

## Defer top-level residual store in fused resid-restrict until it is actually needed

On the finest level of a full V-cycle, the fused residual+restriction kernel can now skip writing the residual field and mark it as pending, with the source phi buffer recorded. The residual is recomputed lazily (materialize_res) only if something reads it or is about to overwrite its source buffer, via hooks placed before every phi write and at API entry points. This saves one full-grid residual store per cycle on the largest level. The cost is extra bookkeeping and a risk of a missed hook leaving a stale residual, plus a possible recompute if a later read occurs.

```diff
diff --git a/octree-mg_amd/csrc/omg_api.cpp b/octree-mg_amd/csrc/omg_api.cpp
--- a/octree-mg_amd/csrc/omg_api.cpp
+++ b/octree-mg_amd/csrc/omg_api.cpp
@@ -290,6 +290,7 @@
     c->block4_phys = env_flag("OMG_BLOCK4_PHYS");
     c->no_defer_gc = env_flag("OMG_NO_DEFER_GC");
     c->no_rhs_pend = env_flag("OMG_NO_RHS_PEND");
+    c->no_res_pend = env_flag("OMG_NO_RES_PEND");
     c->no_fuse_down_bc = env_flag("OMG_NO_FUSE_DOWN_BC");
     c->roctx = env_flag("OMG_ROCTX");
     c->debug = env_flag("OMG_DEBUG");
diff --git a/octree-mg_amd/csrc/omg_cycle.cpp b/octree-mg_amd/csrc/omg_cycle.cpp
--- a/octree-mg_amd/csrc/omg_cycle.cpp
+++ b/octree-mg_amd/csrc/omg_cycle.cpp
@@ -91,6 +91,7 @@
   Level* L = level_ptr(c, lvl);
   if (!L) return;
   if (iv == 1) {
+    res_before_write(c, L, L->d_phi);
     L->phi_gc_ok = true;
     L->gc_deferred = false;
     rb_stale_above(c, lvl);
@@ -168,6 +169,7 @@
                       !L->has_rb && gs_tiled(L->nc, c->op, L->has_rb) && !(L->d_b3 && L->b3_phys);
   if (L->shift_pending && !absorb) materialize_level(c, L);
   if (c->smoother != OMG_SMOOTHER_GSRB) {
+    if (n_sub >= 1) res_before_write(c, L, L->d_phi);
     materialize_rhs(c, L);
     const bool ring = n_sub >= 1 && L->d_rhs_lex && gs_lex_ring_ok(L->nc, c->op);
     if (ring && !L->rhs_lex_ok) {
@@ -227,6 +229,7 @@
     const bool b3 = b3_usable(c, lvl, P3, ph);
     if (four && (n_sub - n + 1) % 4 == 0 && b3 && (!ph || c->block4_phys)) {
       double* other = L->d_phi == L->d_data ? L->d_phi_buf : L->d_data;
+      res_before_write(c, L, other);
       deep_before(c, L, 1 - e);
       if (ph) materialize_rhs(c, L);
       {
@@ -244,6 +247,7 @@
       double* other = L->d_phi == L->d_data ? L->d_phi_buf : L->d_data;
       const bool push1 = L->deep || !(skip_last == 1 && n + 2 == n_sub && e == 1);
       const bool res = want_res && n + 2 == n_sub && push1;
+      res_before_write(c, L, other);
       materialize_rhs(c, L);
       deep_before(c, L, 1 - e);
       {
@@ -260,6 +264,7 @@
       continue;
     }
     if (L->gc_deferred) fill_gc_lvl(c, lvl, 1);
+    res_before_write(c, L, L->d_phi);
     materialize_rhs(c, L);
     if (L->n_bnd && L->n_int && !odd && gs_tiled(L->nc, c->op, L->has_rb)) {
       const int gvm = L->d_rbgv ? (L->rbgv_ok ? 2 : 1) : 0;
@@ -304,9 +309,32 @@
   return L && tiled_nc(L->nc);
 }
 
+void materialize_res(omg_ctx* c, Level* L) {
+  if (!L->res_pend) return;
+  L->res_pend = false;
+  if (!L->n) return;
+  LevelView V = L->sweep_view();
+  V.phi = L->res_src;
+  Prof p(c, "residual", (double)L->n * L->nc * L->nc * L->nc, L->lvl);
+  launch_resid_restrict(V, empty_view(), c->op, c->lambda, nullptr, 0, nullptr, nullptr, c->stream, nullptr, 0,
+                        rhs_shifts(c, L));
+}
+void materialize_res_all(omg_ctx* c) {
+  for (auto& kv : c->levels) materialize_res(c, &kv.second);
+}
+void res_before_write(omg_ctx* c, Level* L, const double* buf) {
+  if (!L || !L->res_pend || L->res_src != buf) return;
+  if (c->in_full_cycle) L->res_pend_off = true;
+  materialize_res(c, L);
+}
+static bool res_pend_ok(omg_ctx* c, const Level* L) {
+  return c->n_ranks == 1 && !c->capturing && !c->no_res_pend && L->n && tiled_level(c, L) && !L->res_pend_off;
+}
+
 void residual_lvl(omg_ctx* c, int lvl, unsigned long long* maxbits) {
   Level* L = level_ptr(c, lvl);
   if (!L || L->n == 0) return;
+  L->res_pend = false;
   if (!tiled_level(c, L)) materialize_rhs(c, L);
   Prof p(c, "residual", (double)L->n * L->nc * L->nc * L->nc, lvl);
   if (tiled_level(c, L))
@@ -348,6 +376,7 @@
 void restrict_lvl(omg_ctx* c, int iv, int lvl) {
   if (lvl <= c->lowest) throw OmgError("cannot restrict lvl <= lowest_lvl");
   if (iv == 1) phi_dirty(c, lvl - 1);
+  if (Level* Cl = level_ptr(c, lvl - 1); Cl && iv == 1) res_before_write(c, Cl, Cl->d_phi);
   Level* F = level_ptr(c, lvl);
   restrict_remote(c, iv, lvl);
   if (F && F->n_pairs) {
@@ -363,6 +392,7 @@
   if (iv_to == 1) phi_dirty(c, lvl + 1);
   Level* F = level_ptr(c, lvl + 1);
   Level* C = level_ptr(c, lvl);
+  if (iv_to == 1) res_before_write(c, F, F->d_phi);
   const LevelView FV = view_of(c, lvl + 1), CV = view_of(c, lvl);
   if (c->n_ranks > 1 && F && C && (F->prol.n_send || F->prol.n_recv)) {
     launch_prolong_pack(CV, FV, iv, F->prol.d_send_items, F->prol.n_send, C->d_sendbuf, c->stream);
@@ -391,10 +421,12 @@
          !F->any_rbx;
 }
 
-void update_coarse(omg_ctx* c, int lvl, bool fused, bool tail_crhs) {
+void update_coarse(omg_ctx* c, int lvl, bool fused, bool tail_crhs, bool res_may_pend) {
   Level* F = level_ptr(c, lvl);
+  if (F) F->res_pend = false;
   if (Level* Cl = level_ptr(c, lvl - 1)) {
     Cl->rhs_lex_ok = Cl->prox_rhs_ok = false;
+    materialize_res(c, Cl);
     if (Cl->all_parents) Cl->shift_pending = false;
     else materialize_level(c, Cl);
     materialize_rhs(c, Cl);
@@ -452,9 +484,12 @@
                               F->d_dix, c->stream, F->d_bnd, F->n_bnd, rhs_shifts(c, F));
       }
     } else {
+      const bool pend = res_may_pend && res_pend_ok(c, F);
       Prof p(c, "resid_restrict", (double)F->n * F->nc * F->nc * F->nc, lvl);
       launch_resid_restrict(F->sweep_view(), view_of(c, lvl - 1), c->op, c->lambda, nullptr, 1, F->d_parent_local,
-                            F->d_dix, c->stream, nullptr, 0, rhs_shifts(c, F));
+                            F->d_dix, c->stream, nullptr, 0, rhs_shifts(c, F), !pend);
+      F->res_pend = pend;
+      F->res_src = pend ? F->d_phi : nullptr;
     }
     restrict_remote(c, 1, lvl);
     restrict_remote(c, 4, lvl);
@@ -506,6 +541,7 @@
       (c->n_ranks > 1 && (F->prol.n_send || F->prol.n_recv)))
     return false;
   if (F->shift_pending) materialize_level(c, F);
+  res_before_write(c, F, F->d_phi);
   materialize_rhs(c, F);
   rb_stale_above(c, lvl + 1);
   const bool split = F->has_remote;
@@ -549,6 +585,7 @@
   if (F->shift_pending) materialize_level(c, F);
   rb_stale_above(c, l);
   double* other = F->d_phi == F->d_data ? F->d_phi_buf : F->d_data;
+  res_before_write(c, F, other);
   const LevelView cv = C->view();
   int done = 3;
   deep_before(c, F, 0);
@@ -585,6 +622,7 @@
   Level* C = level_ptr(c, lvl);
   if (save_old && (then_gsrb || !correct_fill_fused(c, lvl)))
     throw OmgError("internal: old = phi fused into an unfused correction");
+  if (F) res_before_write(c, F, F->d_phi);
   rb_stale_above(c, lvl + 1);
   if (correct_fill_fused(c, lvl)) {
     const bool sub = (size_t)F->n == 8 * C->parents.size() || C->nc * 2 == F->nc;
@@ -722,6 +760,14 @@
   const bool has_highest = highest_lvl >= c->lowest;
   const int min_lvl = c->lowest, max_lvl = has_highest ? highest_lvl : c->highest;
   const bool full = standalone && !has_highest;
+  {
+    const int tt = tail_top(c, max_lvl);
+    const bool top_updates = full && max_lvl > min_lvl && !(tt >= min_lvl && !c->no_tail && max_lvl <= tt);
+    for (auto& kv : c->levels) {
+      if (top_updates && kv.first == max_lvl) kv.second.res_pend = false;
+      else materialize_res(c, &kv.second);
+    }
+  }
   if (c->phi_shift_pending) {
     if (!full) {
       materialize_phi(c);
@@ -765,7 +811,7 @@
     const bool fused = !four && smooth_resid_ok(c, l);
     smooth_boxes(c, l, c->n_cycle_down, 1, fused ? 1 : 0, false, four, four);
     if (Level* Fd = level_ptr(c, l); Fd && Fd->gc_deferred) fill_gc_lvl(c, l, 1);
-    update_coarse(c, l, fused, tail_crhs && l == top + 1);
+    update_coarse(c, l, fused, tail_crhs && l == top + 1, full && l == max_lvl);
     faces_join(c, level_ptr(c, l));
   }
   if (tail) {
@@ -814,6 +860,7 @@
 }
 
 double fas_fmg(omg_ctx* c, bool have_guess, bool want_max_res) {
+  materialize_res_all(c);
   materialize_rhs_all(c);
   if (have_guess) {
     materialize_phi(c);
@@ -871,6 +918,7 @@
 
 double run_cycle(omg_ctx* c, int key, const std::function<double()>& body) {
   if (!graph_ok(c)) return body();
+  materialize_res_all(c);
   std::map<int, double*> phi_at_start;
   for (auto& kv : c->levels) phi_at_start[kv.first] = kv.second.d_phi;
   c->capturing = true;
@@ -933,6 +981,7 @@
     throw OmgError("vlaplacian/vhelmholtz_set_methods: mg%n_extra_vars == 0");
   if (op == OMG_VLAPLACIAN) lambda = 0.0;
   const bool changed = c->op != op;
+  if ((changed || lambda != c->lambda) && !c->host_only) materialize_res_all(c);
   if (changed) rhs_pend_retry(c);
   c->op = op;
   c->lambda = lambda;
diff --git a/octree-mg_amd/csrc/omg_host.h b/octree-mg_amd/csrc/omg_host.h
--- a/octree-mg_amd/csrc/omg_host.h
+++ b/octree-mg_amd/csrc/omg_host.h
@@ -226,7 +226,10 @@
 double max_residual_lvl(omg_ctx* c, int lvl);
 void restrict_lvl(omg_ctx* c, int iv, int lvl);
 void prolong(omg_ctx* c, int lvl, int iv, int iv_to, int add);
-void update_coarse(omg_ctx* c, int lvl, bool fused = false, bool tail_crhs = false);
+void update_coarse(omg_ctx* c, int lvl, bool fused = false, bool tail_crhs = false, bool res_may_pend = false);
+void materialize_res(omg_ctx* c, Level* L);
+void materialize_res_all(omg_ctx* c);
+void res_before_write(omg_ctx* c, Level* L, const double* buf);
 void correct_children(omg_ctx* c, int lvl);
 void check_finite_res(double r, const char* where);
 double fas_vcycle(omg_ctx* c, int highest_lvl, bool want_max_res, bool standalone);
diff --git a/octree-mg_amd/csrc/omg_internal.h b/octree-mg_amd/csrc/omg_internal.h
--- a/octree-mg_amd/csrc/omg_internal.h
+++ b/octree-mg_amd/csrc/omg_internal.h
@@ -137,6 +137,9 @@
   bool shift_pending = false;
   int rhs_pend = 0;
   bool rhs_pend_off = false;
+  bool res_pend = false;
+  double* res_src = nullptr;
+  bool res_pend_off = false;
   int8_t* d_nbk = nullptr;
   int* d_nba = nullptr;
   int* d_sendpos = nullptr;
@@ -284,6 +287,7 @@
   int rhs_n = 0;
   bool in_full_cycle = false;
   bool no_rhs_pend = false;
+  bool no_res_pend = false;
   hipStream_t stream2 = nullptr;
   hipStream_t stream_comm = nullptr;
   int comm_priority = 0;
diff --git a/octree-mg_amd/csrc/omg_kernels.h b/octree-mg_amd/csrc/omg_kernels.h
--- a/octree-mg_amd/csrc/omg_kernels.h
+++ b/octree-mg_amd/csrc/omg_kernels.h
@@ -151,7 +151,7 @@
 void launch_resid_restrict(const LevelView& F, const LevelView& C, int op, double lambda,
                            unsigned long long* maxbits, int restrict_on, const int* parent_local,
                            const int* dixp, hipStream_t st, const int* list = nullptr, int n_list = 0,
-                           RhsShifts rs = RhsShifts());
+                           RhsShifts rs = RhsShifts(), bool store = true);
 void launch_prolong_fill(const LevelView& C, const LevelView& F, int iv, const int* parent_local,
                          const int* dixp, const GcBC& bc, double* sendbuf, bool sub, bool skip1,
                          hipStream_t st, const int* list = nullptr, int n_list = 0, bool save_old = false,
diff --git a/octree-mg_amd/csrc/omg_mean.cpp b/octree-mg_amd/csrc/omg_mean.cpp
--- a/octree-mg_amd/csrc/omg_mean.cpp
+++ b/octree-mg_amd/csrc/omg_mean.cpp
@@ -85,6 +85,7 @@
 
 void materialize_level(omg_ctx* c, Level* L) {
   if (!L->shift_pending) return;
+  res_before_write(c, L, L->d_phi);
   phi_mean_ready(c);
   L->shift_pending = false;
   rb_stale_above(c, L->lvl);
@@ -119,7 +120,7 @@
   for (auto& kv : c->levels) materialize_rhs(c, &kv.second);
 }
 void rhs_pend_retry(omg_ctx* c) {
-  for (auto& kv : c->levels) kv.second.rhs_pend_off = false;
+  for (auto& kv : c->levels) kv.second.rhs_pend_off = kv.second.res_pend_off = false;
 }
 static bool rhs_pend_ok(omg_ctx* c, const Level* L) {
   return c->n_ranks == 1 && c->smoother == OMG_SMOOTHER_GSRB && !c->no_rhs_pend && L->d_b3 && !L->b3_phys &&
@@ -134,6 +135,7 @@
   drop_rhs_lex(c);
 }
 void enter(omg_ctx* c, bool writes) {
+  materialize_res_all(c);
   materialize_rhs_all(c);
   materialize_phi(c);
   for (auto& kv : c->levels)
@@ -142,6 +144,7 @@
 }
 
 void subtract_mean(omg_ctx* c, int iv, int ghosts, int mode) {
+  if (mode != kInCycle) materialize_res_all(c);
   if (iv == 1) {
     materialize_phi(c);
     for (auto& kv : c->levels)
diff --git a/octree-mg_amd/csrc/omg_tiles.hip b/octree-mg_amd/csrc/omg_tiles.hip
--- a/octree-mg_amd/csrc/omg_tiles.hip
+++ b/octree-mg_amd/csrc/omg_tiles.hip
@@ -11,13 +11,13 @@
 constexpr int kSumsLPW = 32, kSumsR = 4;
 constexpr bool kSumsNT = true, kSubNTLd = false, kSubNTSt = false;
 
-template <int NC, int OP, int BS>
+template <int NC, int OP, int BS, bool STORE = true>
 __device__ __forceinline__ void resid_restrict_core(const LevelView& F, const LevelView& Cv, double lambda,
                                                     unsigned long long* maxbits, int restrict_on,
                                                     const int* parent_local, const int* dixp, int b, double* sb,
                                                     const v2d* fr);
 
-template <int NC, int OP, int BS>
+template <int NC, int OP, int BS, bool STORE = true>
 __device__ __forceinline__ void resid_restrict_box(const LevelView& F, const LevelView& Cv, double lambda,
                                                    unsigned long long* maxbits, int restrict_on,
                                                    const int* parent_local, const int* dixp, int b, double* sb,
@@ -47,10 +47,21 @@
       }
   }
   __syncthreads();
-  resid_restrict_core<NC, OP, BS>(F, Cv, lambda, maxbits, restrict_on, parent_local, dixp, b, sb, fr);
-}
-
-template <int NC, int OP, int BS>
+  resid_restrict_core<NC, OP, BS, STORE>(F, Cv, lambda, maxbits, restrict_on, parent_local, dixp, b, sb, fr);
+}
+
+template <bool ON>
+__device__ __forceinline__ int step_zero(double mx) {
+  if constexpr (ON) {
+    int zero = 0;
+    asm volatile("" : "+v"(zero) : "v"(mx));
+    return zero;
+  } else {
+    return 0;
+  }
+}
+
+template <int NC, int OP, int BS, bool STORE>
 __device__ __forceinline__ void resid_restrict_core(const LevelView& F, const LevelView& Cv, double lambda,
                                                     unsigned long long* maxbits, int restrict_on,
                                                     const int* parent_local, const int* dixp, int b, double* sb,
@@ -70,7 +81,8 @@
     const int e = q2 >= HV / 2, o = 1 - e;
     Nbr7 s0, s1;
     if constexpr (HN % 2 == 0) {
-      pair_stencil<NC>(sb + o * HV, sb + 2 * HV + o * FH, FS, e, 2 * q2 - e * HV, s0, s1);
+      pair_stencil<NC>(sb + o * HV, sb + 2 * HV + o * FH, FS, e,
+                       2 * q2 - e * HV + step_zero<!STORE && (NR > 1)>(mx), s0, s1);
     } else {
       int i, j, k;
       TL::decode(2 * q2, i, j, k);
@@ -90,7 +102,7 @@
     const double r0 = fr[r].x - l0, r1 = fr[r].y - l1;
     mx = amax(mx, amax(fabs(r0), fabs(r1)));
     rv[r] = make_double2(r0, r1);
-    st_nt(res + 2 * q2, r0, r1);
+    if constexpr (STORE) st_nt(res + 2 * q2, r0, r1);
   }
   if (maxbits) launch_max<BS>(maxbits, mx);
   if (!restrict_on || parent_local[b] < 0) return;
@@ -123,7 +135,7 @@
   }
 }
 
-template <int NC, int OP, int BS>
+template <int NC, int OP, int BS, bool STORE = true>
 __global__ void __launch_bounds__(BS) k_resid_restrict(LevelView F, LevelView Cv, double lambda,
                                                        unsigned long long* maxbits, int restrict_on,
                                                        const int* parent_local, const int* dixp,
@@ -131,8 +143,8 @@
                                                        int n_rsh) {
   __shared__ double sb[Tl<NC>::NST];
   const int q = xcd_box(blockIdx.x, gridDim.x, F.rev);
-  resid_restrict_box<NC, OP, BS>(F, Cv, lambda, maxbits, restrict_on, parent_local, dixp, list ? list[q] : q, sb,
-                                 rsh, n_rsh);
+  resid_restrict_box<NC, OP, BS, STORE>(F, Cv, lambda, maxbits, restrict_on, parent_local, dixp,
+                                        list ? list[q] : q, sb, rsh, n_rsh);
 }
 
 template <int NC>
@@ -878,15 +890,20 @@
 
 void launch_resid_restrict(const LevelView& F, const LevelView& C, int op, double lambda,
                            unsigned long long* maxbits, int restrict_on, const int* parent_local,
-                           const int* dixp, hipStream_t st, const int* list, int n_list, RhsShifts rs) {
+                           const int* dixp, hipStream_t st, const int* list, int n_list, RhsShifts rs,
+                           bool store) {
   const int n = list ? n_list : F.n;
   if (n == 0) return;
   if (rs.n < 0 || rs.n > kRhsPendMax || (rs.n && !rs.s))
     throw std::runtime_error("launch_resid_restrict: at most kRhsPendMax pending rhs shifts");
   const dim3 g(n);
-#define OMG_RR_OP(NC, BS, OPV)                                                                                  \
-  k_resid_restrict<NC, OPV, BS><<<g, dim3(BS), 0, st>>>(F, C, lambda, maxbits, restrict_on, parent_local, dixp, \
-                                                        list, rs.s, rs.n);
+#define OMG_RR_OP(NC, BS, OPV)                                                                             \
+  if (store)                                                                                               \
+    k_resid_restrict<NC, OPV, BS, true><<<g, dim3(BS), 0, st>>>(F, C, lambda, maxbits, restrict_on,        \
+                                                                parent_local, dixp, list, rs.s, rs.n);     \
+  else                                                                                                     \
+    k_resid_restrict<NC, OPV, BS, false><<<g, dim3(BS), 0, st>>>(F, C, lambda, maxbits, restrict_on,       \
+                                                                 parent_local, dixp, list, rs.s, rs.n);
 #define OMG_RR(NC, BS) OMG_FOR_OP(op, OMG_RR_OP, NC, BS)
   switch (F.nc) {
     case 16: OMG_RR(16, 512) break;
```

Result: faster. 39.35 billion cell-updates/s (median of 6 runs) (+2.7%).
